# cl-volume-renderer/cl-volume-renderer

Measured on AMD Instinct MI355X. Metric: msamples_per_sec, higher is better.
Workload: dtype f32

## Files before the change

cl_volume_renderer_amd/csrc/bounce_device.hpp:

```cpp
#pragma once
#include "render_device.hpp"

namespace clvr {

__device__ __forceinline__ VolumePacked make_volume(const RenderArgs &a) {
  return VolumePacked{a.grec, a.stepb, a.volume_lin, a.sdf_lin, a.X, a.Y, a.Z, a.NBX, a.NBY};
}

__device__ __forceinline__ uint32_t udivmod24(uint32_t n, uint32_t d, uint32_t &rem) {
  uint32_t q = (uint32_t)((float)n * __builtin_amdgcn_rcpf((float)d));
  uint32_t qd;
  asm("v_mul_u32_u24 %0, %1, %2" : "=v"(qd) : "v"(q), "v"(d));
  int32_t r = (int32_t)(n - qd);
  if (r < 0) { q -= 1u; r += (int32_t)d; }
  if (r >= (int32_t)d) { q += 1u; r -= (int32_t)d; }
  rem = (uint32_t)r;
  return q;
}

__device__ __forceinline__ unsigned prefix_count(unsigned long long mask) {
  return __builtin_amdgcn_mbcnt_hi((unsigned)(mask >> 32), __builtin_amdgcn_mbcnt_lo((unsigned)mask, 0u));
}
__device__ __forceinline__ unsigned lane_id() { return prefix_count(~0ull); }

enum : int { ST_IDLE = 0, ST_MARCH = 1, ST_CERT = 2, ST_EVENT = 8 };
enum : int { EV_START = 3,
             EV_HIT_COLOR_PENDING = 4,
             EV_CHECK = 5 };
constexpr int kCertNever = 255;

template <int MODE>
__device__ __forceinline__ void finish_item(const RenderArgs &a, int64_t entry, uint32_t hit, uint32_t gx, uint32_t gy,
                                            uint32_t bv_r, uint32_t bv_g, uint32_t bv_b) {
  const uint32_t cr = (bv_r / 2u) & 0xFFFFu, cg = (bv_g / 2u) & 0xFFFFu, cb = (bv_b / 2u) & 0xFFFFu;
  if (MODE == CLWH_ACCUM_VOXEL_CACHE && a.grants == nullptr) {
    cache_add(a.cache, entry, cr, cg, cb, 0u);
  } else {
    const unsigned long long packed = (unsigned long long)cr | ((unsigned long long)cg << 16) |
                                      ((unsigned long long)cb << 32) | (1ull << 48);
    atomicAdd(a.delta + hit, packed);
  }
  if (a.contrib_out) {
    uint32_t *q = a.contrib_out + ((size_t)gy * (size_t)a.launch_w + gx) * 4;
    q[0] = cr; q[1] = cg; q[2] = cb; q[3] = 1u;
  }
}

constexpr int kFixupDwords = 32;

__device__ __forceinline__ bool certify_exit(const RenderArgs &a, f3 p, f3 d, int budget, int &away) {
  const unsigned cx = min((unsigned)(int)p.x >> a.macro_shift, (unsigned)a.MNX - 1u), cy = min((unsigned)(int)p.y >> a.macro_shift, (unsigned)a.MNY - 1u),
                 cz = min((unsigned)(int)p.z >> a.macro_shift, (unsigned)a.MNZ - 1u);
  const unsigned octant = (d.x < 0.0f ? 1u : 0u) | (d.y < 0.0f ? 2u : 0u) | (d.z < 0.0f ? 4u : 0u);
  const int entry = a.macro[(((cz * (unsigned)a.MNY + cy) * (unsigned)a.MNX + cx) << 3) | octant];
  const bool refused = (entry & (int)kCertRefused) != 0;
  const int box_min = refused ? 0 : entry;
  away = refused ? ((entry & 0x7F) - 1) << a.macro_shift : 0;
  const float dmin = fminf(fminf(fabsf(d.x), fabsf(d.y)), fabsf(d.z));
  const float dsum = d.x + d.y + d.z;
  const float T = (float)((budget - 5) * box_min);
  const float fx = d.x < 0.0f ? p.x : (float)a.X - p.x, fy = d.y < 0.0f ? p.y : (float)a.Y - p.y, fz = d.z < 0.0f ? p.z : (float)a.Z - p.z;
  const bool leaves = T * fabsf(d.x) >= fx || T * fabsf(d.y) >= fy || T * fabsf(d.z) >= fz;
  return box_min != 0 && budget > 5 && leaves && dmin >= 0.0009765625f && dsum == dsum;
}
__device__ __forceinline__ bool start_certificate(uint32_t mask, f3 d, float dmin_needed) {
  const unsigned octant = (d.x < 0.0f ? 1u : 0u) | (d.y < 0.0f ? 2u : 0u) | (d.z < 0.0f ? 4u : 0u);
  const float dmin = fminf(fminf(fabsf(d.x), fabsf(d.y)), fabsf(d.z));
  const float dsum = d.x + d.y + d.z;
  return ((mask >> octant) & 1u) != 0u && dmin >= dmin_needed && dsum == dsum;
}
__device__ __forceinline__ f3 hull_direction(unsigned k) {
  static_assert(kHullGrid == 64, "cell centres are odd multiples of 1/64");
  const float u = (float)(2 * (int)(k & 63u) - 63) * 0.015625f, v = (float)(2 * (int)((k >> 6) & 63u) - 63) * 0.015625f;
  const float z = (1.0f - fabsf(u)) - fabsf(v);
  const float x = z >= 0.0f ? u : copysignf(1.0f - fabsf(v), u), y = z >= 0.0f ? v : copysignf(1.0f - fabsf(u), v);
  const float r = __builtin_amdgcn_rsqf((x * x + y * y) + z * z);
  return f3{x * r, y * r, z * r};
}
__device__ __forceinline__ bool certify_exit(const RenderArgs &a, f3 p, f3 d, int budget) {
  int away;
  return certify_exit(a, p, d, budget, away);
}

template <int SMALL>
__device__ __forceinline__ void index_tables_to_lds(VolumePacked &vol, const RenderArgs &a, int threads) {
  extern __shared__ uint32_t lds_parts[];
  if (SMALL == 2) {
    vol.parts = lds_parts;
    vol.parts_y0 = a.X;
    vol.parts_z0 = a.X + a.Y;
    for (int k = (int)threadIdx.x; k < a.X + a.Y + a.Z; k += threads)
      lds_parts[k] = k < a.X ? vol.part_x<1>((unsigned)k) : (k < a.X + a.Y ? vol.part_y<1>((unsigned)(k - a.X)) : vol.part_z<1>((unsigned)(k - a.X - a.Y)));
  }
}
__device__ __forceinline__ unsigned home_queue_of(const RenderArgs &a, unsigned waves_per_block) {
  unsigned home_queue = (unsigned)__builtin_amdgcn_s_getreg((3 << 11) | 20) & 7u;
  if (a.unit_affinity == 1) home_queue = (blockIdx.x * waves_per_block + (threadIdx.x >> 6)) & 7u;
  if (a.unit_affinity == 2) home_queue = 0u;
  return home_queue;
}

#ifdef CLVR_BOUNCE_STATS
constexpr bool kBounceStats = true;
constexpr bool kStartCertVerify = (CLVR_BOUNCE_STATS + 0) != 2;
#else
constexpr bool kBounceStats = false;
constexpr bool kStartCertVerify = false;
#endif
template <bool ON> struct BounceStatsT;
template <> struct BounceStatsT<false> {
  __device__ void step(int) {}
  __device__ void cert_begin(int, int) {}
  __device__ void cert_end(int, int) {}
  __device__ void closing_half(int) {}
  __device__ void event_phase(int) {}
  __device__ void refill(uint32_t) {}
  __device__ void fresh_items(int, int) {}
  __device__ void swap_point() {}
  __device__ void start_cert(bool, bool) {}
  __device__ void hull_cert(bool, bool, bool) {}
  __device__ void hull_more(bool, bool, bool, bool) {}
  __device__ void hull_fired(bool, bool) {}
  __device__ void march_end(uint32_t *, int) {}
  template <bool TWO_RAYS> __device__ void flush(uint32_t *) {}
};
template <> struct BounceStatsT<true> {
  uint32_t step_iters = 0, step_lanes = 0, event_phases = 0, event_lanes = 0, refills = 0, refill_lanes = 0;
  uint32_t ev_kind[4] = {0, 0, 0, 0};
  uint32_t cert_phases = 0, cert_lanes = 0, cert_granted = 0;
  uint32_t step_idle = 0;
  uint32_t swaps = 0;
  uint32_t closing = 0, marching_before = 0;
  __device__ __forceinline__ void step(int st) {
    step_iters += 1; step_lanes += (uint32_t)__popcll(__ballot(st == ST_MARCH));
    step_idle += (uint32_t)__popcll(__ballot(st == ST_IDLE));
  }
  __device__ __forceinline__ void cert_begin(int st, int n_cert) {
    cert_phases += 1; cert_lanes += (uint32_t)n_cert;
    marching_before = (uint32_t)__popcll(__ballot(st == ST_MARCH));
  }
  __device__ __forceinline__ void cert_end(int st, int n_cert) { cert_granted += (uint32_t)(n_cert - (__popcll(__ballot(st == ST_MARCH)) - (int)marching_before)); }
  __device__ __forceinline__ void closing_half(int st) {
    closing = (uint32_t)__popcll(__ballot(st >= ST_EVENT));
    event_lanes += closing;
    ev_kind[1] += (uint32_t)__popcll(__ballot(st == ST_EVENT + EV_EXIT || st == ST_EVENT + EV_CHECK));
    ev_kind[2] += (uint32_t)__popcll(__ballot(st == ST_EVENT + EV_HIT || st == ST_EVENT + EV_HIT_COLOR_PENDING));
    ev_kind[3] += (uint32_t)__popcll(__ballot(st == ST_EVENT + EV_NONE));
  }
  __device__ __forceinline__ void event_phase(int st) {
    if (__ballot(st >= ST_EVENT) != 0ull) { event_phases += 1; event_lanes += (uint32_t)__popcll(__ballot(st >= ST_EVENT)); }
  }
  __device__ __forceinline__ void refill(uint32_t count) { refills += 1; refill_lanes += count; }
  __device__ __forceinline__ void fresh_items(int st, int o) {
    const uint32_t n_fresh = (uint32_t)__popcll(__ballot(st == ST_EVENT + EV_START && o == 1));
    ev_kind[0] += n_fresh; event_lanes += n_fresh;
    if (closing + n_fresh != 0u) event_phases += 1;
  }
  __device__ __forceinline__ void swap_point() { swaps += 1; }
  uint32_t start_tried = 0, start_granted = 0;
  bool start_open = false;
  __device__ __forceinline__ void start_cert(bool tried, bool granted) {
    start_tried += (uint32_t)__popcll(__ballot(tried)); start_granted += (uint32_t)__popcll(__ballot(granted));
    start_open = start_open || granted;
  }
  uint32_t hull_tried = 0, hull_granted = 0, hull_both = 0;
  bool hull_open = false;
  __device__ __forceinline__ void hull_cert(bool tried, bool granted, bool both) {
    hull_tried += (uint32_t)__popcll(__ballot(tried)); hull_granted += (uint32_t)__popcll(__ballot(granted));
    hull_both += (uint32_t)__popcll(__ballot(both));
    hull_open = hull_open || granted;
  }
  uint32_t more_tried[3] = {0, 0, 0}, more_granted[3] = {0, 0, 0};
  int more_open = -1;
  __device__ __forceinline__ void hull_more(bool rebound_tried, bool rebound_granted, bool armed, bool first_leg) {
    more_tried[0] += (uint32_t)__popcll(__ballot(armed && first_leg)); more_tried[2] += (uint32_t)__popcll(__ballot(armed && !first_leg));
    more_tried[1] += (uint32_t)__popcll(__ballot(rebound_tried)); more_granted[1] += (uint32_t)__popcll(__ballot(rebound_granted));
    if (rebound_granted) more_open = 1;
  }
  __device__ __forceinline__ void hull_fired(bool fired, bool first_leg) {
    more_granted[0] += (uint32_t)__popcll(__ballot(fired && first_leg)); more_granted[2] += (uint32_t)__popcll(__ballot(fired && !first_leg));
    if (fired) more_open = first_leg ? 0 : 2;
  }
  __device__ __forceinline__ void march_end(uint32_t *counters, int ev) {
    if (start_open && ev != EV_EXIT) atomicAdd(&counters[CTR_START_WRONG], 1u);
    if (hull_open && ev != EV_EXIT) atomicAdd(&counters[CTR_HULL_WRONG], 1u);
    if (more_open >= 0 && ev != EV_EXIT) atomicAdd(&counters[CTR_HULL_DEFER + 3 * more_open + 2], 1u);
    start_open = false;
    hull_open = false;
    more_open = -1;
  }
  template <bool TWO_RAYS> __device__ __forceinline__ void flush(uint32_t *counters) {
    atomicAdd(&counters[CTR_STEP_ITERS], step_iters); atomicAdd(&counters[CTR_STEP_LANES], step_lanes);
    atomicAdd(&counters[CTR_EVENT_PHASES], event_phases); atomicAdd(&counters[CTR_EVENT_LANES], event_lanes);
    atomicAdd(&counters[CTR_REFILLS], refills); atomicAdd(&counters[CTR_REFILL_LANES], refill_lanes);
    if (TWO_RAYS) { atomicAdd(&counters[CTR_SWAPS], swaps); return; }
    for (int k = 0; k < 4; ++k) atomicAdd(&counters[CTR_EV_KIND + k], ev_kind[k]);
    atomicAdd(&counters[CTR_CERT_PHASES], cert_phases); atomicAdd(&counters[CTR_CERT_LANES], cert_lanes);
    atomicAdd(&counters[CTR_CERT_GRANTED], cert_granted); atomicAdd(&counters[CTR_STEP_IDLE], step_idle);
    atomicAdd(&counters[CTR_START_TRIED], start_tried); atomicAdd(&counters[CTR_START_GRANTED], start_granted);
    atomicAdd(&counters[CTR_HULL_TRIED], hull_tried); atomicAdd(&counters[CTR_HULL_GRANTED], hull_granted); atomicAdd(&counters[CTR_HULL_BOTH], hull_both);
    for (int k = 0; k < 3; ++k) { atomicAdd(&counters[CTR_HULL_DEFER + 3 * k], more_tried[k]); atomicAdd(&counters[CTR_HULL_DEFER + 3 * k + 1], more_granted[k]); }
  }
};
using BounceStats = BounceStatsT<kBounceStats>;

}
```

cl_volume_renderer_amd/csrc/clwh_context.hip:

```cpp
#include <algorithm>
#include <cstdio>
#include <cstdlib>
#include <cstring>
#include <mutex>
#include <new>

#include "clwh_host.hpp"

using namespace clvr;

static thread_local int g_last_hip_error = 0;
void clvr::note_hip_error(hipError_t e) { g_last_hip_error = (int)e; }

static std::atomic<uint64_t> g_content_version{0};
static std::mutex g_cells_mutex;
static std::map<const void *, std::weak_ptr<VersionCell>> g_version_cells;
void clwh_touch(clwh_mem *m) { m->cell->v.store(++g_content_version, std::memory_order_relaxed); }

static std::shared_ptr<VersionCell> version_cell_of(const void *dptr) {
  std::lock_guard<std::mutex> lock(g_cells_mutex);
  auto it = g_version_cells.find(dptr);
  if (it != g_version_cells.end())
    if (auto live = it->second.lock()) return live;
  auto cell = std::make_shared<VersionCell>();
  g_version_cells[dptr] = cell;
  if (g_version_cells.size() > 4096) {
    for (auto i = g_version_cells.begin(); i != g_version_cells.end();)
      i = i->second.expired() ? g_version_cells.erase(i) : std::next(i);
  }
  return cell;
}

static size_t elem_size(int kind) {
  switch (kind) {
    case CLWH_ELEM_S8: case CLWH_ELEM_U8: return 1;
    case CLWH_ELEM_S16: case CLWH_ELEM_U16: return 2;
    case CLWH_ELEM_S32: case CLWH_ELEM_U32: case CLWH_ELEM_F32: return 4;
    default: return 0;
  }
}


void clvr::tf_to_dev(const clwh_tf &tf, TfDev &d) {
  std::memset(&d, 0, sizeof d);
  d.n = tf.n;
  for (int k = 0; k < tf.n; ++k) {
    const clwh_tf_rule &r = tf.rules[k];
    TfRuleDev &o = d.rules[k];
    o.v_lo = r.v_lo; o.v_hi = r.v_hi; o.g_lo = r.g_lo; o.g_hi = r.g_hi;
    o.flags = (r.use_gradient ? TF_USE_GRADIENT : 0u) | (r.writes_color ? TF_WRITES_COLOR : 0u) |
              (r.terminal ? TF_TERMINAL : 0u);
    o.color = ((uint32_t)r.color[0] & 255u) | (((uint32_t)r.color[1] & 255u) << 8) |
              (((uint32_t)r.color[2] & 255u) << 16) | (((uint32_t)r.color[3] & 255u) << 24);
    if (r.use_gradient) d.uses_gradient = 1;
  }
  for (int k = 0; k < tf.n && !d.uses_gradient; ++k) {
    const clwh_tf_rule &r = tf.rules[k];
    if (r.v_lo <= 0 && 0 <= r.v_hi) { d.border_class = k + 1; break; }
    if (r.terminal) break;
  }
}

int clvr::jit_for_source(clwh_ctx *ctx, const char *source, std::shared_ptr<JitTf> &out) {
  auto it = ctx->classes.cache.find(source);
  if (it != ctx->classes.cache.end()) {
    out = it->second;
    return CLWH_OK;
  }
  auto j = std::make_shared<JitTf>();
  j->source = source;
  std::string log;
  const int rc = tf_jit_compile(source, j->code, log);
  if (rc != CLWH_OK) {
    if (!log.empty()) std::fprintf(stderr, "clwhip: transfer-function source is neither in the rule grammar nor compilable:\n%s\n", log.c_str());
    return rc;
  }
  ctx->classes.cache[source] = j;
  out = j;
  return CLWH_OK;
}

int clvr::ensure_classes(clwh_ctx *ctx, const std::shared_ptr<JitTf> &jit, const clwh_mem *volume, TfDev &tf_out, const uint8_t **cls_out) {
  TfClasses &c = ctx->classes;
  if (c.cls.ptr && c.vol == volume->dptr && c.vol_ver == volume->version() && c.source == jit->source) {
    tf_out = c.tf;
    *cls_out = c.cls.as<uint8_t>();
    return CLWH_OK;
  }
  if (!jit->module) {
    HIP_TRY(hipModuleLoadData(&jit->module, jit->code.data()));
    HIP_TRY(hipModuleGetFunction(&jit->classify, jit->module, "clvr_tf_classify"));
  }
  const size_t voxels = volume->dims[0] * volume->dims[1] * volume->dims[2];
  CLWH_TRY(c.cls.reserve(ctx->stream, voxels));
  constexpr int kColors = CLWH_TF_MAX_RULES;
  CLWH_TRY(c.palette.reserve(ctx->stream, (kColors + 2) * sizeof(unsigned long long)));
  unsigned long long *palette = c.palette.as<unsigned long long>();
  HIP_TRY(hipMemsetAsync(palette, 0xFF, kColors * sizeof(unsigned long long), ctx->stream));
  HIP_TRY(hipMemsetAsync(palette + kColors, 0, 2 * sizeof(unsigned long long), ctx->stream));
  const void *vol = volume->dptr;
  int X = (int)volume->dims[0], Y = (int)volume->dims[1], Z = (int)volume->dims[2], max_colors = kColors;
  unsigned char *cls = c.cls.as<unsigned char>();
  int *error = reinterpret_cast<int *>(palette + kColors);
  int *border = reinterpret_cast<int *>(palette + kColors + 1);
  void *args[] = {&vol, &X, &Y, &Z, &cls, &palette, &max_colors, &error, &border};
  const size_t blocks = std::min<size_t>((voxels + 255u) / 256u, (size_t)1u << 23);
  HIP_TRY(hipModuleLaunchKernel(jit->classify, (unsigned)blocks, 1, 1, 256, 1, 1, 0, ctx->stream, args, nullptr));
  unsigned long long host[kColors + 2];
  HIP_TRY(hipMemcpyAsync(host, palette, sizeof host, hipMemcpyDeviceToHost, ctx->stream));
  HIP_TRY(hipStreamSynchronize(ctx->stream));
  c.vol = nullptr;
  if ((int)(host[kColors] & 0xFFFFFFFFull) != 0) return CLWH_ERR_TF_UNSUPPORTED;
  TfDev t;
  std::memset(&t, 0, sizeof t);
  t.opaque = 1;
  for (int k = 0; k < kColors && host[k] != ~0ull; ++k) {
    t.rules[k].flags = (host[k] >> 32) & 1ull ? TF_WRITES_COLOR : 0u;
    t.rules[k].color = (uint32_t)(host[k] & 0xFFFFFFFFull);
    t.n = k + 1;
  }
  t.border_class = (int32_t)(host[kColors + 1] & 0xFFull);
  c.tf = t;
  c.vol = volume->dptr;
  c.vol_ver = volume->version();
  c.source = jit->source;
  tf_out = t;
  *cls_out = cls;
  return CLWH_OK;
}


Tuning clvr::tuning_from_environment() {
  Tuning t;
  auto clamped = [](const char *e, int lo, int hi) { return std::max(lo, std::min(hi, std::atoi(e))); };
  if (const char *e = std::getenv("CLWH_TUNE_STEP")) t.step_min_lanes = clamped(e, 0, 64);
  if (const char *e = std::getenv("CLWH_TUNE_REFILL")) t.refill_min_lanes = clamped(e, 0, 64);
  if (const char *e = std::getenv("CLWH_TUNE_LITERAL_GRADIENT")) t.literal_gradient = std::atoi(e) != 0;
  if (const char *e = std::getenv("CLWH_TUNE_AFFINITY")) t.unit_affinity = std::atoi(e);
  if (const char *e = std::getenv("CLWH_TUNE_QUEUES")) t.unit_queues = clamped(e, 1, 8);
  if (const char *e = std::getenv("CLWH_TUNE_GROUP")) t.unit_group = std::max(1, std::atoi(e));
  if (const char *e = std::getenv("CLWH_TUNE_CHUNK_BLOCK_LOG2")) t.unit_block_log2 = clamped(e, 0, 8);
  if (const char *e = std::getenv("CLWH_TUNE_BLOCKS")) t.bounce_max_blocks = (uint32_t)std::max(1, std::atoi(e));
  if (const char *e = std::getenv("CLWH_TUNE_MACRO_SHIFT")) t.macro_shift = std::atoi(e);
  if (const char *e = std::getenv("CLWH_TUNE_LONG_LAUNCH")) t.force_long_launch = std::atoi(e) != 0;
  if (const char *e = std::getenv("CLWH_TUNE_BOUNCE_RAYS")) t.bounce_rays = std::atoi(e) == 2 ? 2 : 1;
  if (const char *e = std::getenv("CLWH_TUNE_SDF")) t.sdf_front = std::strcmp(e, "front") == 0;
  if (const char *e = std::getenv("CLWH_TUNE_DIST_LINES")) t.dist_lines = std::strcmp(e, "scan") == 0 ? 1 : std::strcmp(e, "search") == 0 ? 2 : 0;
  if (const char *e = std::getenv("CLWH_TUNE_LABEL_STATS")) t.label_stats = std::strcmp(e, "item") == 0 ? 1 : std::strcmp(e, "direct") == 0 ? 2 : 0;
  if (const char *e = std::getenv("CLWH_TUNE_SLICE_COARSE")) t.slice_coarse = std::atoi(e) != 0;
  if (const char *e = std::getenv("CLWH_TUNE_SDFBIT_WAVES")) t.sdfbit_waves = std::atoi(e) == 16 ? 16 : 8;
  if (const char *e = std::getenv("CLWH_TUNE_SDFBIT_GRID")) t.sdfbit_grid = std::max(1, std::atoi(e));
  if (const char *e = std::getenv("CLWH_TUNE_SDFBIT_REC")) t.sdfbit_rec_lds = std::strcmp(e, "lds") == 0 ? 1 : 0;
  if (const char *e = std::getenv("CLWH_TUNE_CERT")) t.cert_min_step = clamped(e, 0, 127);
  if (const char *e = std::getenv("CLWH_TUNE_CERT_HINT")) t.cert_hint = std::atoi(e) != 0;
  if (const char *e = std::getenv("CLWH_TUNE_START_CERT")) t.start_cert = std::atoi(e) != 0;
  if (const char *e = std::getenv("CLWH_TUNE_HULL_CERT")) t.hull_cert = std::atoi(e) != 0;
  if (const char *e = std::getenv("CLWH_TUNE_HULL_DEFER")) t.hull_defer = std::atoi(e) != 0;
  return t;
}

int clvr::check_device_flags(clwh_ctx *ctx) {
  PassScratch &p = ctx->pass;
  if (!p.fixup_overflow_pending || !p.sticky_flags.ptr) return CLWH_OK;
  uint32_t flag = 0;
  HIP_TRY(hipMemcpyAsync(&flag, p.sticky_flags.ptr, sizeof flag, hipMemcpyDeviceToHost, ctx->stream));
  HIP_TRY(hipStreamSynchronize(ctx->stream));
  p.fixup_overflow_pending = false;
  if (!flag) return CLWH_OK;
  HIP_TRY(hipMemsetAsync(p.sticky_flags.ptr, 0, sizeof(uint32_t), ctx->stream));
  return CLWH_ERR_INTERNAL_OVERFLOW;
}

int clvr::timed_begin(clwh_ctx *ctx, int which, hipEvent_t *end) {
  LaunchTimers &t = ctx->timers;
  if (!t.enabled) return CLWH_OK;
  if (t.used == t.pairs.size()) {
    LaunchTimers::Pair &fresh = t.pairs.emplace_back();
    int rc = fresh.begin.ensure(hipEventDefault);
    if (rc == CLWH_OK) rc = fresh.end.ensure(hipEventDefault);
    if (rc != CLWH_OK) {
      t.pairs.pop_back();
      return rc;
    }
  }
  LaunchTimers::Pair &p = t.pairs[t.used++];
  p.which = which;
  HIP_TRY(hipEventRecord(p.begin.ev, ctx->stream));
  *end = p.end.ev;
  return CLWH_OK;
}

static int order_streams(clwh_ctx *ctx, hipStream_t first, hipStream_t then) {
  HIP_TRY(hipSetDevice(ctx->device));
  CLWH_TRY(ctx->handoff.ensure(hipEventDisableTiming));
  HIP_TRY(hipEventRecord(ctx->handoff.ev, first));
  HIP_TRY(hipStreamWaitEvent(then, ctx->handoff.ev, 0));
  return CLWH_OK;
}

extern "C" {

int clwh_ctx_create_on_stream(int device, void *hip_stream, clwh_ctx **out) {
  if (!out) return CLWH_ERR_INVALID_VALUE;
  *out = nullptr;
  int count = 0;
  hipError_t e = hipGetDeviceCount(&count);
  if (e != hipSuccess || count <= 0) {
    note_hip_error(e);
    return CLWH_ERR_NO_DEVICE;
  }
  if (device < 0 || device >= count) return CLWH_ERR_NO_DEVICE;
  HIP_TRY(hipSetDevice(device));
  clwh_ctx *c = new (std::nothrow) clwh_ctx();
  if (!c) return CLWH_ERR_OUT_OF_MEMORY;
  c->device = device;
  c->stream = (hipStream_t)hip_stream;
  c->own_stream = false;
  c->tune = tuning_from_environment();
  *out = c;
  return CLWH_OK;
}

int clwh_ctx_create(int device, clwh_ctx **out) {
  CLWH_TRY(clwh_ctx_create_on_stream(device, nullptr, out));
  hipStream_t s;
  hipError_t e = hipStreamCreateWithFlags(&s, hipStreamNonBlocking);
  if (e != hipSuccess) {
    note_hip_error(e);
    delete *out;
    *out = nullptr;
    return CLWH_ERR_HIP;
  }
  (*out)->stream = s;
  (*out)->own_stream = true;
  return CLWH_OK;
}

int clwh_ctx_destroy(clwh_ctx *ctx) {
  if (!ctx) return CLWH_ERR_INVALID_VALUE;
  (void)hipSetDevice(ctx->device);
  (void)hipStreamSynchronize(ctx->stream);
  for (auto &kv : ctx->classes.cache)
    if (kv.second->module) (void)hipModuleUnload(kv.second->module);
  ctx->scene.reset();
  const hipStream_t owned = ctx->own_stream ? ctx->stream : nullptr;
  delete ctx;
  if (owned) (void)hipStreamDestroy(owned);
  return CLWH_OK;
}

int clwh_ctx_finish(clwh_ctx *ctx) {
  if (!ctx) return CLWH_ERR_INVALID_VALUE;
  HIP_TRY(hipStreamSynchronize(ctx->stream));
  return check_device_flags(ctx);
}

int clwh_ctx_acquire_from(clwh_ctx *ctx, void *hip_stream) {
  if (!ctx) return CLWH_ERR_INVALID_VALUE;
  return order_streams(ctx, (hipStream_t)hip_stream, ctx->stream);
}

int clwh_ctx_release_to(clwh_ctx *ctx, void *hip_stream) {
  if (!ctx) return CLWH_ERR_INVALID_VALUE;
  return order_streams(ctx, ctx->stream, (hipStream_t)hip_stream);
}

void *clwh_ctx_stream(clwh_ctx *ctx) { return ctx ? (void *)ctx->stream : nullptr; }
int clwh_ctx_device(clwh_ctx *ctx) { return ctx ? ctx->device : -1; }

int clwh_ctx_set_timing(clwh_ctx *ctx, int enabled) {
  if (!ctx) return CLWH_ERR_INVALID_VALUE;
  ctx->timers.enabled = enabled != 0;
  ctx->timers.used = 0;
  return CLWH_OK;
}

int clwh_ctx_timing_read_all(clwh_ctx *ctx, float *ms, int32_t *launches, int32_t n) {
  if (!ctx || !ms || !launches || n <= 0) return CLWH_ERR_INVALID_VALUE;
  for (int k = 0; k < n; ++k) { ms[k] = 0.0f; launches[k] = 0; }
  HIP_TRY(hipSetDevice(ctx->device));
  LaunchTimers &timers = ctx->timers;
  for (size_t i = 0; i < timers.used; ++i) {
    const LaunchTimers::Pair &p = timers.pairs[i];
    HIP_TRY(hipEventSynchronize(p.end.ev));
    float t = 0.0f;
    HIP_TRY(hipEventElapsedTime(&t, p.begin.ev, p.end.ev));
    if (p.which >= 0 && p.which < n) { ms[p.which] += t; launches[p.which] += 1; }
  }
  timers.used = 0;
  return CLWH_OK;
}

int clwh_ctx_timing_read(clwh_ctx *ctx, float *total_ms, int32_t *launches) {
  if (!ctx || !total_ms || !launches) return CLWH_ERR_INVALID_VALUE;
  float ms[CLWH_TIMER_COUNT];
  int32_t n[CLWH_TIMER_COUNT];
  const int rc = clwh_ctx_timing_read_all(ctx, ms, n, CLWH_TIMER_COUNT);
  *total_ms = ms[CLWH_TIMER_BOUNCE];
  *launches = n[CLWH_TIMER_BOUNCE];
  return rc;
}


static int mem_new(clwh_ctx *ctx, void *dptr, size_t bytes, bool owned, clwh_mem **out) {
  clwh_mem *m = new (std::nothrow) clwh_mem();
  if (!m) return CLWH_ERR_OUT_OF_MEMORY;
  m->ctx = ctx;
  m->dptr = dptr;
  m->bytes = bytes;
  m->owned = owned;
// ... 155 lines not shown
```

cl_volume_renderer_amd/csrc/clwh_host.hpp:

```cpp
#pragma once

#include <atomic>
#include <deque>
#include <map>
#include <memory>
#include <string>
#include <vector>

#include "clwh_internal.hpp"

namespace clvr {

void note_hip_error(hipError_t e);
inline int hip_failed(hipError_t e) {
  note_hip_error(e);
  return e == hipErrorOutOfMemory ? CLWH_ERR_OUT_OF_MEMORY : CLWH_ERR_HIP;
}
#define HIP_TRY(expr)                                   \
  do {                                                  \
    hipError_t _e = (expr);                             \
    if (_e != hipSuccess) return clvr::hip_failed(_e);  \
  } while (0)
#define CLWH_TRY(expr)                \
  do {                                \
    int _rc = (expr);                 \
    if (_rc != CLWH_OK) return _rc;   \
  } while (0)

struct NoCopy {
  NoCopy() = default;
  NoCopy(const NoCopy &) = delete;
  NoCopy &operator=(const NoCopy &) = delete;
};

struct DeviceBuffer : NoCopy {
  void *ptr = nullptr;
  size_t bytes = 0;
  ~DeviceBuffer() { if (ptr) (void)hipFree(ptr); }
  template <class T>
  T *as() const { return static_cast<T *>(ptr); }
  void *release() {
    void *p = ptr;
    ptr = nullptr;
    bytes = 0;
    return p;
  }
  int reserve(hipStream_t stream, size_t need, bool *reallocated = nullptr) {
    if (reallocated) *reallocated = bytes < need;
    if (bytes >= need) return CLWH_OK;
    if (ptr) {
      HIP_TRY(hipStreamSynchronize(stream));
      HIP_TRY(hipFree(ptr));
      (void)release();
    }
    HIP_TRY(hipMalloc(&ptr, need));
    bytes = need;
    return CLWH_OK;
  }
};

struct Event : NoCopy {
  hipEvent_t ev = nullptr;
  ~Event() { if (ev) (void)hipEventDestroy(ev); }
  int ensure(unsigned flags) {
    if (!ev) HIP_TRY(hipEventCreateWithFlags(&ev, flags));
    return CLWH_OK;
  }
};

struct PinnedWord : NoCopy {
  uint32_t *ptr = nullptr;
  ~PinnedWord() { if (ptr) (void)hipHostFree(ptr); }
  int ensure() {
    if (!ptr) HIP_TRY(hipHostMalloc((void **)&ptr, 64, hipHostMallocDefault));
    return CLWH_OK;
  }
};

int tf_jit_compile(const char *user_source, std::vector<char> &code, std::string &log);
struct JitTf {
  std::string source;
  std::vector<char> code;
  hipModule_t module = nullptr;
  hipFunction_t classify = nullptr;
};

struct PackedScene {
  int device = 0;
  DeviceBuffer data;
  const void *vol = nullptr, *sdf = nullptr;
  uint64_t vol_ver = 0, sdf_ver = 0;
  TfDev tf{};
  std::string tf_identity;
  int32_t macro_shift = 0;
  bool start_table = false;
  bool hull_table = false;
  int32_t dims[3] = {0, 0, 0};
  uint64_t generation = 0;
  Event ready;
  bool stale = false;
  ~PackedScene();
};

struct VersionCell {
  std::atomic<uint64_t> v{0};
};


struct Tuning {
  int32_t step_min_lanes = 0;
  int32_t refill_min_lanes = 0;
  int32_t macro_shift = 0;
  int32_t bounce_rays = 1;
  int32_t force_long_launch = 0;
  int32_t literal_gradient = 0;
  int32_t unit_block_log2 = 4;
  int32_t unit_group = 1, unit_affinity = 0, unit_queues = 8;
  int32_t cert_hint = 1;
  int32_t start_cert = 1;
  int32_t hull_cert = 1;
  int32_t hull_defer = 1;
  int32_t cert_min_step = -1;
  uint32_t bounce_max_blocks = 2048;
  int32_t sdfbit_waves = 8;
  int32_t sdfbit_grid = 512;
  int32_t sdfbit_rec_lds = 0;
  int32_t sdf_front = 0;
  int32_t dist_lines = 0;
  int32_t label_stats = 0;
  int32_t slice_coarse = 1;
};
Tuning tuning_from_environment();

struct PrimaryHits {
  struct Key {
    float cam_pos[3], cam_dir[3];
    int32_t frame_w, frame_h, launch_w, launch_h, tile_rank, tile_world;
    int64_t cache_entries;
    int32_t mode, shading;
    uint64_t packed_generation;
    const void *env;
    uint64_t env_version;
    int32_t env_w, env_h;
  } key{};
  bool valid = false;
  DeviceBuffer pix_slot, hits;
  DeviceBuffer hull_codes;
  DeviceBuffer hull_planes;
  uint32_t n_hits = 0;
  bool n_hits_known = false;
  PinnedWord host_n_hits;
  Event n_hits_event;
  bool n_hits_in_flight = false;
  uint32_t last_known_n_hits = 0;
};

struct PassScratch {
  static constexpr size_t kCounters = CTR_QUEUE_STRIDE * 10;
  DeviceBuffer counters;
  DeviceBuffer fixups, delta;
  DeviceBuffer sticky_flags;
  bool fixup_overflow_pending = false;
};

struct VoxelPlan {
  DeviceBuffer plan;
  DeviceBuffer temp;
  bool valid = false;
  uint32_t n = 0;
};

struct TfClasses {
  std::map<std::string, std::shared_ptr<JitTf>> cache;
  DeviceBuffer cls;
  DeviceBuffer palette;
  const void *vol = nullptr;
  uint64_t vol_ver = 0;
  std::string source;
  TfDev tf{};
};

struct SdfScratch {
  DeviceBuffer counters;
  DeviceBuffer flags;
  DeviceBuffer bits;
#ifdef CLVR_SDFBIT_TIMING
  DeviceBuffer timing;
#endif
};

struct TileScratch {
  DeviceBuffer tiles, seeds;
  PinnedWord host;
};

struct GrowScratch {
  DeviceBuffer admissible;
  TileScratch work;
};

struct LabelScratch {
  DeviceBuffer admissible, keys, temp, counters;
  PinnedWord host;
};

struct DistanceScratch {
  DeviceBuffer map_a, map_b, bits;
};

struct GeodesicScratch {
  DeviceBuffer keys, trace;
  TileScratch work;
};

struct RegionStatsScratch {
  DeviceBuffer result;
};

struct OverlayScratch {
  DeviceBuffer pixel_ids, occupancy;
};

struct ProjectionData {
  DeviceBuffer data;
  bool valid = false;
  const void *vol = nullptr;
  uint64_t vol_ver = 0;
  size_t dims[3] = {0, 0, 0};
  DeviceBuffer dilated;
  bool dilated_valid = false;
  DeviceBuffer mesh_counts, mesh_temp, mesh_points;
  DeviceBuffer lut_prefix;
  bool lut_valid = false;
  const void *lut = nullptr;
  uint64_t lut_ver = 0;
  int32_t lut_len = 0;
};

struct LaunchTimers {
  struct Pair {
    Event begin, end;
    int which = 0;
  };
  bool enabled = false;
  std::deque<Pair> pairs;
  size_t used = 0;
};

}

struct clwh_ctx {
  int device = 0;
  hipStream_t stream = nullptr;
  bool own_stream = false;
  clvr::Event handoff;
  clvr::Tuning tune;
  clvr::PrimaryHits primary;
  clvr::PassScratch pass;
  clvr::VoxelPlan vox;
  clvr::TfClasses classes;
  clvr::SdfScratch sdf;
  clvr::GrowScratch grow;
  clvr::LabelScratch label;
  clvr::DistanceScratch distance;
  clvr::GeodesicScratch geodesic;
  clvr::RegionStatsScratch region_stats;
  clvr::OverlayScratch overlay;
  clvr::ProjectionData proj;
  clvr::DeviceBuffer bilateral_weights;
  std::shared_ptr<clvr::PackedScene> scene;
  clvr::LaunchTimers timers;
};

struct clwh_mem {
  clwh_ctx *ctx = nullptr;
  void *dptr = nullptr;
  size_t bytes = 0;
  bool owned = false;
  bool is_image = false;
  size_t dims[3] = {1, 1, 1};
  int channels = 1;
  int elem_kind = CLWH_ELEM_U8;
  int flags = 0;
  std::shared_ptr<clvr::VersionCell> cell;
  uint64_t version() const { return cell ? cell->v.load(std::memory_order_relaxed) : 0; }
};

enum clwh_kernel_id {
  CLWH_K_EMPTY = 0,
  CLWH_K_RENDER,
  CLWH_K_SDF_BASE,
  CLWH_K_SDF_LAYER,
  CLWH_K_BUFFER_RESET,
  CLWH_K_FETCH_STATS,
  CLWH_K_APPLY_CLIP,
  CLWH_K_TF_SORT_VALUES,
  CLWH_K_TF_FLUSH_COLOR_FRAME,
  CLWH_K_BILATERAL_FILTER
};

struct clwh_kernel {
  clwh_ctx *ctx = nullptr;
  int id = CLWH_K_EMPTY;
  clwh_tf tf{};
  bool has_tf = false;
  std::shared_ptr<clvr::JitTf> jit;
};

void clwh_touch(clwh_mem *m);

namespace clvr {

inline void touch(clwh_mem *m) { clwh_touch(m); }
// ... 102 lines not shown
```

cl_volume_renderer_amd/csrc/clwh_internal.hpp:

```cpp
#pragma once

#include <hip/hip_runtime.h>
#include <stdint.h>

#include "../../include/clwh.h"

namespace clvr {

struct TfRuleDev {
  int32_t v_lo, v_hi, g_lo, g_hi;
  uint32_t flags;
  uint32_t color;
};
struct TfDev {
  int32_t n;
  int32_t uses_gradient;
  int32_t literal_gradient_taps;
  int32_t opaque;
  int32_t border_class;
  TfRuleDev rules[CLWH_TF_MAX_RULES];
};

enum : uint32_t { TF_USE_GRADIENT = 1u, TF_WRITES_COLOR = 2u, TF_TERMINAL = 4u };

struct HitRec {
  float origin[3];
  float direction[3];
  float normal[3];
  uint32_t color;
  int32_t entry_lo;
  int32_t entry_hi;
  uint32_t xy;
  uint32_t pslot;
  uint32_t start_free;
  uint32_t pad;
};
static_assert(sizeof(HitRec) == 64, "HitRec must be one 64-byte line");

enum : uint32_t { PIX_HIT = 0x80000000u };

constexpr uint32_t kCertMinStep = 2u;
constexpr uint32_t kCertRefused = 0x80u;

enum : uint32_t {
  CTR_HITS = 0, CTR_FIXUPS = 2,
  CTR_STEP_ITERS = 8, CTR_STEP_LANES, CTR_EVENT_PHASES, CTR_EVENT_LANES, CTR_REFILLS, CTR_REFILL_LANES,
  CTR_EV_KIND,
  CTR_CERT_PHASES = CTR_EV_KIND + 4, CTR_CERT_LANES, CTR_CERT_GRANTED,
  CTR_SWAPS, CTR_STEP_IDLE,
  CTR_START_TRIED, CTR_START_GRANTED, CTR_START_WRONG,
  CTR_HULL_TRIED, CTR_HULL_GRANTED, CTR_HULL_BOTH, CTR_HULL_WRONG,
  CTR_STATS_END,
  CTR_QUEUE_STRIDE = 32,
  CTR_HULL_DEFER = CTR_QUEUE_STRIDE * 9, CTR_HULL_DEFER_END = CTR_HULL_DEFER + 9,
};
struct RenderArgs {
  int32_t X, Y, Z;
  const uint2 *grec;
  const uint8_t *stepb;
  const int16_t *volume_lin;
  const int8_t *sdf_lin;
  const uint8_t *macro;
  int32_t MNX, MNY, MNZ, macro_shift;
  int32_t cert_min_step;
  int32_t cert_min_lanes;
  int32_t cert_hint;
  const uint8_t *start_free;
  float start_cert_dmin;
  const float4 *hull;
  uint32_t *hull_codes;
  float hull_delta0;
  uint32_t *hull_planes;
  float hull_defer_delta0;
  int32_t NBX, NBY;
  const uint32_t *env;
  int32_t env_w, env_h;
  uint32_t *cache;
  int64_t cache_entries;
  uint32_t *frame;
  int32_t frame_w, frame_h;
  int32_t launch_w, launch_h;
  int32_t tiles_x, tiles_y, tiles_per_row;
  int32_t tile_rank, tile_world;
  float cam_pos[3];
  float cam_dir[3];
  int32_t mode;
  float4 *accum;
  unsigned long long *delta;
  const uint32_t *grants;
  uint32_t *pix_slot;
  HitRec *hits;
  uint32_t *counters;
  uint32_t *fixups;
  uint32_t fixup_capacity;
  uint32_t *sticky_flags;
  uint32_t n_hits;
  uint32_t n_hits_estimate;
  int32_t n_hits_on_device;
  int32_t shading;
  int64_t *hit_index_out;
  uint32_t *contrib_out;
  uint32_t num_tile_slots;
  int32_t n_seeds;
  int32_t seeds[CLWH_MAX_SEEDS];
  int32_t step_min_lanes;
  int32_t refill_min_lanes;
  int32_t force_long_launch;
  int32_t bounce_rays;
  uint32_t bounce_max_blocks;
  int32_t unit_group;
  int32_t unit_block_log2;
  int32_t unit_queues;
  int32_t unit_affinity;
  TfDev tf;
};

struct RepackArgs {
  const int16_t *volume;
  const int8_t *sdf;
  int32_t X, Y, Z;
  int32_t NBX, NBY, NBZ;
  uint2 *grec;
  uint8_t *stepb;
  uint32_t *brick_min;
  const uint8_t *cls_in;
  TfDev tf;
};

struct SdfArgs {
  const int16_t *volume;
  int32_t X, Y, Z;
  int8_t *ping;
  int8_t *pong;
  int32_t max_iterations;
  int32_t iteration;
  int32_t *counters;
  int32_t *done;
  int32_t *counter_out;
  const uint8_t *cls_in;
  TfDev tf;
};

hipError_t launch_repack(const RepackArgs &a, hipStream_t s);
inline int macro_cell_shift(int X, int Y, int Z, int forced) {
  if (forced >= 3 && forced <= 8) return forced;
  auto cells = [&](int sh) { return (int64_t)((X >> sh) + 1) * ((Y >> sh) + 1) * ((Z >> sh) + 1); };
  int shift = 4;
  if (cells(4) > 40000) {
    shift = 5;
    while (shift < 8 && cells(shift) > 300000) ++shift;
  }
  return shift;
}
hipError_t launch_macro_table(const uint32_t *brick_min, int NBX, int NBY, int NBZ, uint8_t *macro, int X, int Y, int Z, int shift, hipStream_t s);
hipError_t launch_start_table(const uint8_t *stepb, uint8_t *table, uint32_t *regular, int2 *ends, int X, int Y, int Z, int NBX, int NBY, int NBZ, hipStream_t s);
inline int start_cert_cap(int X, int Y, int Z) {
  const int longest = X > Y ? (X > Z ? X : Z) : (Y > Z ? Y : Z);
  return longest / 2 < 127 ? longest / 2 : 127;
}
inline float start_cert_dmin(int X, int Y, int Z) {
  const double longest = (double)(X > Y ? (X > Z ? X : Z) : (Y > Z ? Y : Z));
  const double reach = 1.7320508075688772 * (longest + 1.0), cap = (double)start_cert_cap(X, Y, Z);
  for (int k = 1; k <= 64; ++k) {
    const double dmin = (double)k / 64.0;
    double t = 0.0;
    for (int step = 0; step < 70 - 5 && t <= reach; ++step) {
      const double m = (double)(long long)(t * dmin) - 2.0;
      const double bound = m > cap ? cap : m;
      t += bound < 1.0 ? 1.0 : bound;
    }
    if (t > reach) return (float)dmin;
  }
  return 2.0f;
}
constexpr int kHullGrid = 64;
constexpr int kHullPlanes = kHullGrid * kHullGrid;
constexpr float kHullSlack = 0.0625f;
constexpr int kHullMaxDim = 2048;
inline float hull_cert_delta0(int X, int Y, int Z) {
  const double longest = (double)(X > Y ? (X > Z ? X : Z) : (Y > Z ? Y : Z));
  const double reach = 1.7320508075688772 * (longest + 1.0), cap = (double)start_cert_cap(X, Y, Z);
  for (int k = 1; k <= 64; ++k) {
    const double delta0 = (double)k / 64.0;
    double t = 0.0;
    for (int step = 0; step < 70 - 5 && t <= reach; ++step) {
      const double m = (double)(long long)(t * delta0 / 1.7320508075688772) - 2.0;
      const double bound = m > cap ? cap : m;
      t += bound < 1.0 ? 1.0 : bound;
    }
    if (t > reach) return (float)delta0;
  }
  return 2.0f;
}
constexpr int kHullDeferSteps = 3;
constexpr float kHullDeferDeficit = 1.5f;
constexpr int kHullMarginScale = 16;
inline float hull_defer_delta0(int X, int Y, int Z) {
  const double longest = (double)(X > Y ? (X > Z ? X : Z) : (Y > Z ? Y : Z));
  const double reach = 1.7320508075688772 * (longest + 1.0), cap = (double)start_cert_cap(X, Y, Z);
  for (int k = 1; k <= 64; ++k) {
    const double delta0 = (double)k / 64.0;
    double t = 0.0;
    for (int step = 0; step < 70 - 5 - kHullDeferSteps && t <= reach; ++step) {
      const double m = (double)(long long)(t * delta0 / 1.7320508075688772) - 2.0;
      const double bound = m > cap ? cap : m;
      t += bound < 1.0 ? 1.0 : bound;
    }
    if (t > reach) return (float)delta0;
  }
  return 2.0f;
}
hipError_t launch_hull_table(const int2 *ends, const uint32_t *regular, float4 *hull, int X, int Y, int Z, hipStream_t s);
constexpr uint64_t kStartTableBudget = 2ull << 30;
hipError_t launch_primary(const RenderArgs &a, hipStream_t s);
hipError_t launch_bounce(const RenderArgs &a, hipStream_t s);
inline bool bounce_queues_fit(uint32_t n_hits, int32_t unit_block_log2, int32_t n_seeds) {
  return (uint64_t)(((n_hits + 63u) >> 6) + 8u * (1u << unit_block_log2)) * (uint64_t)n_seeds < (1ull << 24);
}
hipError_t launch_env_fixup(const RenderArgs &a, hipStream_t s);
hipError_t launch_commit(const RenderArgs &a, hipStream_t s);
constexpr int64_t kVoxKeyInvalid = (int64_t)1 << 38;
constexpr int64_t kVoxKeyNone = ((int64_t)1 << 38) + 1;
hipError_t launch_vox_keys(const RenderArgs &a, int64_t *keys, uint32_t *iota, uint32_t n, hipStream_t s);
hipError_t launch_vox_grant(const RenderArgs &a, const int64_t *sorted_keys, const uint32_t *order, uint32_t n, uint32_t *grants, hipStream_t s);
hipError_t launch_commit_voxel(const RenderArgs &a, hipStream_t s);
hipError_t sort_entry_pairs(void *temp, size_t &temp_bytes, const int64_t *keys_in, int64_t *keys_out, const uint32_t *vals_in,
                            uint32_t *vals_out, size_t n, unsigned end_bit, hipStream_t s);
hipError_t launch_resolve(const RenderArgs &a, hipStream_t s);
hipError_t launch_ao(const RenderArgs &a, hipStream_t s);
hipError_t launch_accum_resolve(const RenderArgs &a, const float4 *accum_all, hipStream_t s);
hipError_t launch_accum_resolve_tiles(const RenderArgs &a, const float4 *accum, uint32_t *tiles_out, hipStream_t s);
hipError_t launch_frame_from_tiles(const RenderArgs &a, const uint32_t *tiles_all, hipStream_t s);
struct ProbeShape {
  uint32_t in_words, out_words;
};
ProbeShape probe_shape(int which);
hipError_t launch_device_probe(int which, const uint32_t *in, uint64_t n, uint32_t *out, const uint32_t *aux, const int32_t params[4], hipStream_t s);
struct SdfFrontArgs {
  int8_t *sdf;
  int32_t X, Y, Z;
  int32_t TX, TY, TZ;
  const uint8_t *flags_cur;
  uint8_t *flags_next;
  uint8_t *flags_clear;
  uint8_t *tile_done;
  int32_t iteration;
  int32_t max_iterations;
  int32_t *counters;
};

struct SdfBitArgs {
  int8_t *sdf;
  const uint32_t *ev;
  const uint32_t *r_in;
  uint32_t *r_out;
  uint8_t *state;
  uint8_t *wake;
  int32_t launch;
  int32_t *presence;
  int32_t X, Y, Z, WP;
  int32_t BX, BY, BZ, core_z;
  int32_t r0, steps;
  uint32_t *planes;
  size_t plane_words;
  uint32_t *list;
  uint32_t *list_count;
  uint32_t *list_head;
#ifdef CLVR_SDFBIT_TIMING
  unsigned long long *timing;
#endif
};
void sdfbit_block_grid(int X, int Y, int Z, int waves, int32_t *BX, int32_t *BY, int32_t *BZ, int32_t *core_z);
hipError_t launch_sdfbit_events(const SdfArgs &a, uint32_t *ev, int32_t WP, hipStream_t s);
hipError_t launch_sdfbit_seed(const SdfBitArgs &a, hipStream_t s);
hipError_t launch_sdfbit_expand(const SdfBitArgs &a, const uint32_t *reached, int32_t max_iterations, hipStream_t s);
hipError_t launch_sdfbit_state(const SdfBitArgs &a, hipStream_t s);
hipError_t launch_sdfbit_layers(const SdfBitArgs &a, int waves, unsigned grid_blocks, bool rec_in_lds, hipStream_t s);

inline unsigned row_block(int X) { return X <= 64 ? 64u : (X <= 128 ? 128u : 256u); }
inline dim3 row_grid(int X, int Y, int Z) { return dim3(((unsigned)X + row_block(X) - 1u) / row_block(X), (unsigned)Y, (unsigned)Z); }
hipError_t launch_sdf_base(const SdfArgs &a, hipStream_t s);
hipError_t launch_sdf_base_front(const SdfArgs &a, uint8_t *flags, int32_t TX, int32_t TY, hipStream_t s);
hipError_t launch_sdf_front(const SdfFrontArgs &a, hipStream_t s);
hipError_t launch_sdf_layer(const SdfArgs &a, hipStream_t s);
hipError_t launch_fetch_stats(const int16_t *vol, int X, int Y, int Z, int32_t *stats, hipStream_t s);
hipError_t launch_tf_sort_values(const int16_t *vol, int X, int Y, int Z, uint32_t *frame, int width, int height,
                                 float min_v, float max_v, float min_g, float max_g, hipStream_t s);
hipError_t launch_tf_flush_color_frame(uint32_t *color_frame, int fw, int fh, const int32_t *frame, const int32_t *lookup,
                                       int lookup_len, hipStream_t s);
hipError_t launch_bilateral_filter(const int16_t *src, int X, int Y, int Z, int16_t *dst, const float *weights, hipStream_t s);
hipError_t launch_apply_clip(const int16_t *src, int SX, int SY, int SZ, int16_t *dst, int DX, int DY, int DZ,
                             const uint32_t *start, const uint32_t *len, hipStream_t s);


struct ViewVolume {
  const int16_t *bricks;
  const uint32_t *table, *dilated, *coarse;
  int32_t X, Y, Z, NBX, NBY, NBZ, CNX, CNY;
};
struct ViewFrame {
  uint32_t *frame;
  int32_t frame_w, frame_h;
  int32_t launch_w, launch_h, tiles_x, num_tiles;
};
struct ViewCamera {
  float cam_pos[3], cam_dir[3];
  float step, t_near, t_far;
  int32_t k_cap;
};

struct ProjRepackArgs {
  const int16_t *volume;
  int32_t X, Y, Z, NBX, NBY, NBZ;
  int16_t *bricks;
  uint32_t *table;
};
struct ProjArgs {
  ViewVolume vol;
  ViewFrame fr;
  ViewCamera cam;
  float window_center, window_width;
  float *values;
  float *t_extreme;
};
hipError_t launch_proj_repack(const ProjRepackArgs &a, hipStream_t s);
hipError_t launch_projection(const ProjArgs &a, int mode, bool dense, hipStream_t s);

struct CompArgs {
  ViewVolume vol;
  ViewFrame fr;
  ViewCamera cam;
  const float4 *lut;
  const uint32_t *prefix;
  int32_t lut_first, lut_len;
  float alpha_stop, ambient;
  float4 *rgba;
  float *t_first;
  float *t_stop;
};
hipError_t launch_comp_prefix(const float4 *lut, int32_t lut_len, uint32_t *prefix, hipStream_t s);
hipError_t launch_composite(const CompArgs &a, bool shade, bool dense, hipStream_t s);

struct IsoArgs {
  ViewVolume vol;
  ViewFrame fr;
  ViewCamera cam;
  int64_t threshold;
  int32_t skip_bound;
  int32_t refine;
  float color[3], ambient;
  float *t_hit;
  float4 *normal;
};
hipError_t launch_iso_dilate(const ViewVolume &v, uint32_t *dilated, hipStream_t s);
hipError_t launch_isosurface(const IsoArgs &a, bool below, bool dense, hipStream_t s);

struct SliceArgs {
  ViewVolume vol;
  ViewFrame fr;
  int32_t use_coarse;
  float origin[3], du[3], dv[3], normal[3];
  float step;
  float window_center, window_width;
  int32_t slab_samples;
  float *values;
  float *t_extreme;
};
hipError_t launch_slice(const SliceArgs &a, int mode, bool dense, hipStream_t s);
// ... 186 lines not shown
```

cl_volume_renderer_amd/csrc/clwh_render.hip:

```cpp
#include <algorithm>
#include <cstdio>
#include <cstring>
#include <mutex>

#include "clwh_host.hpp"

using namespace clvr;


static std::mutex g_scenes_mutex;
static std::vector<std::weak_ptr<PackedScene>> g_packed_scenes;
static std::atomic<uint64_t> g_packed_generation{0};

PackedScene::~PackedScene() {
  (void)hipSetDevice(device);
  (void)hipDeviceSynchronize();
}

struct PackedLayout {
  int X, Y, Z, NBX, NBY, NBZ, mshift, MNX, MNY, MNZ;
  size_t records, n_bricks, off_stepb, off_brick_min, off_macro, off_start, off_hull_ends, off_hull, bytes;
  bool start_table;
  bool hull_table;
};
// ... 81 lines not shown
  r.cls_in = cls_in;
  r.tf = tf;
  CLWH_TRY(timed(ctx, CLWH_TIMER_REPACK, [&] {
    const hipError_t e = launch_repack(r, ctx->stream);
    if (e != hipSuccess) return e;
    return launch_macro_table(r.brick_min, L.NBX, L.NBY, L.NBZ, data + L.off_macro, L.X, L.Y, L.Z, L.mshift, ctx->stream);
  }));
  if (L.start_table)
    CLWH_TRY(timed(ctx, CLWH_TIMER_REPACK, [&] {
      int2 *ends = L.hull_table ? reinterpret_cast<int2 *>(data + L.off_hull_ends) : nullptr;
      const hipError_t e = launch_start_table(r.stepb, data + L.off_start + 16u, reinterpret_cast<uint32_t *>(data + L.off_start), ends, L.X, L.Y, L.Z, L.NBX, L.NBY, L.NBZ, ctx->stream);
      if (e != hipSuccess || !L.hull_table) return e;
      return launch_hull_table(ends, reinterpret_cast<const uint32_t *>(data + L.off_start), reinterpret_cast<float4 *>(data + L.off_hull), L.X, L.Y, L.Z, ctx->stream);
    }));
  HIP_TRY(hipEventRecord(entry->ready.ev, ctx->stream));
  ctx->scene = entry;
  {
    std::lock_guard<std::mutex> lock(g_scenes_mutex);
    entry->vol = volume->dptr;
    entry->sdf = sdf->dptr;
    entry->vol_ver = volume->version();
    entry->sdf_ver = sdf->version();
    entry->tf = tf;
    entry->tf_identity = tf_identity;
    entry->macro_shift = L.mshift;
    entry->start_table = L.start_table;
    entry->hull_table = L.hull_table;
    entry->dims[0] = L.X; entry->dims[1] = L.Y; entry->dims[2] = L.Z;
    entry->generation = ++g_packed_generation;
    entry->stale = false;
    bool listed = false;
    for (auto &w : g_packed_scenes)
      if (w.lock() == entry) listed = true;
    if (!listed) g_packed_scenes.push_back(entry);
  }
  return CLWH_OK;
}


static void describe_frame(RenderArgs &a, int32_t launch_w, int32_t launch_h, int32_t frame_w, int32_t frame_h,
                           int32_t rank, int32_t world, const float cam_pos[3], const float cam_dir[3]) {
  a.launch_w = launch_w;
  a.launch_h = launch_h;
  a.frame_w = frame_w;
  a.frame_h = frame_h;
  a.tiles_x = launch_w / 8;
  a.tiles_y = launch_h / 8;
  a.tile_rank = rank;
  a.tile_world = world;
  a.tiles_per_row = (a.tiles_x + world - 1) / world;
  a.num_tile_slots = (uint32_t)a.tiles_y * (uint32_t)a.tiles_per_row;
  for (int q = 0; q < 3; ++q) {
    a.cam_pos[q] = cam_pos[q];
    a.cam_dir[q] = cam_dir[q];
  }
}

static size_t pixel_slots(const RenderArgs &a) { return (size_t)a.num_tile_slots * 64u; }
static size_t launch_pixels(const RenderArgs &a) { return (size_t)a.launch_w * (size_t)a.launch_h; }
static bool is_planned(const RenderArgs &a) { return a.mode == CLWH_ACCUM_VOXEL_CACHE && a.n_seeds > 1; }

static int validate_desc(const clwh_render_desc *d) {
  if (!is_image(d->volume, 3, 1, CLWH_ELEM_S16) || !is_image(d->sdf, 3, 1, CLWH_ELEM_S8) ||
      !is_image(d->env, 2, 4, CLWH_ELEM_U8))
    return CLWH_ERR_BAD_ARGS;
  if (d->frame && !is_image(d->frame, 2, 4, CLWH_ELEM_U8)) return CLWH_ERR_BAD_ARGS;
  if (!same_dims(d->volume, d->sdf)) return CLWH_ERR_SIZE_MISMATCH;
  if (!launch_size_ok(d->width, d->height)) return CLWH_ERR_BAD_NDRANGE;
  if (d->width > 65535u || d->height > 65535u) return CLWH_ERR_BAD_NDRANGE;
  if (d->env->dims[0] > 32768u || d->env->dims[1] > 32768u) return CLWH_ERR_INVALID_VALUE;
  if (!dims_fit_int32(d->volume)) return CLWH_ERR_INVALID_VALUE;
  const int world = d->tile_world < 1 ? 1 : d->tile_world;
  if (d->tile_rank < 0 || d->tile_rank >= world) return CLWH_ERR_INVALID_VALUE;
  if (d->n_seeds < 0 || d->n_seeds > CLWH_MAX_SEEDS) return CLWH_ERR_INVALID_VALUE;
  if (d->n_seeds > 1 && d->contrib) return CLWH_ERR_BAD_ARGS;
  if (d->shading != CLWH_SHADE_LIGHT && d->shading != CLWH_SHADE_AO) return CLWH_ERR_INVALID_VALUE;
  if (d->shading == CLWH_SHADE_AO && d->accum_mode != CLWH_ACCUM_VOXEL_CACHE) return CLWH_ERR_BAD_ARGS;
  return CLWH_OK;
}

static int describe_launch(const clwh_ctx *ctx, const clwh_render_desc *d, RenderArgs &a) {
  std::memset(&a, 0, sizeof a);
  a.X = (int32_t)d->volume->dims[0];
  a.Y = (int32_t)d->volume->dims[1];
  a.Z = (int32_t)d->volume->dims[2];
  env_into_args(a, d->env);
  const int32_t fw = d->frame ? (int32_t)d->frame->dims[0] : (int32_t)d->width;
  const int32_t fh = d->frame ? (int32_t)d->frame->dims[1] : (int32_t)d->height;
  const int world = d->tile_world < 1 ? 1 : d->tile_world;
  describe_frame(a, (int32_t)d->width, (int32_t)d->height, fw, fh, d->tile_rank, world, d->cam_pos, d->cam_dir);
  a.frame = d->frame ? (uint32_t *)d->frame->dptr : nullptr;
  a.mode = d->accum_mode;
  a.shading = d->shading;
  if (a.mode == CLWH_ACCUM_VOXEL_CACHE) {
    if (!d->buffer_volume || d->buffer_volume->bytes < 8) return CLWH_ERR_BAD_ARGS;
    a.cache = (uint32_t *)d->buffer_volume->dptr;
    a.cache_entries = (int64_t)(d->buffer_volume->bytes / (d->shading == CLWH_SHADE_AO ? 4 : 8));
  } else if (a.mode == CLWH_ACCUM_IMAGE_SPACE) {
    const int64_t need = clwh_accum_len(d->width, d->height, world) * 16;
    if (!d->accum || (int64_t)d->accum->bytes < need) return CLWH_ERR_BAD_ARGS;
    a.accum = (float4 *)d->accum->dptr;
  } else {
    return CLWH_ERR_INVALID_VALUE;
  }
  if (d->hit_index) {
    if (d->hit_index->bytes < launch_pixels(a) * 8) return CLWH_ERR_SIZE_MISMATCH;
    a.hit_index_out = (int64_t *)d->hit_index->dptr;
  }
  if (d->contrib) {
    if (d->contrib->bytes < launch_pixels(a) * 16) return CLWH_ERR_SIZE_MISMATCH;
    a.contrib_out = (uint32_t *)d->contrib->dptr;
  }
  if (d->n_seeds > 0) {
    a.n_seeds = d->n_seeds;
    for (int q = 0; q < d->n_seeds; ++q) a.seeds[q] = d->seeds[q];
  } else {
    a.n_seeds = 1;
    a.seeds[0] = d->seed;
  }
  const Tuning &t = ctx->tune;
  a.step_min_lanes = t.step_min_lanes;
  a.refill_min_lanes = t.refill_min_lanes;
  a.force_long_launch = t.force_long_launch;
  a.bounce_rays = t.bounce_rays;
  a.bounce_max_blocks = t.bounce_max_blocks;
  a.unit_group = t.unit_group;
  a.unit_block_log2 = t.unit_block_log2;
  a.unit_affinity = t.unit_affinity;
  a.unit_queues = t.unit_queues;
  a.cert_hint = t.cert_hint;
  a.start_cert_dmin = start_cert_dmin(a.X, a.Y, a.Z);
  a.hull_delta0 = hull_cert_delta0(a.X, a.Y, a.Z);
  a.hull_defer_delta0 = hull_defer_delta0(a.X, a.Y, a.Z);
  return CLWH_OK;
}

static int bind_scene(clwh_kernel *k, const clwh_render_desc *d, RenderArgs &a) {
  clwh_ctx *ctx = k->ctx;
  const uint8_t *cls_in = nullptr;
  CLWH_TRY(kernel_tf(k, d->volume, a.tf, &cls_in));
  a.tf.literal_gradient_taps = ctx->tune.literal_gradient;
  const PackedLayout L = packed_layout(d->volume, ctx->tune.macro_shift, wants_start_table(ctx->tune, a.tf, d->volume), wants_hull_table(ctx->tune, a.tf, d->volume));
  CLWH_TRY(ensure_packed(ctx, L, d->volume, d->sdf, a.tf, cls_in, k->jit ? k->jit->source : std::string()));
  const uint8_t *packed = ctx->scene->data.as<uint8_t>();
  a.grec = reinterpret_cast<const uint2 *>(packed);
  a.NBX = L.NBX;
  a.NBY = L.NBY;
  a.stepb = packed + L.off_stepb;
  a.volume_lin = (const int16_t *)d->volume->dptr;
  a.sdf_lin = (const int8_t *)d->sdf->dptr;
  a.macro = packed + L.off_macro;
  a.start_free = L.start_table ? packed + L.off_start + 16u : nullptr;
  a.hull = L.hull_table ? reinterpret_cast<const float4 *>(packed + L.off_hull) : nullptr;
  a.macro_shift = L.mshift;
  a.MNX = L.MNX; a.MNY = L.MNY; a.MNZ = L.MNZ;
  bool zero_may_hit = a.tf.border_class != 0;
  for (int q = 0; q < a.tf.n && a.tf.uses_gradient && !a.tf.opaque; ++q)
    if (a.tf.rules[q].v_lo <= 0 && 0 <= a.tf.rules[q].v_hi) zero_may_hit = true;
  const int cert_auto = a.macro_shift < 4 ? 12 >> (4 - a.macro_shift) : std::min(12 << (a.macro_shift - 4), 48);
  a.cert_min_step = zero_may_hit ? 0 : (ctx->tune.cert_min_step >= 0 ? ctx->tune.cert_min_step : cert_auto);
  return CLWH_OK;
}

static int ensure_primary_hits(clwh_ctx *ctx, const clwh_render_desc *d, RenderArgs &a) {
  PrimaryHits &p = ctx->primary;
  PassScratch &s = ctx->pass;
  const size_t slots = pixel_slots(a);
  CLWH_TRY(p.pix_slot.reserve(ctx->stream, slots * sizeof(uint32_t)));
  CLWH_TRY(p.hits.reserve(ctx->stream, slots * sizeof(HitRec)));
  if (a.hull) CLWH_TRY(p.hull_codes.reserve(ctx->stream, slots * sizeof(uint32_t)));
  const bool defer = a.hull && ctx->tune.hull_defer != 0;
  if (defer) CLWH_TRY(p.hull_planes.reserve(ctx->stream, slots * sizeof(uint32_t)));
  CLWH_TRY(s.counters.reserve(ctx->stream, PassScratch::kCounters * sizeof(uint32_t)));
  bool fresh_flags = false;
  CLWH_TRY(s.sticky_flags.reserve(ctx->stream, 64, &fresh_flags));
  if (fresh_flags) HIP_TRY(hipMemsetAsync(s.sticky_flags.ptr, 0, 64, ctx->stream));
  a.sticky_flags = s.sticky_flags.as<uint32_t>();
  a.pix_slot = p.pix_slot.as<uint32_t>();
  a.hits = p.hits.as<HitRec>();
  a.hull_codes = a.hull ? p.hull_codes.as<uint32_t>() : nullptr;
  a.hull_planes = defer ? p.hull_planes.as<uint32_t>() : nullptr;
  a.counters = s.counters.as<uint32_t>();

  PrimaryHits::Key key;
  std::memset(&key, 0, sizeof key);
  for (int q = 0; q < 3; ++q) {
    key.cam_pos[q] = a.cam_pos[q];
    key.cam_dir[q] = a.cam_dir[q];
  }
  key.frame_w = a.frame_w; key.frame_h = a.frame_h;
  key.launch_w = a.launch_w; key.launch_h = a.launch_h;
  key.tile_rank = a.tile_rank; key.tile_world = a.tile_world;
  key.cache_entries = a.cache_entries;
  key.mode = a.mode;
  key.shading = a.shading;
  key.packed_generation = ctx->scene->generation;
  key.env = d->env->dptr;
  key.env_version = d->env->version();
  key.env_w = a.env_w; key.env_h = a.env_h;
  if (p.valid && std::memcmp(&key, &p.key, sizeof key) == 0 && !a.hit_index_out) return CLWH_OK;
  p.valid = false;
  HIP_TRY(hipMemsetAsync(a.counters, 0, PassScratch::kCounters * sizeof(uint32_t), ctx->stream));
  CLWH_TRY(timed(ctx, CLWH_TIMER_PRIMARY, [&] { return launch_primary(a, ctx->stream); }));
  CLWH_TRY(p.host_n_hits.ensure());
  CLWH_TRY(p.n_hits_event.ensure(hipEventDisableTiming));
  HIP_TRY(hipMemcpyAsync(p.host_n_hits.ptr, a.counters + CTR_HITS, sizeof(uint32_t), hipMemcpyDeviceToHost, ctx->stream));
  HIP_TRY(hipEventRecord(p.n_hits_event.ev, ctx->stream));
  p.n_hits_in_flight = true;
  ctx->vox.valid = false;
  p.n_hits_known = false;
  p.key = key;
  p.valid = true;
  return CLWH_OK;
}

static int pick_up_hit_count(clwh_ctx *ctx, RenderArgs &a) {
  PrimaryHits &p = ctx->primary;
  if (p.n_hits_in_flight && !p.n_hits_known) {
    if (hipEventQuery(p.n_hits_event.ev) == hipSuccess) {
      p.n_hits = *p.host_n_hits.ptr;
      p.n_hits_known = true;
      p.n_hits_in_flight = false;
      p.last_known_n_hits = p.n_hits;
    } else {
      (void)hipGetLastError();
    }
  }
  const size_t slots = pixel_slots(a);
  a.n_hits_on_device = !p.n_hits_known;
  a.n_hits = p.n_hits_known ? p.n_hits : (uint32_t)std::min<size_t>(slots, 0xFFFFFFFFu);
  a.n_hits_estimate = a.n_hits;
  if (!p.n_hits_known && p.last_known_n_hits != 0)
    a.n_hits_estimate = (uint32_t)std::min<uint64_t>(a.n_hits, std::max<uint64_t>(2ull * p.last_known_n_hits, slots / 4u));
  if (!bounce_queues_fit(a.n_hits, ctx->tune.unit_block_log2, a.n_seeds)) return CLWH_ERR_INVALID_VALUE;
  return CLWH_OK;
}

static int size_pass_buffers(clwh_ctx *ctx, RenderArgs &a) {
  PassScratch &s = ctx->pass;
  const double rate = std::min(1.0, std::max(1.0 / 64.0, 3.0 * 8.0e-6 * (0.16 * a.env_w + 0.32 * a.env_h)));
  const size_t fix_cap = std::max<size_t>((size_t)((double)a.n_hits_estimate * (double)a.n_seeds * rate), 4096u);
  CLWH_TRY(s.fixups.reserve(ctx->stream, fix_cap * 128u));
  a.fixups = s.fixups.as<uint32_t>();
  a.fixup_capacity = (uint32_t)std::min<size_t>(s.fixups.bytes / 128u, 0x7fffffffu);
  if (a.mode == CLWH_ACCUM_IMAGE_SPACE || is_planned(a)) {
    bool fresh = false;
    CLWH_TRY(s.delta.reserve(ctx->stream, std::max<size_t>(pixel_slots(a), 1) * sizeof(unsigned long long), &fresh));
    a.delta = s.delta.as<unsigned long long>();
    if (fresh) HIP_TRY(hipMemsetAsync(s.delta.ptr, 0, s.delta.bytes, ctx->stream));
  }
  return CLWH_OK;
}

static int plan_voxel_grants(clwh_ctx *ctx, RenderArgs &a) {
  if (!is_planned(a)) return CLWH_OK;
  VoxelPlan &v = ctx->vox;
  constexpr size_t kPerElement = 2 * sizeof(int64_t) + 3 * sizeof(uint32_t);
  bool moved = false;
  CLWH_TRY(v.plan.reserve(ctx->stream, pixel_slots(a) * kPerElement, &moved));
  if (moved) v.valid = false;
  const size_t have = v.plan.bytes / kPerElement;
  int64_t *keys_in = v.plan.as<int64_t>(), *keys = keys_in + have;
  uint32_t *iota = reinterpret_cast<uint32_t *>(keys + have), *order = iota + have, *grants = order + have;
  if (!v.valid) {
    const uint32_t n = a.n_hits;
    HIP_TRY(launch_vox_keys(a, keys_in, iota, n, ctx->stream));
    size_t need = 0;
    HIP_TRY(sort_entry_pairs(nullptr, need, keys_in, keys, iota, order, n, 39u, ctx->stream));
    CLWH_TRY(v.temp.reserve(ctx->stream, std::max<size_t>(need, 16)));
    size_t tb = v.temp.bytes;
    HIP_TRY(sort_entry_pairs(v.temp.ptr, tb, keys_in, keys, iota, order, n, 39u, ctx->stream));
    v.valid = true;
    v.n = n;
  }
  HIP_TRY(launch_vox_grant(a, keys, order, v.n, grants, ctx->stream));
  a.grants = grants;
  return CLWH_OK;
}

#ifdef CLVR_BOUNCE_STATS
static int print_bounce_stats(clwh_ctx *ctx, const RenderArgs &a) {
  uint32_t h[CTR_HULL_DEFER_END];
  HIP_TRY(hipMemcpyAsync(h, a.counters, sizeof h, hipMemcpyDeviceToHost, ctx->stream));
  HIP_TRY(hipStreamSynchronize(ctx->stream));
  auto per = [&](int sum, int n) { return h[n] ? (double)h[sum] / h[n] : 0.0; };
  std::fprintf(stderr, "[bounce stats] items=%llu step_iters=%u avg_march_lanes=%.2f event_phases=%u avg_event_lanes=%.2f "
               "refills=%u avg_refill=%.2f events start/exit/hit/none=%u/%u/%u/%u cert_phases=%u avg_cert_lanes=%.2f cert_granted=%u\n",
               (unsigned long long)h[CTR_HITS] * (unsigned long long)a.n_seeds, h[CTR_STEP_ITERS], per(CTR_STEP_LANES, CTR_STEP_ITERS),
               h[CTR_EVENT_PHASES], per(CTR_EVENT_LANES, CTR_EVENT_PHASES), h[CTR_REFILLS], per(CTR_REFILL_LANES, CTR_REFILLS), h[CTR_EV_KIND],
               h[CTR_EV_KIND + 1], h[CTR_EV_KIND + 2], h[CTR_EV_KIND + 3], h[CTR_CERT_PHASES], per(CTR_CERT_LANES, CTR_CERT_PHASES), h[CTR_CERT_GRANTED]);
  if (h[CTR_SWAPS]) std::fprintf(stderr, "[bounce stats] two rays per lane: %u swap points\n", h[CTR_SWAPS]);
  std::fprintf(stderr, "[bounce stats] per step iteration: avg_idle_lanes=%.2f (lane sum %u)\n", per(CTR_STEP_IDLE, CTR_STEP_ITERS), h[CTR_STEP_IDLE]);
  std::fprintf(stderr, "[bounce stats] lane_steps=%u event_lanes=%u start certificates (%s) tried/granted/wrong=%u/%u/%u dmin=%.6f\n", h[CTR_STEP_LANES],
               h[CTR_EVENT_LANES], (CLVR_BOUNCE_STATS + 0) == 2 ? "taken" : "verified: marched literally", h[CTR_START_TRIED], h[CTR_START_GRANTED],
               h[CTR_START_WRONG], (double)a.start_cert_dmin);
  std::fprintf(stderr, "[bounce stats] hull certificates tried/granted/wrong=%u/%u/%u, of the granted the octant proof grants %u; either proof grants %u first legs; delta0=%.6f\n",
               h[CTR_HULL_TRIED], h[CTR_HULL_GRANTED], h[CTR_HULL_WRONG], h[CTR_HULL_BOTH], h[CTR_START_GRANTED] + h[CTR_HULL_GRANTED] - h[CTR_HULL_BOTH],
               (double)a.hull_delta0);
  const uint32_t *m = h + CTR_HULL_DEFER;
  std::fprintf(stderr, "[bounce stats] hull certificates tried/granted/wrong: first legs deferred=%u/%u/%u rebounds at once=%u/%u/%u rebounds deferred=%u/%u/%u; "
               "J=%d D=%.4g defer_delta0=%.6f; look-ups=%u\n", m[0], m[1], m[2], m[3], m[4], m[5], m[6], m[7], m[8], kHullDeferSteps, (double)kHullDeferDeficit,
               (double)a.hull_defer_delta0, h[CTR_CERT_LANES] - ((CLVR_BOUNCE_STATS + 0) == 2 ? m[1] + m[7] : 0u));
  return CLWH_OK;
}
#endif

static int run_pass(clwh_ctx *ctx, const RenderArgs &a) {
  CLWH_TRY(timed(ctx, CLWH_TIMER_BOUNCE, [&] { return launch_bounce(a, ctx->stream); }));
#ifdef CLVR_BOUNCE_STATS
  CLWH_TRY(print_bounce_stats(ctx, a));
#endif
  CLWH_TRY(timed(ctx, CLWH_TIMER_FIXUP, [&] {
    hipError_t e = launch_env_fixup(a, ctx->stream);
    if (e == hipSuccess) e = launch_commit(a, ctx->stream);
    if (e == hipSuccess && is_planned(a)) e = launch_commit_voxel(a, ctx->stream);
    return e;
  }));
  ctx->pass.fixup_overflow_pending = true;
  return CLWH_OK;
}

extern "C" {

int64_t clwh_cache_len(uint32_t X, uint32_t Y, uint32_t Z) {
  return ((int64_t)X * Z * Y + (int64_t)X * Z + X + 1) * 4;
}

int64_t clwh_accum_len(uint32_t width, uint32_t height, int32_t tile_world) {
  if (tile_world < 1) tile_world = 1;
  const int64_t tiles_x = width / 8, tiles_y = height / 8;
  const int64_t tiles_per_row = (tiles_x + tile_world - 1) / tile_world;
  return tiles_y * tiles_per_row * 64;
}

int clwh_render(clwh_kernel *k, const clwh_render_desc *d) {
  if (!k || !d || k->id != CLWH_K_RENDER || !k->has_tf) return CLWH_ERR_INVALID_VALUE;
  clwh_ctx *ctx = k->ctx;
  RenderArgs a;
  CLWH_TRY(validate_desc(d));
  CLWH_TRY(describe_launch(ctx, d, a));
  HIP_TRY(hipSetDevice(ctx->device));
  CLWH_TRY(bind_scene(k, d, a));
  CLWH_TRY(ensure_primary_hits(ctx, d, a));
  CLWH_TRY(pick_up_hit_count(ctx, a));

  HIP_TRY(hipMemsetAsync(a.counters + CTR_HITS + 1, 0, (PassScratch::kCounters - CTR_HITS - 1) * sizeof(uint32_t), ctx->stream));
  if (a.contrib_out) HIP_TRY(hipMemsetAsync(a.contrib_out, 0, launch_pixels(a) * 16, ctx->stream));

  if (d->resolve_only) {
    if (!a.frame) return CLWH_ERR_BAD_ARGS;
  } else if (d->shading == CLWH_SHADE_AO) {
    CLWH_TRY(timed(ctx, CLWH_TIMER_AO, [&] { return launch_ao(a, ctx->stream); }));
  } else {
    CLWH_TRY(size_pass_buffers(ctx, a));
    CLWH_TRY(plan_voxel_grants(ctx, a));
    CLWH_TRY(run_pass(ctx, a));
  }
  if ((d->write_frame || d->resolve_only) && a.frame)
    CLWH_TRY(timed(ctx, CLWH_TIMER_RESOLVE, [&] { return launch_resolve(a, ctx->stream); }));
  if (d->frame) touch(d->frame);
  return CLWH_OK;
}


int clwh_accum_resolve(clwh_ctx *ctx, clwh_mem *accum_all, int32_t tile_world, uint32_t width, uint32_t height,
                       clwh_mem *frame, clwh_mem *env, const float cam_pos[3], const float cam_dir[3]) {
  if (!ctx || !accum_all || !frame || !env || !cam_pos || !cam_dir || tile_world < 1) return CLWH_ERR_INVALID_VALUE;
  if (!is_image(frame, 2, 4, CLWH_ELEM_U8) || !is_image(env, 2, 4, CLWH_ELEM_U8)) return CLWH_ERR_BAD_ARGS;
  if (!launch_size_ok(width, height)) return CLWH_ERR_BAD_NDRANGE;
  const int64_t need = clwh_accum_len(width, height, tile_world) * 16 * tile_world;
  if ((int64_t)accum_all->bytes < need) return CLWH_ERR_SIZE_MISMATCH;
  RenderArgs a;
  std::memset(&a, 0, sizeof a);
  describe_frame(a, (int32_t)width, (int32_t)height, (int32_t)frame->dims[0], (int32_t)frame->dims[1], 0, tile_world,
                 cam_pos, cam_dir);
  a.frame = (uint32_t *)frame->dptr;
  env_into_args(a, env);
  HIP_TRY(hipSetDevice(ctx->device));
  CLWH_TRY(timed(ctx, CLWH_TIMER_RESOLVE, [&] { return launch_accum_resolve(a, (const float4 *)accum_all->dptr, ctx->stream); }));
  touch(frame);
  return CLWH_OK;
}

int clwh_accum_resolve_tiles(clwh_ctx *ctx, clwh_mem *accum, int32_t tile_rank, int32_t tile_world, uint32_t width, uint32_t height,
                             clwh_mem *tiles_rgba8, clwh_mem *env, const float cam_pos[3], const float cam_dir[3]) {
  if (!ctx || !accum || !tiles_rgba8 || !env || !cam_pos || !cam_dir || tile_world < 1 || tile_rank < 0 || tile_rank >= tile_world)
    return CLWH_ERR_INVALID_VALUE;
  if (!is_image(env, 2, 4, CLWH_ELEM_U8)) return CLWH_ERR_BAD_ARGS;
  if (!launch_size_ok(width, height)) return CLWH_ERR_BAD_NDRANGE;
  const int64_t n = clwh_accum_len(width, height, tile_world);
  if ((int64_t)accum->bytes < n * 16 || (int64_t)tiles_rgba8->bytes < n * 4) return CLWH_ERR_SIZE_MISMATCH;
  RenderArgs a;
  std::memset(&a, 0, sizeof a);
  describe_frame(a, (int32_t)width, (int32_t)height, (int32_t)width, (int32_t)height, tile_rank, tile_world, cam_pos, cam_dir);
  env_into_args(a, env);
  HIP_TRY(hipSetDevice(ctx->device));
  CLWH_TRY(timed(ctx, CLWH_TIMER_RESOLVE, [&] {
    return launch_accum_resolve_tiles(a, (const float4 *)accum->dptr, (uint32_t *)tiles_rgba8->dptr, ctx->stream);
  }));
  touch(tiles_rgba8);
  return CLWH_OK;
}

int clwh_frame_from_tiles(clwh_ctx *ctx, clwh_mem *tiles_all, int32_t tile_world, uint32_t width, uint32_t height, clwh_mem *frame) {
  if (!ctx || !tiles_all || !frame || tile_world < 1) return CLWH_ERR_INVALID_VALUE;
  if (!is_image(frame, 2, 4, CLWH_ELEM_U8)) return CLWH_ERR_BAD_ARGS;
  if (!launch_size_ok(width, height)) return CLWH_ERR_BAD_NDRANGE;
  if ((int64_t)tiles_all->bytes < clwh_accum_len(width, height, tile_world) * 4 * tile_world) return CLWH_ERR_SIZE_MISMATCH;
  const float zero[3] = {0.0f, 0.0f, 0.0f};
  RenderArgs a;
  std::memset(&a, 0, sizeof a);
  describe_frame(a, (int32_t)width, (int32_t)height, (int32_t)frame->dims[0], (int32_t)frame->dims[1], 0, tile_world, zero, zero);
  a.frame = (uint32_t *)frame->dptr;
  HIP_TRY(hipSetDevice(ctx->device));
  HIP_TRY(launch_frame_from_tiles(a, (const uint32_t *)tiles_all->dptr, ctx->stream));
  touch(frame);
  return CLWH_OK;
}


int clwh_ctx_invalidate_derived(clwh_ctx *ctx, int what) {
  if (!ctx) return CLWH_ERR_INVALID_VALUE;
  if ((what & CLWH_DERIVED_SCENE) && ctx->scene) {
    {
      std::lock_guard<std::mutex> lock(g_scenes_mutex);
      ctx->scene->stale = true;
    }
    if (ctx->scene.use_count() > 1) ctx->scene.reset();
  }
  if (what & (CLWH_DERIVED_SCENE | CLWH_DERIVED_CAMERA)) ctx->primary.valid = false;
  if (what & CLWH_DERIVED_PROJECTION) ctx->proj.valid = ctx->proj.lut_valid = ctx->proj.dilated_valid = false;
  return CLWH_OK;
}

int clwh_ctx_scene_info(clwh_ctx *ctx, uint64_t *scene_id, uint64_t *bytes, int32_t *holders) {
  if (!ctx) return CLWH_ERR_INVALID_VALUE;
  std::lock_guard<std::mutex> lock(g_scenes_mutex);
  if (scene_id) *scene_id = ctx->scene ? ctx->scene->generation : 0;
  if (bytes) *bytes = ctx->scene ? ctx->scene->data.bytes : 0;
  if (holders) *holders = ctx->scene ? (int32_t)ctx->scene.use_count() : 0;
  return CLWH_OK;
}

int clwh_debug_device_probe(clwh_ctx *ctx, int32_t which, clwh_mem *in, uint64_t n, clwh_mem *out, clwh_mem *aux, const int32_t params[4]) {
  if (!ctx || !in || !out || !params) return CLWH_ERR_INVALID_VALUE;
  const ProbeShape shape = probe_shape(which);
  if (shape.in_words == 0u) return CLWH_ERR_INVALID_VALUE;
  const bool env = which == CLWH_PROBE_ENV_EXACT || which == CLWH_PROBE_ENV_FAST;
  if (env && (!aux || params[0] < 1 || params[1] < 1)) return CLWH_ERR_INVALID_VALUE;
  if (n >= (1ull << 31) || in->bytes < n * shape.in_words * 4u || out->bytes < n * shape.out_words * 4u) return CLWH_ERR_SIZE_MISMATCH;
  if (env && aux->bytes < (uint64_t)params[0] * (uint64_t)params[1] * 4u) return CLWH_ERR_SIZE_MISMATCH;
  if (n == 0) return CLWH_OK;
  HIP_TRY(hipSetDevice(ctx->device));
  HIP_TRY(launch_device_probe(which, (const uint32_t *)in->dptr, n, (uint32_t *)out->dptr, env ? (const uint32_t *)aux->dptr : nullptr, params, ctx->stream));
  return CLWH_OK;
}

static PackedLayout scene_layout(clwh_ctx *ctx) {
  std::lock_guard<std::mutex> lock(g_scenes_mutex);
  clwh_mem shape{};
  for (int q = 0; q < 3; ++q) shape.dims[q] = (size_t)ctx->scene->dims[q];
  return packed_layout(&shape, ctx->scene->macro_shift, ctx->scene->start_table, ctx->scene->hull_table);
}

int clwh_debug_macro_table(clwh_ctx *ctx, void *host_out, uint64_t capacity, int32_t info_out[4]) {
  if (!ctx || !info_out) return CLWH_ERR_INVALID_VALUE;
  if (!ctx->scene) return CLWH_ERR_BAD_ARGS;
  const PackedLayout L = scene_layout(ctx);
  info_out[0] = L.MNX; info_out[1] = L.MNY; info_out[2] = L.MNZ; info_out[3] = L.mshift;
  const size_t bytes = (size_t)L.MNX * L.MNY * L.MNZ * 8u;
  if (!host_out) return CLWH_OK;
  if (capacity < bytes || ctx->scene->data.bytes != L.bytes) return CLWH_ERR_SIZE_MISMATCH;
  HIP_TRY(hipSetDevice(ctx->device));
  HIP_TRY(hipMemcpyAsync(host_out, ctx->scene->data.as<uint8_t>() + L.off_macro, bytes, hipMemcpyDeviceToHost, ctx->stream));
  HIP_TRY(hipStreamSynchronize(ctx->stream));
  return CLWH_OK;
}

int clwh_debug_packed_scene(clwh_ctx *ctx, int32_t which, void *host_out, uint64_t capacity, int32_t info_out[4]) {
  if (!ctx || !info_out) return CLWH_ERR_INVALID_VALUE;
  if (which != CLWH_SCENE_HIT_RECORDS && which != CLWH_SCENE_STEP_BYTES && which != CLWH_SCENE_BRICK_MIN) return CLWH_ERR_INVALID_VALUE;
  if (!ctx->scene) return CLWH_ERR_BAD_ARGS;
  const PackedLayout L = scene_layout(ctx);
  info_out[0] = L.NBX; info_out[1] = L.NBY; info_out[2] = L.NBZ; info_out[3] = 0;
  if (!host_out) return CLWH_OK;
  const size_t offset = which == CLWH_SCENE_HIT_RECORDS ? 0u : (which == CLWH_SCENE_STEP_BYTES ? L.off_stepb : L.off_brick_min);
  const size_t bytes = which == CLWH_SCENE_HIT_RECORDS ? L.records * sizeof(uint2) : (which == CLWH_SCENE_STEP_BYTES ? L.records : L.n_bricks * sizeof(uint32_t));
  if (capacity < bytes || ctx->scene->data.bytes != L.bytes) return CLWH_ERR_SIZE_MISMATCH;
  HIP_TRY(hipSetDevice(ctx->device));
  HIP_TRY(hipMemcpyAsync(host_out, ctx->scene->data.as<uint8_t>() + offset, bytes, hipMemcpyDeviceToHost, ctx->stream));
  HIP_TRY(hipStreamSynchronize(ctx->stream));
  return CLWH_OK;
}

int clwh_debug_view_data(clwh_ctx *ctx, int32_t which, void *host_out, uint64_t capacity, int32_t info_out[4]) {
  if (!ctx || !info_out) return CLWH_ERR_INVALID_VALUE;
  if (which != CLWH_VIEW_BRICKS && which != CLWH_VIEW_TABLE && which != CLWH_VIEW_DILATED && which != CLWH_VIEW_COARSE) return CLWH_ERR_INVALID_VALUE;
  const ProjectionData &p = ctx->proj;
  if (!p.valid) return CLWH_ERR_BAD_ARGS;
  const size_t NBX = (p.dims[0] + 7) / 8, NBY = (p.dims[1] + 7) / 8, NBZ = (p.dims[2] + 7) / 8;
  const size_t n_bricks = NBX * NBY * NBZ, n_cells = ((NBX + 3) / 4) * ((NBY + 3) / 4) * ((NBZ + 3) / 4);
  info_out[0] = (int32_t)NBX; info_out[1] = (int32_t)NBY; info_out[2] = (int32_t)NBZ; info_out[3] = (int32_t)n_cells;
  const bool second_level = which == CLWH_VIEW_DILATED || which == CLWH_VIEW_COARSE;
  if (second_level && !p.dilated_valid) return CLWH_ERR_BAD_ARGS;
  if (!host_out) return CLWH_OK;
  const size_t off_table = n_bricks * 512u * sizeof(int16_t);
  const DeviceBuffer &from = second_level ? p.dilated : p.data;
  const size_t offset = which == CLWH_VIEW_TABLE ? off_table : (which == CLWH_VIEW_COARSE ? n_bricks * sizeof(uint32_t) : 0u);
  const size_t bytes = which == CLWH_VIEW_BRICKS ? off_table : (which == CLWH_VIEW_COARSE ? n_cells : n_bricks) * sizeof(uint32_t);
  if (capacity < bytes || from.bytes < offset + bytes) return CLWH_ERR_SIZE_MISMATCH;
  HIP_TRY(hipSetDevice(ctx->device));
  HIP_TRY(hipMemcpyAsync(host_out, from.as<uint8_t>() + offset, bytes, hipMemcpyDeviceToHost, ctx->stream));
  HIP_TRY(hipStreamSynchronize(ctx->stream));
  return CLWH_OK;
}

int clwh_debug_start_table(clwh_ctx *ctx, void *host_out, uint64_t capacity, int32_t info_out[4]) {
  if (!ctx || !info_out) return CLWH_ERR_INVALID_VALUE;
  if (!ctx->scene) return CLWH_ERR_BAD_ARGS;
  const PackedLayout L = scene_layout(ctx);
  info_out[0] = L.X; info_out[1] = L.Y; info_out[2] = L.Z; info_out[3] = L.start_table ? 1 : 0;
  if (!host_out || !L.start_table) return CLWH_OK;
  const size_t bytes = (size_t)L.X * L.Y * L.Z;
  if (capacity < bytes || ctx->scene->data.bytes != L.bytes) return CLWH_ERR_SIZE_MISMATCH;
  HIP_TRY(hipSetDevice(ctx->device));
  HIP_TRY(hipMemcpyAsync(host_out, ctx->scene->data.as<uint8_t>() + L.off_start + 16u, bytes, hipMemcpyDeviceToHost, ctx->stream));
  HIP_TRY(hipStreamSynchronize(ctx->stream));
  return CLWH_OK;
}

int clwh_debug_start_cert_dmin(int32_t X, int32_t Y, int32_t Z, float *dmin_out) {
  if (!dmin_out || X < 1 || Y < 1 || Z < 1) return CLWH_ERR_INVALID_VALUE;
  *dmin_out = start_cert_dmin(X, Y, Z);
  return CLWH_OK;
}

int clwh_debug_hull_table(clwh_ctx *ctx, void *host_out, uint64_t capacity, int32_t info_out[4]) {
  if (!ctx || !info_out) return CLWH_ERR_INVALID_VALUE;
  if (!ctx->scene) return CLWH_ERR_BAD_ARGS;
  const PackedLayout L = scene_layout(ctx);
  info_out[0] = kHullGrid; info_out[1] = kHullPlanes; info_out[2] = 0; info_out[3] = L.hull_table ? 1 : 0;
  if (!host_out || !L.hull_table) return CLWH_OK;
  const size_t bytes = (size_t)kHullPlanes * sizeof(float4);
  if (capacity < bytes || ctx->scene->data.bytes != L.bytes) return CLWH_ERR_SIZE_MISMATCH;
  HIP_TRY(hipSetDevice(ctx->device));
  HIP_TRY(hipMemcpyAsync(host_out, ctx->scene->data.as<uint8_t>() + L.off_hull, bytes, hipMemcpyDeviceToHost, ctx->stream));
  HIP_TRY(hipStreamSynchronize(ctx->stream));
  return CLWH_OK;
}

int clwh_debug_hull_cert_bound(int32_t X, int32_t Y, int32_t Z, float out[2]) {
  if (!out || X < 1 || Y < 1 || Z < 1) return CLWH_ERR_INVALID_VALUE;
  out[0] = hull_cert_delta0(X, Y, Z);
  out[1] = kHullSlack;
  return CLWH_OK;
}

int clwh_debug_hull_defer_bound(int32_t X, int32_t Y, int32_t Z, float out[4]) {
  if (!out || X < 1 || Y < 1 || Z < 1) return CLWH_ERR_INVALID_VALUE;
  out[0] = hull_defer_delta0(X, Y, Z);
  out[1] = (float)kHullDeferSteps;
  out[2] = kHullDeferDeficit;
  out[3] = (float)kHullMarginScale;
  return CLWH_OK;
}

int clwh_debug_hull_planes(clwh_ctx *ctx, void *host_out, uint64_t capacity, uint32_t *n_hits_out) {
  if (!ctx || !n_hits_out) return CLWH_ERR_INVALID_VALUE;
  PrimaryHits &p = ctx->primary;
  if (!p.valid || !p.hits.ptr || !ctx->pass.counters.ptr) return CLWH_ERR_BAD_ARGS;
  HIP_TRY(hipSetDevice(ctx->device));
  HIP_TRY(hipMemcpyAsync(n_hits_out, ctx->pass.counters.as<uint32_t>() + CTR_HITS, sizeof(uint32_t), hipMemcpyDeviceToHost, ctx->stream));
  HIP_TRY(hipStreamSynchronize(ctx->stream));
  if (!host_out) return CLWH_OK;
  const bool built = ctx->scene && ctx->scene->hull_table && ctx->tune.hull_defer != 0 && p.hull_planes.ptr;
  const size_t bytes = (size_t)*n_hits_out * sizeof(uint32_t);
  if (capacity < bytes || (built && p.hull_planes.bytes < bytes)) return CLWH_ERR_SIZE_MISMATCH;
  if (!built) { std::memset(host_out, 0, bytes); return CLWH_OK;}
  HIP_TRY(hipMemcpyAsync(host_out, p.hull_planes.ptr, bytes, hipMemcpyDeviceToHost, ctx->stream));
  HIP_TRY(hipStreamSynchronize(ctx->stream));
  return CLWH_OK;
}

int clwh_debug_hull_codes(clwh_ctx *ctx, void *host_out, uint64_t capacity, uint32_t *n_hits_out) {
  if (!ctx || !n_hits_out) return CLWH_ERR_INVALID_VALUE;
  PrimaryHits &p = ctx->primary;
  if (!p.valid || !p.hits.ptr || !ctx->pass.counters.ptr) return CLWH_ERR_BAD_ARGS;
  HIP_TRY(hipSetDevice(ctx->device));
  HIP_TRY(hipMemcpyAsync(n_hits_out, ctx->pass.counters.as<uint32_t>() + CTR_HITS, sizeof(uint32_t), hipMemcpyDeviceToHost, ctx->stream));
  HIP_TRY(hipStreamSynchronize(ctx->stream));
  if (!host_out) return CLWH_OK;
  const bool built = ctx->scene && ctx->scene->hull_table && p.hull_codes.ptr;
  const size_t bytes = (size_t)*n_hits_out * sizeof(uint32_t);
  if (capacity < bytes || (built && p.hull_codes.bytes < bytes)) return CLWH_ERR_SIZE_MISMATCH;
  if (!built) { std::memset(host_out, 0, bytes); return CLWH_OK; }
  HIP_TRY(hipMemcpyAsync(host_out, p.hull_codes.ptr, bytes, hipMemcpyDeviceToHost, ctx->stream));
  HIP_TRY(hipStreamSynchronize(ctx->stream));
  return CLWH_OK;
}

int clwh_debug_hit_records(clwh_ctx *ctx, void *host_out, uint64_t capacity, uint32_t *n_hits_out) {
  if (!ctx || !n_hits_out) return CLWH_ERR_INVALID_VALUE;
  PrimaryHits &p = ctx->primary;
  if (!p.valid || !p.hits.ptr || !ctx->pass.counters.ptr) return CLWH_ERR_BAD_ARGS;
  HIP_TRY(hipSetDevice(ctx->device));
  HIP_TRY(hipMemcpyAsync(n_hits_out, ctx->pass.counters.as<uint32_t>() + CTR_HITS, sizeof(uint32_t), hipMemcpyDeviceToHost, ctx->stream));
  HIP_TRY(hipStreamSynchronize(ctx->stream));
  if (!host_out) return CLWH_OK;
  const size_t bytes = (size_t)*n_hits_out * sizeof(HitRec);
  if (capacity < bytes || p.hits.bytes < bytes) return CLWH_ERR_SIZE_MISMATCH;
  HIP_TRY(hipMemcpyAsync(host_out, p.hits.ptr, bytes, hipMemcpyDeviceToHost, ctx->stream));
  HIP_TRY(hipStreamSynchronize(ctx->stream));
  return CLWH_OK;
}

}
```

cl_volume_renderer_amd/csrc/primary_kernels.hip:

```cpp
#include "bounce_device.hpp"

namespace clvr {

template <bool USE_GRAD>
__global__ __launch_bounds__(64) void k_primary(const RenderArgs a) {
  const uint32_t slot = xcd_contiguous_slot(blockIdx.x, a.num_tile_slots);
  int tx, ty;
  if (!tile_from_slot(a, slot, tx, ty)) return;
  const uint32_t lane = threadIdx.x;
  const uint32_t x = (uint32_t)tx * 8u + (lane & 7u);
  const uint32_t y = (uint32_t)ty * 8u + (lane >> 3);
  const uint32_t pslot = slot * 64u + lane;

  const VolumePacked vol = make_volume(a);
  const f3 cam_o = f3{a.cam_pos[0], a.cam_pos[1], a.cam_pos[2]};
  const f3 cam_d = f3{a.cam_dir[0], a.cam_dir[1], a.cam_dir[2]};
  const Ray vray = generate_ray(cam_o, cam_d, (int)x, (int)y, a.frame_w, a.frame_h);
  const float dx = (float)a.X, dy = (float)a.Y, dz = (float)a.Z;

  bool cut_ok;
  f3 cut_point;
  if (!(within(vray.origin.x, dx) && within(vray.origin.y, dy) && within(vray.origin.z, dz))) {
    cut_ok = cut_box(dx, dy, dz, vray, cut_point);
  } else {
    cut_ok = true;
    cut_point = vray.origin;
  }

  bool hit = false;
  Ray current_ray{cut_point, vray.direction};
  uint32_t current_color = 0u;
  if (cut_ok) {
    int ev;
    current_ray = march_to_next_event<USE_GRAD>(vol, a.tf, current_ray, ev, current_color);
    hit = (ev == EV_HIT);
  }

  const unsigned long long hit_mask = __ballot(hit);
  uint32_t base = 0u;
  if (hit_mask != 0ull) {
    const int leader = __ffsll((long long)hit_mask) - 1;
    if ((int)lane == leader) base = atomicAdd(&a.counters[CTR_HITS], (uint32_t)__popcll(hit_mask));
    base = __shfl(base, leader);
  }

  constexpr int kHullCoarse = kHullGrid / 4;
  __shared__ float4 hull_coarse[kHullCoarse * kHullCoarse];
  if (a.hull != nullptr && hit_mask != 0ull) {
    for (int c = (int)lane; c < kHullCoarse * kHullCoarse; c += 64)
      hull_coarse[c] = a.hull[((c / kHullCoarse) * 4 + 2) * kHullGrid + (c % kHullCoarse) * 4 + 2];
    __syncthreads();
  }

  int64_t raw_entry = -1;
  if (hit) {
    const uint32_t h = base + prefix_count(hit_mask);
    const f3 normal = -normalize3(gradient_nn(vol, current_ray.origin));
    raw_entry = cache_entry_of(a.X, a.Z, current_ray.origin);
    int64_t entry = raw_entry;
    if (a.mode == CLWH_ACCUM_VOXEL_CACHE && !(entry >= 0 && entry < a.cache_entries)) entry = -2;
    uint4 q0, q1, q2, q3;
    q0.x = __float_as_uint(current_ray.origin.x); q0.y = __float_as_uint(current_ray.origin.y);
    q0.z = __float_as_uint(current_ray.origin.z); q0.w = __float_as_uint(current_ray.direction.x);
    q1.x = __float_as_uint(current_ray.direction.y); q1.y = __float_as_uint(current_ray.direction.z);
    q1.z = __float_as_uint(normal.x); q1.w = __float_as_uint(normal.y);
    q2.x = __float_as_uint(normal.z); q2.y = current_color;
    q2.z = (uint32_t)((uint64_t)entry & 0xFFFFFFFFull); q2.w = (uint32_t)((uint64_t)entry >> 32);
    uint32_t start_free = 0u;
    if (a.start_free) {
      const f3 p = (current_ray.origin + current_ray.direction) + normal * 2.0f;
      if (__float_as_uint(p.x) < __float_as_uint(dx) && __float_as_uint(p.y) < __float_as_uint(dy) && __float_as_uint(p.z) < __float_as_uint(dz))
        start_free = a.start_free[((size_t)(int)p.z * (size_t)a.Y + (size_t)(int)p.y) * (size_t)a.X + (size_t)(int)p.x];
    }
    if (a.hull) {
      const f3 p = (current_ray.origin + current_ray.direction) + normal * 2.0f;
      float best = -INFINITY;
      int bc = 0;
#pragma unroll 4
      for (int c = 0; c < kHullCoarse * kHullCoarse; ++c) {
        const float4 e = hull_coarse[c];
        const float m = ((e.x * p.x + e.y * p.y) + e.z * p.z) - e.w;
        if (m > best) { best = m; bc = c; }
      }
      int bi = (bc % kHullCoarse) * 4 + 2, bj = (bc / kHullCoarse) * 4 + 2;
      uint32_t code = 0u;
      float margin = best;
      const int i0 = bi, j0 = bj;
#pragma unroll 1
      for (int dj = -3; dj <= 3; ++dj)
        for (int di = -3; di <= 3; ++di) {
          const int i = min(max(i0 + di, 0), kHullGrid - 1), j = min(max(j0 + dj, 0), kHullGrid - 1);
          const float4 e = a.hull[j * kHullGrid + i];
          const float m = ((e.x * p.x + e.y * p.y) + e.z * p.z) - e.w;
          if (m >= margin) { margin = m; bi = i; bj = j; }
        }
      if (margin >= 0.0f) code = ((uint32_t)(bj * kHullGrid + bi) + 1u) | ((uint32_t)fminf(floorf(margin * 256.0f), 65535.0f) << 16);
      a.hull_codes[h] = code;
      if (a.hull_planes) {
        uint32_t word = 0u;
        if (margin >= -kHullDeferDeficit) {
          const int q = (int)fminf(floorf(margin * (float)kHullMarginScale), 127.0f);
          word = ((uint32_t)(bj * kHullGrid + bi) + 1u) | (((uint32_t)q & 0xFFu) << 16);
        }
        a.hull_planes[h] = word;
      }
    }
    q3.x = x | (y << 16); q3.y = pslot; q3.z = start_free; q3.w = 0u;
    uint4 *dst = reinterpret_cast<uint4 *>(&a.hits[h]);
    dst[0] = q0; dst[1] = q1; dst[2] = q2; dst[3] = q3;
    a.pix_slot[pslot] = PIX_HIT | h;
  } else {
    const uint32_t e = sample_environment_map(a.env, a.env_w, a.env_h, vray.direction);
    a.pix_slot[pslot] = e & 0x00FFFFFFu;
  }
  if (a.hit_index_out) a.hit_index_out[(size_t)y * (size_t)a.launch_w + x] = raw_entry;
}

template <bool USE_GRAD>
__global__ __launch_bounds__(256) void k_ao(const RenderArgs a) {
  const uint32_t n_hits = a.n_hits_on_device ? a.counters[CTR_HITS] : a.n_hits;
  const uint32_t h = blockIdx.x * blockDim.x + threadIdx.x;
  if (h >= n_hits) return;
  const VolumePacked vol = make_volume(a);
  const uint4 *src = reinterpret_cast<const uint4 *>(&a.hits[h]);
  const uint4 q0 = src[0], q1 = src[1], q2 = src[2], q3 = src[3];
  const f3 hit_origin = f3{__uint_as_float(q0.x), __uint_as_float(q0.y), __uint_as_float(q0.z)};
  const f3 hit_direction = f3{__uint_as_float(q0.w), __uint_as_float(q1.x), __uint_as_float(q1.y)};
  const f3 normal = f3{__uint_as_float(q1.z), __uint_as_float(q1.w), __uint_as_float(q2.x)};
  const int64_t entry = (int64_t)(((uint64_t)q2.w << 32) | (uint64_t)q2.z);
  const uint32_t gx = q3.x & 0xFFFFu, gy = q3.x >> 16;
  if (entry < 0) return;
  uint32_t *word = a.cache + entry;
  for (int s = 0; s < a.n_seeds; ++s) {
    const uint32_t old = atomicAdd(word, 1u);
    uint32_t granted = 1u, occluded = 0u;
    if ((old & 0xFFFFu) >= 100u) {
      atomicSub(word, 1u);
      granted = 0u;
    } else {
      Ray r{hit_origin + hit_direction, hemisphere_direction(gx, gy, normal, a.seeds[s])};
      for (int k = 0; k < 7; ++k) {
        const int sd = (int)(vol.step_i(f2i(r.origin.x), f2i(r.origin.y), f2i(r.origin.z)) & 0x7Fu);
        r.origin = r.origin + r.direction * cl_max((float)sd, 0.5f);
      }
      int ev;
      uint32_t color = 0u;
      march_to_next_event<USE_GRAD>(vol, a.tf, r, ev, color);
      if (ev == EV_HIT) {
        atomicAdd(word, 0x10000u);
        occluded = 1u;
      }
    }
    if (a.contrib_out) {
      uint32_t *q = a.contrib_out + ((size_t)gy * (size_t)a.launch_w + gx) * 4;
      q[0] = occluded; q[1] = 0u; q[2] = 0u; q[3] = granted;
    }
  }
}

hipError_t launch_primary(const RenderArgs &a, hipStream_t s) {
  if (a.tf.uses_gradient)
    hipLaunchKernelGGL(k_primary<true>, dim3(a.num_tile_slots), dim3(64), 0, s, a);
  else
    hipLaunchKernelGGL(k_primary<false>, dim3(a.num_tile_slots), dim3(64), 0, s, a);
  return hipGetLastError();
}
hipError_t launch_ao(const RenderArgs &a, hipStream_t s) {
  if (a.n_hits == 0) return hipSuccess;
  const dim3 grid((a.n_hits + 255u) / 256u), block(256);
  if (a.tf.uses_gradient) hipLaunchKernelGGL(k_ao<true>, grid, block, 0, s, a);
  else hipLaunchKernelGGL(k_ao<false>, grid, block, 0, s, a);
  return hipGetLastError();
}

}
```

cl_volume_renderer_amd/csrc/render_kernels.hip:

```cpp
#include <algorithm>

#include "bounce_two_rays.hpp"

namespace clvr {

#ifndef CLVR_CERT_PHASE_MIN_LANES
#define CLVR_CERT_PHASE_MIN_LANES 16
#endif
constexpr int kCertPhaseMinLanes = CLVR_CERT_PHASE_MIN_LANES;
#ifndef CLVR_BOUNCE_WAVES_PER_SIMD
#define CLVR_BOUNCE_WAVES_PER_SIMD 7
#endif
#ifndef CLVR_BOUNCE_THREADS
#define CLVR_BOUNCE_THREADS 256
#endif
constexpr int kBounceThreads = CLVR_BOUNCE_THREADS;

template <bool USE_GRAD, int MODE, bool SMALL_VOLUME>
__global__ __launch_bounds__(kBounceThreads, CLVR_BOUNCE_WAVES_PER_SIMD) void k_bounce(const RenderArgs a) {
  constexpr int SMALL = SMALL_VOLUME ? 2 : 0;
  VolumePacked vol = make_volume(a);
  index_tables_to_lds<SMALL>(vol, a, kBounceThreads);
  __shared__ float div255[256];
  if (threadIdx.x < 256u) div255[threadIdx.x] = (float)threadIdx.x / 255.0f;
  __syncthreads();
  const uint32_t n_hits = a.n_hits_on_device ? a.counters[CTR_HITS] : a.n_hits;
  const uint32_t n_chunks = (n_hits + 63u) >> 6;
  const unsigned lane = lane_id();
  const unsigned home_queue = home_queue_of(a, (unsigned)(kBounceThreads / 64));
  unsigned queue_dry = 0u;
  enum : int { C_START_X, C_START_Y, C_START_Z,
               C_NORMAL_X, C_NORMAL_Y, C_NORMAL_Z,
               C_ENTRY_LO,
               C_ENTRY_HI,
               C_PIXEL, C_HIT, C_SEED,
               C_FIX,
               C_BV_R, C_BV_G, C_BV_B, C_FIELDS };
  __shared__ uint32_t cold[C_FIELDS][kBounceThreads];
#define COLD(f) cold[f][threadIdx.x]
#define COLD_ENTRY_HI() ((uint32_t)((int32_t)(COLD(C_ENTRY_HI) << (32 - entry_hi_bits)) >> (32 - entry_hi_bits)))
  Ray ray{{0, 0, 0}, {0, 0, 0}};
  float atten = 0.0f, r_energy = 0.0f, g_energy = 0.0f, b_energy = 0.0f;
  uint32_t color = 0u;
  int o = 0, i = 0;
  int st = ST_IDLE;
  int sd = 0;
  uint32_t march = 0u;
  constexpr uint32_t kOneStep = 1u << 24, kCertReady = 1u << 23, kArmed = 1u << 31;
  const bool cert_hint = a.cert_hint != 0;
  const int cert_min_lanes = a.cert_min_lanes;
  const int cert_at = a.cert_min_step != 0 ? a.cert_min_step : kCertNever;
  const bool start_cert = !USE_GRAD && a.cert_min_step != 0;
  const bool hull_cert = start_cert && a.hull_codes != nullptr;
  const bool hull_defer = hull_cert && a.hull_planes != nullptr;
  const int entry_hi_bits = hull_defer ? 3 : 8;
  const uint32_t *hull_words = hull_defer ? a.hull_planes : a.hull_codes;
  bool exhausted = false;
  BounceStats stats;

  for (;;) {
    if (__ballot(st == ST_MARCH) != 0ull) {
      do {
        stats.step(st);
        if (st == ST_MARCH) {
          ray.origin = ray.origin + ray.direction * fmaxf((float)sd, 0.5f);
          march += (uint32_t)sd - kOneStep;
          if (!USE_GRAD) {
            const bool has_voxel = __float_as_uint(ray.origin.x) < __float_as_uint((float)a.X) &&
                                   __float_as_uint(ray.origin.y) < __float_as_uint((float)a.Y) &&
                                   __float_as_uint(ray.origin.z) < __float_as_uint((float)a.Z);
            if (has_voxel) {
              const unsigned q = vol.template step_marched<SMALL>(ray.origin.x, ray.origin.y, ray.origin.z);
              sd = (int)(q & 0x7Fu);
              if (q & 0x80u) st = ST_EVENT + EV_HIT_COLOR_PENDING;
              else if ((march & ~kArmed) < kOneStep) st = ST_EVENT + EV_NONE;
              else if (((march & kArmed) | (uint32_t)sd) >= (uint32_t)cert_at && (march & kCertReady)) st = ST_CERT;
            } else {
              st = ST_EVENT + EV_CHECK;
            }
          } else if (exited_volume(vol, ray.origin)) {
            st = ST_EVENT + EV_EXIT;
          } else {
            int next_sd;
            bool pending = false;
            const bool is_hit = classify_step<USE_GRAD, SMALL, true>(vol, a.tf, ray.origin, color, next_sd, &pending);
            if (is_hit) {
              st = ST_EVENT + (pending ? EV_HIT_COLOR_PENDING : EV_HIT);
            } else if (march < kOneStep) {
              st = ST_EVENT + EV_NONE;
            } else {
              sd = next_sd;
              if (sd >= cert_at && (march & kCertReady)) st = ST_CERT;
            }
          }
        }
        const int n_cert = __popcll(__ballot(st == ST_CERT));
        if (n_cert != 0 && (n_cert >= cert_min_lanes || __popcll(__ballot(st == ST_MARCH)) < a.step_min_lanes)) {
          stats.cert_begin(st, n_cert);
          const bool fired = !USE_GRAD && st == ST_CERT && (march & kArmed) != 0u && (march & ~kArmed) >= (uint32_t)(70 - kHullDeferSteps) * kOneStep;
          stats.hull_fired(fired, i == 8);
          if (st == ST_CERT) {
            if (!USE_GRAD) march &= ~kArmed;
            int away;
            if (fired && !kStartCertVerify) {
              st = ST_EVENT + EV_EXIT;
            } else if (certify_exit(a, ray.origin, ray.direction, (int)(march >> 24), away)) {
              st = ST_EVENT + EV_EXIT;
            } else {
              march = (march & ~(kOneStep - 1u)) | (kCertReady - (uint32_t)(cert_hint ? away : 0));
              st = ST_MARCH;
            }
          }
          stats.cert_end(st, n_cert);
        }
      } while (__popcll(__ballot(st == ST_MARCH)) >= a.step_min_lanes);
    }

    stats.closing_half(st);
    if (st >= ST_EVENT) {
      int ev = st - ST_EVENT;
      if (ev == EV_CHECK) {
        for (;;) {
          if (exited_volume(vol, ray.origin)) { ev = EV_EXIT; break; }
          int next_sd;
          bool pending = false;
          if (classify_step<USE_GRAD, SMALL, true>(vol, a.tf, ray.origin, color, next_sd, &pending)) {
            ev = pending ? EV_HIT_COLOR_PENDING : EV_HIT;
            break;
          }
          if ((march & ~kArmed) < kOneStep) { ev = EV_NONE; break; }
          ray.origin = ray.origin + ray.direction * fmaxf((float)next_sd, 0.5f);
          march -= kOneStep;
        }
      }
      stats.march_end(a.counters, ev);
      bool ended = false;

      if (ev == EV_EXIT) {
        const float factor = i == 8 ? 8.0f / 8.0f : (i == 9 ? 8.0f / 9.0f : (i == 10 ? 8.0f / 10.0f : 8.0f / (float)i));
        const float p_r = atten * r_energy, p_g = atten * g_energy, p_b = atten * b_energy;
        uint32_t light = 0u;
        const uint32_t fix_word = COLD(C_FIX);
        int fix = (int)(fix_word >> 2) - 2, npend = (int)(fix_word & 3u);
        bool certain = (fix == -1) && sample_environment_map_fast(a.env, a.env_w, a.env_h, ray.direction, light);
        if (certain) {
          COLD(C_BV_R) = f2u((float)COLD(C_BV_R) + p_r * (float)(light & 255u) * factor / 1.0f);
          COLD(C_BV_G) = f2u((float)COLD(C_BV_G) + p_g * (float)((light >> 8) & 255u) * factor / 1.0f);
          COLD(C_BV_B) = f2u((float)COLD(C_BV_B) + p_b * (float)((light >> 16) & 255u) * factor / 1.0f);
        } else {
          if (fix == -1) {
            const uint32_t slot = atomicAdd(&a.counters[CTR_FIXUPS], 1u);
            if (slot < a.fixup_capacity) {
              fix = (int)slot;
              uint32_t *rec = a.fixups + (size_t)slot * kFixupDwords;
              rec[0] = COLD(C_HIT);
              rec[1] = COLD(C_ENTRY_LO);
              rec[2] = COLD_ENTRY_HI();
              rec[3] = COLD(C_PIXEL);
              rec[4] = COLD(C_BV_R); rec[5] = COLD(C_BV_G); rec[6] = COLD(C_BV_B);
            } else {
              a.sticky_flags[0] = 1u;
              fix = -2;
            }
          }
          if (fix >= 0) {
            uint32_t *e = a.fixups + (size_t)fix * kFixupDwords + 8 + 7 * npend;
            e[0] = __float_as_uint(p_r); e[1] = __float_as_uint(p_g); e[2] = __float_as_uint(p_b);
            e[3] = __float_as_uint(factor);
            e[4] = __float_as_uint(ray.direction.x); e[5] = __float_as_uint(ray.direction.y);
            e[6] = __float_as_uint(ray.direction.z);
            npend += 1;
          }
          COLD(C_FIX) = ((uint32_t)(fix + 2) << 2) | (uint32_t)npend;
        }
        o += 1;
        ev = EV_START;
        ended = true;
      } else if (ev == EV_HIT || ev == EV_HIT_COLOR_PENDING) {
        i += 1;
        if (i > 10) {
          o += 1;
          ended = true;
        }
      } else if (ev == EV_NONE) {
        i += 1;
        if (i > 10) {
          o += 1;
          ev = EV_START;
          ended = true;
        }
      }

      if (ended && o > 2) {
        const int fix = (int)(COLD(C_FIX) >> 2) - 2;
        if (fix == -1)
          finish_item<MODE>(a, (int64_t)(((uint64_t)COLD_ENTRY_HI() << 32) | (uint64_t)COLD(C_ENTRY_LO)), COLD(C_HIT), COLD(C_PIXEL) & 0xFFFFu,
                            COLD(C_PIXEL) >> 16, COLD(C_BV_R), COLD(C_BV_G), COLD(C_BV_B));
        else if (fix >= 0) a.fixups[(size_t)fix * kFixupDwords + 7] = COLD(C_FIX) & 3u;
        st = ST_IDLE;
      } else {
        st = ST_EVENT + ev;
      }
    }

    const unsigned long long idle_mask = __ballot(st == ST_IDLE);
    const uint32_t n_idle = (uint32_t)__popcll(idle_mask);
    if (!exhausted && n_idle >= (uint32_t)a.refill_min_lanes) {
      const uint32_t NQ = (uint32_t)a.unit_queues, S = (uint32_t)a.n_seeds, G = (uint32_t)a.unit_group;
      const uint32_t KB = (uint32_t)a.unit_block_log2, n_blocks = (n_chunks + (1u << KB) - 1u) >> KB;
      uint32_t base = 0u, count = 0u, q_sel = 0u;
      if (lane == 0u) {
        for (uint32_t tries = 0; tries < NQ && count == 0u; ++tries) {
          const uint32_t q = (home_queue + tries) % NQ;
          const uint32_t blocks_q = (n_blocks + NQ - 1u - q) / NQ;
          const uint32_t chunks_q = blocks_q << KB;
          if (chunks_q == 0u || ((queue_dry >> q) & 1u)) continue;
          const uint32_t total = chunks_q * S * 64u;
          const uint32_t p = atomicAdd(&a.counters[CTR_QUEUE_STRIDE * (q + 1u)], n_idle);
          if (p + n_idle >= total) queue_dry |= 1u << q;
          if (p < total) {
            base = p;
            count = min(n_idle, total - p);
            q_sel = q;
          }
        }
      }
      base = __shfl(base, 0);
      count = __shfl(count, 0);
      q_sel = __shfl(q_sel, 0);
      stats.refill(count);
      if (count == 0u) {
        exhausted = true;
      } else if (st == ST_IDLE) {
        const uint32_t rank = (uint32_t)__popcll(idle_mask & ((1ull << lane) - 1ull));
        if (rank < count) {
          const uint32_t item = base + rank, p = item >> 6;
          const uint32_t chunks_q = ((n_blocks + NQ - 1u - q_sel) / NQ) << KB;
          uint32_t r, c_in;
          const uint32_t g = udivmod24(p, G * S, r);
          const uint32_t in_group = min(G, chunks_q - g * G);
          const uint32_t s = udivmod24(r, in_group, c_in), ch = g * G + c_in;
          const uint32_t chunk = ((q_sel + NQ * (ch >> KB)) << KB) + (ch & ((1u << KB) - 1u));
          const uint32_t h = chunk * 64u + (item & 63u);
          if (h < n_hits) {
            const uint4 *src = reinterpret_cast<const uint4 *>(&a.hits[h]);
            const uint4 q0 = src[0], q1 = src[1], q2 = src[2], q3 = src[3];
            const f3 hit_origin = f3{__uint_as_float(q0.x), __uint_as_float(q0.y), __uint_as_float(q0.z)};
            const f3 hit_direction = f3{__uint_as_float(q0.w), __uint_as_float(q1.x), __uint_as_float(q1.y)};
            const f3 start = hit_origin + hit_direction;
            color = q2.y;
            const int64_t entry = (int64_t)(((uint64_t)q2.w << 32) | (uint64_t)q2.z);
            bool granted = true;
            if (MODE == CLWH_ACCUM_VOXEL_CACHE)
              granted = a.grants ? s < a.grants[h] : (entry >= 0 && cache_take_token(a.cache, entry, 256u));
            if (granted) {
              COLD(C_START_X) = __float_as_uint(start.x); COLD(C_START_Y) = __float_as_uint(start.y); COLD(C_START_Z) = __float_as_uint(start.z);
              COLD(C_NORMAL_X) = q1.z; COLD(C_NORMAL_Y) = q1.w; COLD(C_NORMAL_Z) = q2.x;
              COLD(C_ENTRY_LO) = q2.z;
              const uint32_t plane = hull_cert ? hull_words[h] : 0u;
              COLD(C_ENTRY_HI) = (q2.w & ((1u << entry_hi_bits) - 1u)) | ((plane & 0x1FFFu) << entry_hi_bits) | (plane & (hull_defer ? 0x00FF0000u : 0u)) | (q3.z << 24);
              COLD(C_PIXEL) = q3.x;
              COLD(C_HIT) = h;
              COLD(C_SEED) = (uint32_t)a.seeds[s];
              COLD(C_FIX) = (uint32_t)(-1 + 2) << 2;
              COLD(C_BV_R) = 0u; COLD(C_BV_G) = 0u; COLD(C_BV_B) = 0u;
              r_energy = div255[color & 255u];
              g_energy = div255[(color >> 8) & 255u];
              b_energy = div255[(color >> 16) & 255u];
              o = 1;
              st = ST_EVENT + EV_START;
            } else if (a.contrib_out) {
              uint32_t *q = a.contrib_out + ((size_t)(q3.x >> 16) * (size_t)a.launch_w + (q3.x & 0xFFFFu)) * 4;
              q[0] = 0u; q[1] = 0u; q[2] = 0u; q[3] = 0u;
            }
          }
        }
      }
    }
    stats.fresh_items(st, o);
    if (__ballot(st != ST_IDLE) == 0ull) {
      if (exhausted && lane == 0u) stats.flush<false>(a.counters);
      if (exhausted) break;
      continue;
    }

    bool sc_tried = false, sc_granted = false;
    bool hc_tried = false, hc_granted = false;
    bool rb_tried = false, rb_granted = false;
    uint32_t armed_path = 0u;
    if (st >= ST_EVENT) {
      const int ev = st - ST_EVENT;
      bool start_path = (ev == EV_START);
      bool bounce = false, from_hit = false;
      f3 bn{0, 0, 0}, bstart{0, 0, 0};
      int bseed = 0;

      if (ev == EV_HIT || ev == EV_HIT_COLOR_PENDING) {
        bn = -normalize3(hit_gradient_and_color<SMALL>(vol, a.tf, ray.origin, ev == EV_HIT_COLOR_PENDING, color));
        bstart = ray.origin + ray.direction;
        bseed = o + i - 1;
        bounce = true;
        from_hit = true;
        if (i > 10) {
          r_energy *= div255[color & 255u];
          g_energy *= div255[(color >> 8) & 255u];
          b_energy *= div255[(color >> 16) & 255u];
          bounce = false;
          start_path = true;
        }
      }

      if (start_path) {
        bn = f3{__uint_as_float(COLD(C_NORMAL_X)), __uint_as_float(COLD(C_NORMAL_Y)), __uint_as_float(COLD(C_NORMAL_Z))};
        bstart = f3{__uint_as_float(COLD(C_START_X)), __uint_as_float(COLD(C_START_Y)), __uint_as_float(COLD(C_START_Z))};
        bseed = o;
        bounce = true;
        from_hit = false;
      }

      if (bounce) {
        const float roughness = div255[color >> 24];
        const uint32_t pixel = COLD(C_PIXEL);
        Ray nr;
        nr.direction = hemisphere_reflective(pixel & 0xFFFFu, pixel >> 16, bn, (int)COLD(C_SEED) + bseed, roughness);
        nr.origin = bstart + bn * 2.0f;
        const float d = fabsf(dot3(nr.direction, bn));
        if (from_hit) {
          atten *= d;
          r_energy *= div255[color & 255u];
          g_energy *= div255[(color >> 8) & 255u];
          b_energy *= div255[(color >> 16) & 255u];
        } else {
          atten = d;
          i = 8;
          if (start_cert) {
            sc_tried = true;
            const uint32_t word = COLD(C_ENTRY_HI);
            sc_granted = start_certificate(word >> 24, nr.direction, a.start_cert_dmin);
          }
        }
        if (hull_cert && (hull_defer || !from_hit)) {
          const uint32_t word = COLD(C_ENTRY_HI);
          const uint32_t code = (word >> entry_hi_bits) & 0x1FFFu;
          const f3 n = hull_direction(code - 1u);
          const float dn = dot3(nr.direction, n);
          const f3 dir = nr.direction;
          const bool dir_ok = fminf(fminf(fabsf(dir.x), fabsf(dir.y)), fabsf(dir.z)) >= 0.0009765625f && (dir.x + dir.y) + dir.z == (dir.x + dir.y) + dir.z;
          float m = hull_defer ? (float)((int32_t)(word << 8) >> 24) * (1.0f / (float)kHullMarginScale) : 0.0f;
          if (from_hit) {
            const f3 p = f3{__uint_as_float(COLD(C_START_X)), __uint_as_float(COLD(C_START_Y)), __uint_as_float(COLD(C_START_Z))} +
                         f3{__uint_as_float(COLD(C_NORMAL_X)), __uint_as_float(COLD(C_NORMAL_Y)), __uint_as_float(COLD(C_NORMAL_Z))} * 2.0f;
            m = m + dot3(n, f3{nr.origin.x - p.x, nr.origin.y - p.y, nr.origin.z - p.z});
          }
          const bool tried = code != 0u, granted = tried && dir_ok && m >= 0.0f && dn >= a.hull_delta0;
          if (from_hit) { rb_tried = tried; rb_granted = granted; }
          else { hc_tried = tried && m >= 0.0f; hc_granted = granted; }
          if (tried && dir_ok && !sc_granted && m < 0.0f && m >= -kHullDeferDeficit && dn >= a.hull_defer_delta0)
            armed_path = (uint32_t)ceilf(-m * __builtin_amdgcn_rcpf(dn) * (1.0f + 0x1p-19f));
        }
        ray = nr;
      }

      if ((sc_granted || hc_granted || rb_granted) && !kStartCertVerify) {
        st = ST_EVENT + EV_EXIT;
      } else {
        sd = (int)(vol.template step_i<SMALL>(f2i(ray.origin.x), f2i(ray.origin.y), f2i(ray.origin.z)) & 0x7Fu);
        march = 70u * kOneStep + kCertReady;
        if (armed_path != 0u) march = kArmed + 70u * kOneStep + kCertReady - armed_path;
        st = ST_MARCH;
      }
    }
    stats.start_cert(sc_tried, sc_granted);
    stats.hull_cert(hc_tried, hc_granted, hc_granted && sc_granted);
    stats.hull_more(rb_tried, rb_granted, armed_path != 0u && st == ST_MARCH, i == 8);
  }
#undef COLD_ENTRY_HI
#undef COLD
}

hipError_t launch_bounce(const RenderArgs &a_in, hipStream_t s) {
  RenderArgs a = a_in;
  const uint64_t total = (uint64_t)a.n_hits * (uint64_t)a.n_seeds;
  if (total == 0) return hipSuccess;
  const uint64_t waves_needed = (total + 63u) / 64u;
  constexpr unsigned wpb = (unsigned)kBounceThreads / 64u;
  const unsigned blocks = (unsigned)std::min<uint64_t>((waves_needed + wpb - 1u) / wpb, ((uint64_t)a.bounce_max_blocks * 4u + wpb - 1u) / wpb);
  const dim3 grid(blocks), block(kBounceThreads);
  const uint64_t waves_likely = ((uint64_t)a.n_hits_estimate * (uint64_t)a.n_seeds + 63u) / 64u;
  const bool long_launch = a.force_long_launch || waves_likely >= 6u * (uint64_t)blocks * wpb;
  if (a.step_min_lanes <= 0) a.step_min_lanes = long_launch ? 16 : 1;
  if (a.refill_min_lanes <= 0) a.refill_min_lanes = long_launch ? 16 : 64;
  a.cert_min_lanes = kCertPhaseMinLanes;
  if (!long_launch) a.cert_min_step = 0;
  if (!bounce_queues_fit(a.n_hits, a.unit_block_log2, a.n_seeds)) return hipErrorInvalidValue;
  const bool g = a.tf.uses_gradient != 0;
  const bool small = (uint64_t)a.NBX * (uint64_t)a.NBY * (uint64_t)((a.Z + 7) / 8) < (1ull << 23) &&
                     a.X + a.Y + a.Z <= VolumePacked::kPartsMaxEntries;
  const size_t lds_parts_bytes = small ? (size_t)(a.X + a.Y + a.Z) * sizeof(uint32_t) : 0u;
  const bool two_rays = a.bounce_rays == 2 && long_launch && a.n_hits < (1u << 26) && kBounceThreads == 256;
  if (two_rays) a.fixup_capacity = std::min<uint32_t>(a.fixup_capacity, (1u << 27) - 4u);
#define CLVR_LAUNCH_BOUNCE(G, M)                                                                    \
  do {                                                                                              \
    if (two_rays) {                                                                                 \
      if (small) hipLaunchKernelGGL((k_bounce2<G, M, true>), grid, block, lds_parts_bytes, s, a);  \
      else hipLaunchKernelGGL((k_bounce2<G, M, false>), grid, block, 0, s, a);                     \
    } else if (small) hipLaunchKernelGGL((k_bounce<G, M, true>), grid, block, lds_parts_bytes, s, a); \
    else hipLaunchKernelGGL((k_bounce<G, M, false>), grid, block, 0, s, a);                        \
  } while (0)
  if (a.mode == CLWH_ACCUM_VOXEL_CACHE) {
    if (g) CLVR_LAUNCH_BOUNCE(true, CLWH_ACCUM_VOXEL_CACHE);
    else CLVR_LAUNCH_BOUNCE(false, CLWH_ACCUM_VOXEL_CACHE);
  } else {
    if (g) CLVR_LAUNCH_BOUNCE(true, CLWH_ACCUM_IMAGE_SPACE);
    else CLVR_LAUNCH_BOUNCE(false, CLWH_ACCUM_IMAGE_SPACE);
  }
#undef CLVR_LAUNCH_BOUNCE
  return hipGetLastError();
}

}
```

cl_volume_renderer_amd/ffi.py:

```python
from __future__ import annotations

import ctypes as C
import os

import numpy as np

_HERE = os.path.dirname(os.path.abspath(__file__))
LIB_PATH = os.environ.get("CLWH_LIBRARY") or os.path.join(_HERE, "libclwhip.so")

OK = 0
ELEM_S8, ELEM_S16, ELEM_S32, ELEM_U8, ELEM_U16, ELEM_U32, ELEM_F32 = range(7)
ARG_MEM, ARG_I32, ARG_U32, ARG_F32, ARG_I64, ARG_U64, ARG_F64 = range(7)
ACCUM_VOXEL_CACHE, ACCUM_IMAGE_SPACE = 0, 1
DERIVED_SCENE, DERIVED_CAMERA, DERIVED_PROJECTION = 1, 2, 4
PROJ_MAX, PROJ_MIN, PROJ_MEAN = 0, 1, 2
PROJ_DENSE = 1
COMP_DENSE, COMP_SHADE = 1, 2
ISO_DENSE, ISO_BELOW = 1, 2
SLICE_MAX, SLICE_MIN, SLICE_MEAN = 0, 1, 2
SLICE_DENSE = 1
MESH_DENSE, MESH_BELOW = 1, 2
GROW_26, GROW_FROM_MASK, GROW_DENSE = 1, 2, 4
GROW_MAX_SEEDS = 65536
LABEL_26, LABEL_FROM_MASK = 1, 2
# ... 223 lines not shown
        ("result", C.POINTER(GeodesicResult)),
    ]


class GeodesicTraceDesc(C.Structure):
    _fields_ = [
        ("dist", C.c_void_p), ("labels", C.c_void_p), ("points", C.c_void_p), ("capacity", C.c_uint64),
        ("dims", C.c_uint32 * 3), ("weight_face", C.c_uint32 * 3), ("weight_edge", C.c_uint32 * 3), ("weight_corner", C.c_uint32),
        ("flags", C.c_int32), ("target", C.c_uint32 * 3),
        ("n_points", C.POINTER(C.c_uint64)),
    ]


assert C.sizeof(GeodesicDesc) == 104 and C.sizeof(GeodesicTraceDesc) == 96 and C.sizeof(GeodesicResult) == 16


class MaskCombineDesc(C.Structure):
    _fields_ = [("a", C.c_void_p), ("b", C.c_void_p), ("out", C.c_void_p), ("dims", C.c_uint32 * 3), ("op", C.c_int32)]


class RegionStats(C.Structure):
    _fields_ = [
        ("count", C.c_uint64), ("sum", C.c_int64), ("sum_sq", C.c_uint64),
        ("vmin", C.c_int32), ("vmax", C.c_int32),
        ("sum_pos", C.c_uint64 * 3),
        ("bbox_lo", C.c_uint32 * 3), ("bbox_hi", C.c_uint32 * 3),
        ("faces", C.c_uint32 * 3), ("border_faces", C.c_uint32 * 3),
    ]

    def as_dict(self):
        return {"count": int(self.count), "sum": int(self.sum), "sum_sq": int(self.sum_sq), "vmin": int(self.vmin), "vmax": int(self.vmax),
                "sum_pos": tuple(int(v) for v in self.sum_pos), "bbox_lo": tuple(self.bbox_lo), "bbox_hi": tuple(self.bbox_hi),
                "faces": tuple(self.faces), "border_faces": tuple(self.border_faces)}


REGION_STATS_DTYPE = np.dtype([("count", np.uint64), ("sum", np.int64), ("sum_sq", np.uint64), ("vmin", np.int32), ("vmax", np.int32),
                               ("sum_pos", np.uint64, (3,)), ("bbox_lo", np.uint32, (3,)), ("bbox_hi", np.uint32, (3,)),
                               ("faces", np.uint32, (3,)), ("border_faces", np.uint32, (3,))])
assert REGION_STATS_DTYPE.itemsize == C.sizeof(RegionStats) == 104
LABEL_STATS_MAX_CAPACITY = 1 << 24


class MaskStatsResult(C.Structure):
    _fields_ = [("stats", RegionStats), ("hist_below", C.c_uint64), ("hist_above", C.c_uint64)]


class MaskStatsDesc(C.Structure):
    _fields_ = [("volume", C.c_void_p), ("mask", C.c_void_p), ("hist", C.c_void_p), ("hist_lo", C.c_int32), ("bin_width", C.c_int32),
                ("n_bins", C.c_int32), ("flags", C.c_int32), ("result", C.POINTER(MaskStatsResult))]


class LabelStatsDesc(C.Structure):
    _fields_ = [("volume", C.c_void_p), ("labels", C.c_void_p), ("stats", C.c_void_p), ("capacity", C.c_uint64), ("flags", C.c_int32),
                ("reserved", C.c_int32)]


class OverlayRegion(C.Structure):
    _fields_ = [("buffer", C.c_void_p), ("kind", C.c_int32), ("dims", C.c_uint32 * 3), ("id_lo", C.c_uint32), ("id_hi", C.c_uint32)]


class OverlayPaint(C.Structure):
    _fields_ = [("palette", C.c_void_p), ("n_colours", C.c_uint32), ("flags", C.c_int32), ("fill_alpha", C.c_uint32),
                ("outline_alpha", C.c_uint32), ("ids", C.c_void_p), ("t_first", C.c_void_p)]


class OverlaySliceDesc(C.Structure):
    _fields_ = [
        ("frame", C.c_void_p), ("region", OverlayRegion), ("paint", OverlayPaint),
        ("origin", C.c_float * 3), ("du", C.c_float * 3), ("dv", C.c_float * 3), ("normal", C.c_float * 3),
        ("width", C.c_uint32), ("height", C.c_uint32),
        ("slab_samples", C.c_int32), ("step", C.c_float),
    ]


class OverlayCameraDesc(C.Structure):
    _fields_ = [
        ("frame", C.c_void_p), ("region", OverlayRegion), ("paint", OverlayPaint),
        ("cam_pos", C.c_float * 3), ("cam_dir", C.c_float * 3),
        ("width", C.c_uint32), ("height", C.c_uint32),
        ("step", C.c_float), ("t_near", C.c_float), ("t_far", C.c_float), ("reserved", C.c_int32),
    ]


_SIZE3 = C.POINTER(C.c_size_t)
_PROTOTYPES = [
    ("clwh_ctx_create", C.c_int, [C.c_int, C.POINTER(C.c_void_p)]),
    ("clwh_ctx_create_on_stream", C.c_int, [C.c_int, C.c_void_p, C.POINTER(C.c_void_p)]),
    ("clwh_ctx_destroy", C.c_int, [C.c_void_p]),
    ("clwh_ctx_finish", C.c_int, [C.c_void_p]),
    ("clwh_ctx_stream", C.c_void_p, [C.c_void_p]),
    ("clwh_ctx_device", C.c_int, [C.c_void_p]),
    ("clwh_mem_create", C.c_int, [C.c_void_p, C.c_size_t, C.c_int, C.POINTER(C.c_void_p)]),
    ("clwh_mem_wrap", C.c_int, [C.c_void_p, C.c_void_p, C.c_size_t, C.POINTER(C.c_void_p)]),
    ("clwh_image_create", C.c_int, [C.c_void_p, _SIZE3, C.c_int, C.c_int, C.c_int, C.POINTER(C.c_void_p)]),
    ("clwh_image_wrap", C.c_int, [C.c_void_p, C.c_void_p, _SIZE3, C.c_int, C.c_int, C.POINTER(C.c_void_p)]),
    ("clwh_mem_push", C.c_int, [C.c_void_p, C.c_void_p, C.c_void_p, C.c_size_t]),
    ("clwh_mem_pull", C.c_int, [C.c_void_p, C.c_void_p, C.c_void_p, C.c_size_t]),
    ("clwh_mem_release", C.c_int, [C.c_void_p]),
    ("clwh_host_register", C.c_int, [C.c_void_p, C.c_size_t]),
    ("clwh_host_unregister", C.c_int, [C.c_void_p]),
    ("clwh_mem_device_ptr", C.c_void_p, [C.c_void_p]),
    ("clwh_mem_size", C.c_size_t, [C.c_void_p]),
    ("clwh_mem_mark_dirty", C.c_int, [C.c_void_p]),
    ("clwh_kernel_get", C.c_int, [C.c_void_p, C.c_char_p, C.c_char_p, C.c_char_p, C.POINTER(C.c_void_p)]),
    ("clwh_kernel_release", C.c_int, [C.c_void_p]),
    ("clwh_launch", C.c_int, [C.c_void_p, _SIZE3, _SIZE3, C.POINTER(Arg), C.c_int]),
    ("clwh_render", C.c_int, [C.c_void_p, C.POINTER(RenderDesc)]),
    ("clwh_cache_len", C.c_int64, [C.c_uint32, C.c_uint32, C.c_uint32]),
    ("clwh_accum_len", C.c_int64, [C.c_uint32, C.c_uint32, C.c_int32]),
    ("clwh_accum_resolve", C.c_int, [C.c_void_p, C.c_void_p, C.c_int32, C.c_uint32, C.c_uint32, C.c_void_p,
                                     C.c_void_p, C.POINTER(C.c_float), C.POINTER(C.c_float)]),
    ("clwh_accum_resolve_tiles", C.c_int, [C.c_void_p, C.c_void_p, C.c_int32, C.c_int32, C.c_uint32, C.c_uint32, C.c_void_p,
                                           C.c_void_p, C.POINTER(C.c_float), C.POINTER(C.c_float)]),
    ("clwh_frame_from_tiles", C.c_int, [C.c_void_p, C.c_void_p, C.c_int32, C.c_uint32, C.c_uint32, C.c_void_p]),
    ("clwh_ctx_invalidate_derived", C.c_int, [C.c_void_p, C.c_int]),
    ("clwh_ctx_scene_info", C.c_int, [C.c_void_p, C.POINTER(C.c_uint64), C.POINTER(C.c_uint64), C.POINTER(C.c_int32)]),
    ("clwh_render_projection", C.c_int, [C.c_void_p, C.POINTER(ProjectionDesc)]),
    ("clwh_render_composite", C.c_int, [C.c_void_p, C.POINTER(CompositeDesc)]),
    ("clwh_render_isosurface", C.c_int, [C.c_void_p, C.POINTER(IsosurfaceDesc)]),
    ("clwh_render_slice", C.c_int, [C.c_void_p, C.POINTER(SliceDesc)]),
    ("clwh_mesh_isosurface", C.c_int, [C.c_void_p, C.POINTER(MeshDesc)]),
    ("clwh_segment_grow", C.c_int, [C.c_void_p, C.POINTER(GrowDesc)]),
    ("clwh_volume_apply_mask", C.c_int, [C.c_void_p, C.POINTER(ApplyMaskDesc)]),
    ("clwh_segment_label", C.c_int, [C.c_void_p, C.POINTER(LabelDesc)]),
    ("clwh_labels_to_mask", C.c_int, [C.c_void_p, C.POINTER(LabelsToMaskDesc)]),
    ("clwh_mask_distance", C.c_int, [C.c_void_p, C.POINTER(DistanceDesc)]),
    ("clwh_mask_morph", C.c_int, [C.c_void_p, C.POINTER(MorphDesc)]),
    ("clwh_mask_combine", C.c_int, [C.c_void_p, C.POINTER(MaskCombineDesc)]),
    ("clwh_mask_geodesic", C.c_int, [C.c_void_p, C.POINTER(GeodesicDesc)]),
    ("clwh_geodesic_trace", C.c_int, [C.c_void_p, C.POINTER(GeodesicTraceDesc)]),
    ("clwh_mask_statistics", C.c_int, [C.c_void_p, C.POINTER(MaskStatsDesc)]),
    ("clwh_label_statistics", C.c_int, [C.c_void_p, C.POINTER(LabelStatsDesc)]),
    ("clwh_overlay_slice", C.c_int, [C.c_void_p, C.POINTER(OverlaySliceDesc)]),
    ("clwh_overlay_camera", C.c_int, [C.c_void_p, C.POINTER(OverlayCameraDesc)]),
    ("clwh_sdf_build", C.c_int, [C.c_void_p, C.c_void_p, C.c_char_p, C.c_void_p, C.POINTER(C.c_int32)]),
    ("clwh_buffer_reset", C.c_int, [C.c_void_p, C.c_void_p]),
    ("clwh_cache_exchange_plan", C.c_int, [C.c_void_p, C.c_void_p, C.c_uint64, C.POINTER(C.c_void_p)]),
    ("clwh_cache_apply_contributions", C.c_int, [C.c_void_p, C.c_void_p, C.c_void_p, C.c_void_p, C.c_int32]),
    ("clwh_cache_exchange_plan_release", C.c_int, [C.c_void_p]),
    ("clwh_tf_parse", C.c_int, [C.c_char_p, C.POINTER(Tf)]),
    ("clwh_debug_float_conversions", C.c_int, [C.c_void_p, C.c_void_p, C.c_uint64, C.c_void_p, C.c_void_p]),
    ("clwh_debug_wave_min", C.c_int, [C.c_void_p, C.c_void_p, C.c_uint64, C.c_void_p]),
    ("clwh_debug_device_probe", C.c_int, [C.c_void_p, C.c_int32, C.c_void_p, C.c_uint64, C.c_void_p, C.c_void_p, C.POINTER(C.c_int32)]),
    ("clwh_debug_macro_table", C.c_int, [C.c_void_p, C.c_void_p, C.c_uint64, C.POINTER(C.c_int32)]),
    ("clwh_debug_packed_scene", C.c_int, [C.c_void_p, C.c_int32, C.c_void_p, C.c_uint64, C.POINTER(C.c_int32)]),
    ("clwh_debug_view_data", C.c_int, [C.c_void_p, C.c_int32, C.c_void_p, C.c_uint64, C.POINTER(C.c_int32)]),
    ("clwh_debug_start_table", C.c_int, [C.c_void_p, C.c_void_p, C.c_uint64, C.POINTER(C.c_int32)]),
    ("clwh_debug_start_cert_dmin", C.c_int, [C.c_int32, C.c_int32, C.c_int32, C.POINTER(C.c_float)]),
    ("clwh_debug_hit_records", C.c_int, [C.c_void_p, C.c_void_p, C.c_uint64, C.POINTER(C.c_uint32)]),
    ("clwh_debug_hull_table", C.c_int, [C.c_void_p, C.c_void_p, C.c_uint64, C.POINTER(C.c_int32)]),
    ("clwh_debug_hull_cert_bound", C.c_int, [C.c_int32, C.c_int32, C.c_int32, C.POINTER(C.c_float)]),
    ("clwh_debug_hull_codes", C.c_int, [C.c_void_p, C.c_void_p, C.c_uint64, C.POINTER(C.c_uint32)]),
    ("clwh_debug_hull_planes", C.c_int, [C.c_void_p, C.c_void_p, C.c_uint64, C.POINTER(C.c_uint32)]),
    ("clwh_debug_hull_defer_bound", C.c_int, [C.c_int32, C.c_int32, C.c_int32, C.POINTER(C.c_float)]),
    ("clwh_strerror", C.c_char_p, [C.c_int]),
    ("clwh_last_hip_error", C.c_int, []),
    ("clwh_version", C.c_char_p, []),
    ("clwh_ctx_acquire_from", C.c_int, [C.c_void_p, C.c_void_p]),
    ("clwh_ctx_release_to", C.c_int, [C.c_void_p, C.c_void_p]),
    ("clwh_ctx_set_timing", C.c_int, [C.c_void_p, C.c_int]),
    ("clwh_ctx_timing_read", C.c_int, [C.c_void_p, C.POINTER(C.c_float), C.POINTER(C.c_int32)]),
    ("clwh_ctx_timing_read_all", C.c_int, [C.c_void_p, C.POINTER(C.c_float), C.POINTER(C.c_int32), C.c_int32]),
]
EXPORTED_SYMBOLS = [p[0] for p in _PROTOTYPES]

_lib = None


def lib():
    global _lib
    if _lib is None:
        if not os.path.exists(LIB_PATH):
            raise RuntimeError(
                "libclwhip.so is missing (%s): build it with `python -m cl_volume_renderer_amd.build`; "
                "there is no CPU fallback for the product path" % LIB_PATH)
        L = C.CDLL(LIB_PATH)
        for name, res, args in _PROTOTYPES:
            if not hasattr(L, name) and os.environ.get("CLWH_LIBRARY"):
                continue
            f = getattr(L, name)
            f.restype = res
            f.argtypes = args
        _lib = L
    return _lib


def _check(status, where):
    if status != OK:
        raise ClwhError(status, where)


def parse_tf(source: str) -> Tf:
    tf = Tf()
    _check(lib().clwh_tf_parse(source.encode(), C.byref(tf)), "clwh_tf_parse")
    return tf


def hull_cert_bound(X: int, Y: int, Z: int):
    v = (C.c_float * 2)()
    _check(lib().clwh_debug_hull_cert_bound(X, Y, Z, v), "clwh_debug_hull_cert_bound")
    return float(v[0]), float(v[1])


def hull_defer_bound(X: int, Y: int, Z: int):
    v = (C.c_float * 4)()
    _check(lib().clwh_debug_hull_defer_bound(X, Y, Z, v), "clwh_debug_hull_defer_bound")
    return float(v[0]), int(v[1]), float(v[2]), int(v[3])


def start_cert_dmin(X: int, Y: int, Z: int) -> float:
    v = C.c_float(0)
    _check(lib().clwh_debug_start_cert_dmin(X, Y, Z, C.byref(v)), "clwh_debug_start_cert_dmin")
    return float(v.value)


def cache_len(X, Y, Z) -> int:
    return int(lib().clwh_cache_len(X, Y, Z))


def accum_len(w, h, world=1) -> int:
    return int(lib().clwh_accum_len(w, h, world))


def _handle(mem):
    return mem.h if mem is not None else None


def _fill_overlay(d, frame, source, kind, dims, palette, width, height, n_colours, flags, fill_alpha, outline_alpha, id_range, ids, t_first):
    d.frame = _handle(frame)
    d.region.buffer, d.region.kind = _handle(source), int(kind)
    for k in range(3):
        d.region.dims[k] = int(dims[k])
    d.region.id_lo, d.region.id_hi = int(id_range[0]), int(id_range[1])
    d.paint.palette = _handle(palette)
    d.paint.n_colours = int(n_colours if n_colours is not None else (palette.nbytes // 4 if palette is not None else 0))
    d.paint.flags, d.paint.fill_alpha, d.paint.outline_alpha = int(flags), int(fill_alpha), int(outline_alpha)
    d.paint.ids, d.paint.t_first = _handle(ids), _handle(t_first)
    d.width, d.height = int(width), int(height)


def _fill_view(d, frame, volume, cam_pos, cam_dir, width, height):
    d.frame, d.volume = frame.h, volume.h
    for k in range(3):
        d.cam_pos[k] = float(cam_pos[k])
        d.cam_dir[k] = float(cam_dir[k])
    d.width, d.height = int(width), int(height)


class Mem:
    def __init__(self, ctx, handle, nbytes, dtype=None, shape=None):
        self.ctx, self.h, self.nbytes, self.dtype, self.shape = ctx, C.c_void_p(handle), nbytes, dtype, shape

    def push(self, arr: np.ndarray):
        a = np.ascontiguousarray(arr)
        _check(lib().clwh_mem_push(self.ctx.h, self.h, a.ctypes.data, a.nbytes), "clwh_mem_push")

    def pull(self, dtype=None, shape=None) -> np.ndarray:
        dtype = np.dtype(dtype or self.dtype or np.uint8)
        out = np.empty(self.nbytes // dtype.itemsize, dtype=dtype)
        _check(lib().clwh_mem_pull(self.ctx.h, self.h, out.ctypes.data, out.nbytes), "clwh_mem_pull")
        shape = shape or self.shape
        return out.reshape(shape) if shape else out

    @property
    def device_ptr(self) -> int:
        return int(lib().clwh_mem_device_ptr(self.h) or 0)

    def release(self):
        if self.h:
            _check(lib().clwh_mem_release(self.h), "clwh_mem_release")
            self.h = None


class Kernel:
    def __init__(self, ctx, handle):
        self.ctx, self.h = ctx, C.c_void_p(handle)

    def launch(self, global_size, local_size, *args):
        g = (C.c_size_t * 3)(*(list(global_size) + [0, 0, 0])[:3])
        l = (C.c_size_t * 3)(*(list(local_size) + [0, 0, 0])[:3])
        arr = (Arg * max(len(args), 1))()
        for i, a in enumerate(args):
            if isinstance(a, Mem):
                arr[i].kind, arr[i].v.mem = ARG_MEM, a.h.value
            elif isinstance(a, (float, np.floating)):
                arr[i].kind, arr[i].v.f32 = ARG_F32, float(a)
            elif isinstance(a, np.unsignedinteger):
                arr[i].kind, arr[i].v.u32 = ARG_U32, int(a)
            elif isinstance(a, (int, np.integer)):
                arr[i].kind, arr[i].v.i32 = ARG_I32, int(a)
            else:
                raise TypeError("unsupported kernel argument %r" % (a,))
        _check(lib().clwh_launch(self.h, g, l, arr, len(args)), "clwh_launch")

    def render(self, *, frame, volume, sdf, env, cam_pos, cam_dir, seed, width, height, buffer_volume=None,
               accum=None, mode=ACCUM_VOXEL_CACHE, tile_rank=0, tile_world=1, write_frame=True,
               hit_index=None, contrib=None, seeds=None, shading=SHADE_LIGHT, resolve_only=False):
        d = RenderDesc()
        d.frame = frame.h if frame is not None else None
        d.volume, d.sdf, d.env = volume.h, sdf.h, env.h
        d.buffer_volume = buffer_volume.h if buffer_volume is not None else None
        for k in range(3):
            d.cam_pos[k] = float(cam_pos[k])
            d.cam_dir[k] = float(cam_dir[k])
        d.seed, d.width, d.height = int(seed), int(width), int(height)
        d.accum_mode = mode
# ... 466 lines not shown
        d.capacity, d.flags = int(capacity), int(flags)
        for k in range(3):
            d.dims[k], d.target[k] = int(dims[k]), int(target[k])
        self._geodesic_weights(d, weights)
        if result:
            d.n_points = C.pointer(n)
        return lib().clwh_geodesic_trace(self.h, C.byref(d)), int(n.value)

    def geodesic_trace(self, dist: Mem, dims, target, labels: Mem = None, connectivity=6, weights=None, capacity=4096):
        if connectivity not in (6, 26):
            raise ValueError("connectivity is 6 or 26")
        capacity = int(capacity)
        buf = self.buffer(max(capacity, 1) * 12, np.uint32)
        try:
            status, n = self.geodesic_trace_raw(dist, dims, target, labels, GEO_26 if connectivity == 26 else 0, weights, buf, capacity)
            _check(status, "clwh_geodesic_trace")
            k = min(n, capacity)
            return (buf.pull(np.uint32)[:3 * k].reshape(k, 3).copy() if k else np.zeros((0, 3), np.uint32)), n
        finally:
            buf.release()

    def split_mask(self, volume: Mem, mask: Mem, dims, radius_sq, weights=(1, 1, 1), connectivity=6):
        eroded = self.mask_morph(mask, dims, MORPH_ERODE, radius_sq, weights)
        try:
            ranks, res, _ = self.label_components(volume, -32768, 32767, connectivity, mask=eroded, capacity=0)
        finally:
            eroded.release()
        n_parts = int(res.n_components)
        if n_parts == 0:
            return ranks, 0
        status, _ = self.mask_geodesic_raw(mask, dims, None, ranks, GEO_FROM_LABELS | (GEO_26 if connectivity == 26 else 0), labels=ranks)
        if status != OK:
            ranks.release()
        _check(status, "clwh_mask_geodesic")
        return ranks, n_parts

    def mask_statistics_raw(self, volume: Mem, mask: Mem, hist: Mem = None, hist_lo=0, bin_width=0, n_bins=0, flags=0, result=True):
        d, res = MaskStatsDesc(), MaskStatsResult()
        d.volume, d.mask, d.hist = _handle(volume), _handle(mask), _handle(hist)
        d.hist_lo, d.bin_width, d.n_bins, d.flags = int(hist_lo), int(bin_width), int(n_bins), int(flags)
        if result:
            d.result = C.pointer(res)
        return lib().clwh_mask_statistics(self.h, C.byref(d)), res

    def mask_statistics(self, volume: Mem, mask: Mem, hist=None):
        table = None
        try:
            if hist is not None:
                lo, width, n = (int(v) for v in hist)
                table = self.buffer(8 * max(n, 1), np.uint64, (max(n, 1),))
                status, res = self.mask_statistics_raw(volume, mask, table, lo, width, n)
            else:
                status, res = self.mask_statistics_raw(volume, mask)
            _check(status, "clwh_mask_statistics")
            counts = table.pull()[:int(hist[2])].copy() if table is not None else None
            return res.stats, counts, int(res.hist_below), int(res.hist_above)
        finally:
            if table is not None:
                table.release()

    def label_statistics_raw(self, volume: Mem, labels: Mem, stats: Mem, capacity, flags=0):
        d = LabelStatsDesc()
        d.volume, d.labels, d.stats = _handle(volume), _handle(labels), _handle(stats)
        d.capacity, d.flags = int(capacity), int(flags)
        return lib().clwh_label_statistics(self.h, C.byref(d))

    def label_statistics(self, volume: Mem, labels: Mem, capacity, stats: Mem = None) -> Mem:
        own = stats is None
        if own:
            stats = self.buffer(104 * max(int(capacity), 1), REGION_STATS_DTYPE, (max(int(capacity), 1),))
        status = self.label_statistics_raw(volume, labels, stats, capacity)
        if status != OK and own:
            stats.release()
        _check(status, "clwh_label_statistics")
        return stats

    def scene_info(self):
        sid, nb, holders = C.c_uint64(0), C.c_uint64(0), C.c_int32(0)
        _check(lib().clwh_ctx_scene_info(self.h, C.byref(sid), C.byref(nb), C.byref(holders)), "clwh_ctx_scene_info")
        return int(sid.value), int(nb.value), int(holders.value)

    def device_probe(self, which, records: np.ndarray, params=(0, 0, 0, 0), aux: np.ndarray = None) -> np.ndarray:
        w_in, w_out = PROBE_WORDS[which]
        rec = np.ascontiguousarray(records, dtype=np.uint32).reshape(-1, w_in)
        n = rec.shape[0]
        m_in, m_out = self.buffer_from(rec if n else np.zeros(1, np.uint32)), self.buffer(max(n, 1) * w_out * 4, np.uint32)
        m_aux = self.buffer_from(np.ascontiguousarray(aux, dtype=np.uint32)) if aux is not None else None
        try:
            _check(lib().clwh_debug_device_probe(self.h, which, m_in.h, C.c_uint64(n), m_out.h, m_aux.h if m_aux else None,
                                                 (C.c_int32 * 4)(*[int(v) for v in params])), "clwh_debug_device_probe")
            self.finish()
            return m_out.pull().reshape(-1, w_out)[:n]
        finally:
            for m in (m_in, m_out, m_aux):
                if m is not None:
                    m.release()

    def macro_table(self):
        info = (C.c_int32 * 4)()
        _check(lib().clwh_debug_macro_table(self.h, None, C.c_uint64(0), info), "clwh_debug_macro_table")
        out = np.empty((info[2], info[1], info[0], 8), np.uint8)
        _check(lib().clwh_debug_macro_table(self.h, out.ctypes.data_as(C.c_void_p), C.c_uint64(out.nbytes), info), "clwh_debug_macro_table")
        return out, int(info[3])

    def packed_scene(self, which):
        info = (C.c_int32 * 4)()
        _check(lib().clwh_debug_packed_scene(self.h, which, None, C.c_uint64(0), info), "clwh_debug_packed_scene")
        n = info[0] * info[1] * info[2]
        out = (np.empty((n, 512, 2), np.uint32) if which == SCENE_HIT_RECORDS else
               np.empty((n, 512), np.uint8) if which == SCENE_STEP_BYTES else np.empty(n, np.uint32))
        _check(lib().clwh_debug_packed_scene(self.h, which, out.ctypes.data_as(C.c_void_p), C.c_uint64(out.nbytes), info), "clwh_debug_packed_scene")
        return out, (int(info[0]), int(info[1]), int(info[2]))

    def view_data(self, which):
        info = (C.c_int32 * 4)()
        _check(lib().clwh_debug_view_data(self.h, which, None, C.c_uint64(0), info), "clwh_debug_view_data")
        n = info[0] * info[1] * info[2]
        out = np.empty((n, 512), np.int16) if which == VIEW_BRICKS else np.empty(info[3] if which == VIEW_COARSE else n, np.uint32)
        _check(lib().clwh_debug_view_data(self.h, which, out.ctypes.data_as(C.c_void_p), C.c_uint64(out.nbytes), info), "clwh_debug_view_data")
        return out, (int(info[0]), int(info[1]), int(info[2]))

    def start_table(self):
        info = (C.c_int32 * 4)()
        _check(lib().clwh_debug_start_table(self.h, None, C.c_uint64(0), info), "clwh_debug_start_table")
        if not info[3]:
            return None
        out = np.empty((info[2], info[1], info[0]), np.uint8)
        _check(lib().clwh_debug_start_table(self.h, out.ctypes.data_as(C.c_void_p), C.c_uint64(out.nbytes), info), "clwh_debug_start_table")
        return out

    def hull_table(self):
        info = (C.c_int32 * 4)()
        _check(lib().clwh_debug_hull_table(self.h, None, C.c_uint64(0), info), "clwh_debug_hull_table")
        if not info[3]:
            return None
        out = np.empty((info[1], 4), np.float32)
        _check(lib().clwh_debug_hull_table(self.h, out.ctypes.data_as(C.c_void_p), C.c_uint64(out.nbytes), info), "clwh_debug_hull_table")
        return out

    def hull_codes(self):
        n = C.c_uint32(0)
        _check(lib().clwh_debug_hull_codes(self.h, None, C.c_uint64(0), C.byref(n)), "clwh_debug_hull_codes")
        out = np.empty(int(n.value), np.uint32)
        _check(lib().clwh_debug_hull_codes(self.h, out.ctypes.data_as(C.c_void_p), C.c_uint64(out.nbytes), C.byref(n)), "clwh_debug_hull_codes")
        return out[:int(n.value)]

    def hull_planes(self):
        n = C.c_uint32(0)
        _check(lib().clwh_debug_hull_planes(self.h, None, C.c_uint64(0), C.byref(n)), "clwh_debug_hull_planes")
        out = np.empty(int(n.value), np.uint32)
        _check(lib().clwh_debug_hull_planes(self.h, out.ctypes.data_as(C.c_void_p), C.c_uint64(out.nbytes), C.byref(n)), "clwh_debug_hull_planes")
        return out[:int(n.value)]

    def hit_records(self):
        n = C.c_uint32(0)
        _check(lib().clwh_debug_hit_records(self.h, None, C.c_uint64(0), C.byref(n)), "clwh_debug_hit_records")
        out = np.empty((int(n.value), 16), np.uint32)
        _check(lib().clwh_debug_hit_records(self.h, out.ctypes.data_as(C.c_void_p), C.c_uint64(out.nbytes), C.byref(n)), "clwh_debug_hit_records")
        return out[:int(n.value)]

    def image_wrap(self, device_ptr: int, dims, channels, dtype, shape=None) -> Mem:
        dtype = np.dtype(dtype)
        d = (C.c_size_t * 3)(*(list(dims) + [1, 1, 1])[:3])
        h = C.c_void_p()
        _check(lib().clwh_image_wrap(self.h, C.c_void_p(device_ptr), d, channels, _ELEM_OF_DTYPE[dtype], C.byref(h)),
               "clwh_image_wrap")
        n = int(np.prod([max(int(x), 1) for x in list(dims)[:3]])) * channels * dtype.itemsize
        return Mem(self, h.value, n, dtype, shape)

    def acquire_from(self, stream: int):
        _check(lib().clwh_ctx_acquire_from(self.h, C.c_void_p(stream)), "clwh_ctx_acquire_from")

    def release_to(self, stream: int):
        _check(lib().clwh_ctx_release_to(self.h, C.c_void_p(stream)), "clwh_ctx_release_to")

    def finish(self):
        _check(lib().clwh_ctx_finish(self.h), "clwh_ctx_finish")

    def set_timing(self, enabled=True):
        _check(lib().clwh_ctx_set_timing(self.h, 1 if enabled else 0), "clwh_ctx_set_timing")

    def timing_read(self):
        ms, n = C.c_float(0), C.c_int32(0)
        _check(lib().clwh_ctx_timing_read(self.h, C.byref(ms), C.byref(n)), "clwh_ctx_timing_read")
        return float(ms.value), int(n.value)

    def timing_read_all(self):
        n = len(TIMERS)
        ms, cnt = (C.c_float * n)(), (C.c_int32 * n)()
        _check(lib().clwh_ctx_timing_read_all(self.h, ms, cnt, n), "clwh_ctx_timing_read_all")
        return {name: (float(ms[i]), int(cnt[i])) for i, name in enumerate(TIMERS)}

    @property
    def stream(self) -> int:
        return int(lib().clwh_ctx_stream(self.h) or 0)

    def destroy(self):
        if self.h:
            _check(lib().clwh_ctx_destroy(self.h), "clwh_ctx_destroy")
            self.h = None
```

include/clwh.h:

```cpp
#ifndef CLWH_H
#define CLWH_H

#include <stddef.h>
#include <stdint.h>

#ifdef __cplusplus
extern "C" {
#endif

typedef struct clwh_ctx clwh_ctx;
typedef struct clwh_mem clwh_mem;
typedef struct clwh_kernel clwh_kernel;

enum clwh_status {
  CLWH_OK = 0,
  CLWH_ERR_INVALID_VALUE = 1,
  CLWH_ERR_NO_DEVICE = 2,
  CLWH_ERR_OUT_OF_MEMORY = 3,
  CLWH_ERR_HIP = 4,
  CLWH_ERR_UNKNOWN_KERNEL = 5,
  CLWH_ERR_TF_UNSUPPORTED = 6,
  CLWH_ERR_BAD_ARGS = 7,
  CLWH_ERR_BAD_NDRANGE = 8,
  CLWH_ERR_SIZE_MISMATCH = 9,
// ... 328 lines not shown
int clwh_mask_geodesic(clwh_ctx *ctx, const clwh_geodesic_desc *desc);

typedef struct clwh_geodesic_trace_desc {
  clwh_mem *dist;
  clwh_mem *labels;
  clwh_mem *points;
  uint64_t capacity;
  uint32_t dims[3];
  uint32_t weight_face[3];
  uint32_t weight_edge[3];
  uint32_t weight_corner;
  int32_t flags;
  uint32_t target[3];
  uint64_t *n_points;
} clwh_geodesic_trace_desc;
int clwh_geodesic_trace(clwh_ctx *ctx, const clwh_geodesic_trace_desc *desc);

typedef struct clwh_region_stats {
  uint64_t count;
  int64_t sum;
  uint64_t sum_sq;
  int32_t vmin, vmax;
  uint64_t sum_pos[3];
  uint32_t bbox_lo[3], bbox_hi[3];
  uint32_t faces[3];
  uint32_t border_faces[3];
} clwh_region_stats;

typedef struct clwh_mask_stats_result {
  clwh_region_stats stats;
  uint64_t hist_below, hist_above;
} clwh_mask_stats_result;
typedef struct clwh_mask_stats_desc {
  clwh_mem *volume;
  clwh_mem *mask;
  clwh_mem *hist;
  int32_t hist_lo;
  int32_t bin_width;
  int32_t n_bins;
  int32_t flags;
  clwh_mask_stats_result *result;
} clwh_mask_stats_desc;
int clwh_mask_statistics(clwh_ctx *ctx, const clwh_mask_stats_desc *desc);

typedef struct clwh_label_stats_desc {
  clwh_mem *volume;
  clwh_mem *labels;
  clwh_mem *stats;
  uint64_t capacity;
  int32_t flags;
  int32_t reserved;
} clwh_label_stats_desc;
int clwh_label_statistics(clwh_ctx *ctx, const clwh_label_stats_desc *desc);

enum clwh_region_kind { CLWH_REGION_MASK = 0, CLWH_REGION_LABELS = 1 };
enum clwh_overlay_flags {
  CLWH_OVERLAY_FILL = 1,
  CLWH_OVERLAY_OUTLINE = 2,
  CLWH_OVERLAY_DENSE = 4
};
typedef struct clwh_overlay_region {
  clwh_mem *buffer;
  int32_t kind;
  uint32_t dims[3];
  uint32_t id_lo, id_hi;
} clwh_overlay_region;
typedef struct clwh_overlay_paint {
  clwh_mem *palette;
  uint32_t n_colours;
  int32_t flags;
  uint32_t fill_alpha, outline_alpha;
  clwh_mem *ids;
  clwh_mem *t_first;
} clwh_overlay_paint;
typedef struct clwh_overlay_slice_desc {
  clwh_mem *frame;
  clwh_overlay_region region;
  clwh_overlay_paint paint;
  float origin[3], du[3], dv[3], normal[3];
  uint32_t width, height;
  int32_t slab_samples;
  float step;
} clwh_overlay_slice_desc;
typedef struct clwh_overlay_camera_desc {
  clwh_mem *frame;
  clwh_overlay_region region;
  clwh_overlay_paint paint;
  float cam_pos[3], cam_dir[3];
  uint32_t width, height;
  float step;
  float t_near, t_far;
  int32_t reserved;
} clwh_overlay_camera_desc;
int clwh_overlay_slice(clwh_ctx *ctx, const clwh_overlay_slice_desc *desc);
int clwh_overlay_camera(clwh_ctx *ctx, const clwh_overlay_camera_desc *desc);

int clwh_sdf_build(clwh_ctx *ctx, clwh_mem *volume, const char *tf_source, clwh_mem *sdf,
                   int32_t *n_launches);

int clwh_buffer_reset(clwh_ctx *ctx, clwh_mem *buffer_volume);

typedef struct clwh_exchange_plan clwh_exchange_plan;
int clwh_cache_exchange_plan(clwh_ctx *ctx, clwh_mem *entries, uint64_t n, clwh_exchange_plan **out);
int clwh_cache_apply_contributions(clwh_ctx *ctx, clwh_exchange_plan *plan, clwh_mem *buffer_volume, clwh_mem *rgb,
                                   int32_t rgb_stride);
int clwh_cache_exchange_plan_release(clwh_exchange_plan *plan);

int clwh_ctx_acquire_from(clwh_ctx *ctx, void *hip_stream);
int clwh_ctx_release_to(clwh_ctx *ctx, void *hip_stream);

#define CLWH_TF_MAX_RULES 16
typedef struct clwh_tf_rule {
  int32_t v_lo, v_hi;
  int32_t g_lo, g_hi;
  int32_t use_gradient;
  int32_t writes_color;
  int32_t terminal;
  int32_t color[4];
} clwh_tf_rule;
typedef struct clwh_tf {
  int32_t n;
  clwh_tf_rule rules[CLWH_TF_MAX_RULES];
} clwh_tf;
int clwh_tf_parse(const char *source, clwh_tf *out);

int clwh_debug_float_conversions(clwh_ctx *ctx, clwh_mem *floats_in, uint64_t n, clwh_mem *i32_out, clwh_mem *u32_out);
int clwh_debug_wave_min(clwh_ctx *ctx, clwh_mem *u32_in, uint64_t n, clwh_mem *u32_out);
enum clwh_probe {
  CLWH_PROBE_ARITH = 0,
  CLWH_PROBE_HASH = 1,
  CLWH_PROBE_HEMISPHERE = 2,
  CLWH_PROBE_RAY = 3,
  CLWH_PROBE_CUT = 4,
  CLWH_PROBE_ENV_EXACT = 5,
  CLWH_PROBE_ENV_FAST = 6,
  CLWH_PROBE_ENV_APPROX = 7,
  CLWH_PROBE_TONE = 8,
  CLWH_PROBE_TAPS = 9,
  CLWH_PROBE_COUNT = 10
};
int clwh_debug_device_probe(clwh_ctx *ctx, int32_t which, clwh_mem *in, uint64_t n, clwh_mem *out, clwh_mem *aux, const int32_t params[4]);
int clwh_debug_macro_table(clwh_ctx *ctx, void *host_out, uint64_t capacity, int32_t info_out[4]);
enum clwh_scene_array { CLWH_SCENE_HIT_RECORDS = 0, CLWH_SCENE_STEP_BYTES = 1, CLWH_SCENE_BRICK_MIN = 2 };
int clwh_debug_packed_scene(clwh_ctx *ctx, int32_t which, void *host_out, uint64_t capacity, int32_t info_out[4]);
enum clwh_view_array { CLWH_VIEW_BRICKS = 0, CLWH_VIEW_TABLE = 1, CLWH_VIEW_DILATED = 2, CLWH_VIEW_COARSE = 3 };
int clwh_debug_view_data(clwh_ctx *ctx, int32_t which, void *host_out, uint64_t capacity, int32_t info_out[4]);
int clwh_debug_start_table(clwh_ctx *ctx, void *host_out, uint64_t capacity, int32_t info_out[4]);
int clwh_debug_start_cert_dmin(int32_t X, int32_t Y, int32_t Z, float *dmin_out);
int clwh_debug_hit_records(clwh_ctx *ctx, void *host_out, uint64_t capacity, uint32_t *n_hits_out);
int clwh_debug_hull_table(clwh_ctx *ctx, void *host_out, uint64_t capacity, int32_t info_out[4]);
int clwh_debug_hull_cert_bound(int32_t X, int32_t Y, int32_t Z, float out[2]);
int clwh_debug_hull_codes(clwh_ctx *ctx, void *host_out, uint64_t capacity, uint32_t *n_hits_out);
int clwh_debug_hull_planes(clwh_ctx *ctx, void *host_out, uint64_t capacity, uint32_t *n_hits_out);
int clwh_debug_hull_defer_bound(int32_t X, int32_t Y, int32_t Z, float out[4]);
const char *clwh_strerror(int status);
int clwh_last_hip_error(void);
const char *clwh_version(void);
int clwh_ctx_set_timing(clwh_ctx *ctx, int enabled);
int clwh_ctx_timing_read(clwh_ctx *ctx, float *total_ms, int32_t *launches);
enum clwh_timer {
  CLWH_TIMER_BOUNCE = 0,
  CLWH_TIMER_PRIMARY = 1,
  CLWH_TIMER_FIXUP = 2,
  CLWH_TIMER_RESOLVE = 3,
  CLWH_TIMER_REPACK = 4,
  CLWH_TIMER_AO = 5,
  CLWH_TIMER_COUNT = 6
};
int clwh_ctx_timing_read_all(clwh_ctx *ctx, float *ms, int32_t *launches, int32_t n);

#ifdef __cplusplus
}
#endif
#endif
```

Baseline: 46730.

## End bounce paths early when remaining energy cannot change quantized colour; add wide hull words

Adds a zero-contribution rule: at each bounce event, an upper bound on the remaining contribution (attenuation times max channel energy, scaled) is compared against a sub-quantum threshold, and the path is ended instead of marched further. It also adds a 'wide' hull word per primary hit holding a quantized margin, which rebounds read in place of the plane word, plus extra statistics and debug entry points. The intent is to skip marching work that cannot change the integer-accumulated output, at the cost of an extra per-hit buffer write and some extra per-event arithmetic. Correctness relies on the bound really being below one quantization step.

```diff
diff --git a/cl_volume_renderer_amd/csrc/bounce_device.hpp b/cl_volume_renderer_amd/csrc/bounce_device.hpp
--- a/cl_volume_renderer_amd/csrc/bounce_device.hpp
+++ b/cl_volume_renderer_amd/csrc/bounce_device.hpp
@@ -26,7 +26,8 @@
 enum : int { ST_IDLE = 0, ST_MARCH = 1, ST_CERT = 2, ST_EVENT = 8 };
 enum : int { EV_START = 3,
              EV_HIT_COLOR_PENDING = 4,
-             EV_CHECK = 5 };
+             EV_CHECK = 5,
+             EV_ZERO = 6 };
 constexpr int kCertNever = 255;
 
 template <int MODE>
@@ -121,6 +122,10 @@
   __device__ void hull_cert(bool, bool, bool) {}
   __device__ void hull_more(bool, bool, bool, bool) {}
   __device__ void hull_fired(bool, bool) {}
+  __device__ void zero_end(bool, bool, uint32_t, uint32_t, uint32_t) {}
+  __device__ void reach_init(const RenderArgs &) {}
+  __device__ void reach(const RenderArgs &, bool, float, f3, f3) {}
+  __device__ void ray_end(uint32_t *, bool, uint32_t, uint32_t, uint32_t) {}
   __device__ void march_end(uint32_t *, int) {}
   template <bool TWO_RAYS> __device__ void flush(uint32_t *) {}
 };
@@ -132,6 +137,7 @@
   uint32_t swaps = 0;
   uint32_t closing = 0, marching_before = 0;
   __device__ __forceinline__ void step(int st) {
+    reach_steps += (uint32_t)__popcll(__ballot(reach_open && st == ST_MARCH));
     step_iters += 1; step_lanes += (uint32_t)__popcll(__ballot(st == ST_MARCH));
     step_idle += (uint32_t)__popcll(__ballot(st == ST_IDLE));
   }
@@ -181,10 +187,54 @@
     more_granted[0] += (uint32_t)__popcll(__ballot(fired && first_leg)); more_granted[2] += (uint32_t)__popcll(__ballot(fired && !first_leg));
     if (fired) more_open = first_leg ? 0 : 2;
   }
+  uint32_t reach_tried = 0, reach_granted = 0, reach_steps = 0;
+  bool reach_open = false;
+  __device__ __forceinline__ float *reach_table() {
+    __shared__ float table[64];
+    return table;
+  }
+  __device__ __forceinline__ void reach_init(const RenderArgs &a) {
+    if (threadIdx.x < 64u) {
+      const int longest = a.X > a.Y ? (a.X > a.Z ? a.X : a.Z) : (a.Y > a.Z ? a.Y : a.Z);
+      const double cap = (double)(longest / 2 < 127 ? longest / 2 : 127), slope = (double)threadIdx.x / 64.0;
+      double t = 0.0;
+      for (int step = 0; step < 70 - 5; ++step) {
+        const double m = (double)(long long)(t * slope / 1.7320508075688772) - 2.0;
+        const double bound = m > cap ? cap : m;
+        t += bound < 1.0 ? 1.0 : bound;
+      }
+      reach_table()[threadIdx.x] = (float)t * (1.0f - 0x1p-20f);
+    }
+  }
+  __device__ __forceinline__ void reach(const RenderArgs &a, bool candidate, float dn, f3 p, f3 d) {
+    const bool tried = candidate && dn >= 0.0f && dn < a.hull_delta0 && dn < 1.0f;
+    bool granted = false;
+    if (tried) {
+      const float r = reach_table()[(int)(dn * 64.0f)];
+      const float fx = d.x < 0.0f ? p.x : (float)a.X - p.x, fy = d.y < 0.0f ? p.y : (float)a.Y - p.y, fz = d.z < 0.0f ? p.z : (float)a.Z - p.z;
+      granted = r * fabsf(d.x) >= fx + 1.0f || r * fabsf(d.y) >= fy + 1.0f || r * fabsf(d.z) >= fz + 1.0f;
+    }
+    reach_tried += (uint32_t)__popcll(__ballot(tried)); reach_granted += (uint32_t)__popcll(__ballot(granted));
+    reach_open = granted;
+  }
+  uint32_t zero_tried = 0, zero_granted = 0;
+  bool zero_open = false;
+  uint32_t zero_bv[3] = {0, 0, 0};
+  __device__ __forceinline__ void zero_end(bool tried, bool granted, uint32_t bv_r, uint32_t bv_g, uint32_t bv_b) {
+    zero_tried += (uint32_t)__popcll(__ballot(tried)); zero_granted += (uint32_t)__popcll(__ballot(granted && !zero_open));
+    if (granted && !zero_open) { zero_open = true; zero_bv[0] = bv_r; zero_bv[1] = bv_g; zero_bv[2] = bv_b; }
+  }
+  __device__ __forceinline__ void ray_end(uint32_t *counters, bool ended, uint32_t bv_r, uint32_t bv_g, uint32_t bv_b) {
+    if (ended && zero_open && (bv_r != zero_bv[0] || bv_g != zero_bv[1] || bv_b != zero_bv[2])) atomicAdd(&counters[CTR_ZERO_END + 2], 1u);
+    if (ended) zero_open = false;
+  }
   __device__ __forceinline__ void march_end(uint32_t *counters, int ev) {
-    if (start_open && ev != EV_EXIT) atomicAdd(&counters[CTR_START_WRONG], 1u);
-    if (hull_open && ev != EV_EXIT) atomicAdd(&counters[CTR_HULL_WRONG], 1u);
-    if (more_open >= 0 && ev != EV_EXIT) atomicAdd(&counters[CTR_HULL_DEFER + 3 * more_open + 2], 1u);
+    if (reach_open && ev != EV_EXIT) atomicAdd(&counters[CTR_REACH + 2], 1u);
+    reach_open = false;
+    const bool exit = ev == EV_EXIT || ev == EV_ZERO;
+    if (start_open && !exit) atomicAdd(&counters[CTR_START_WRONG], 1u);
+    if (hull_open && !exit) atomicAdd(&counters[CTR_HULL_WRONG], 1u);
+    if (more_open >= 0 && !exit) atomicAdd(&counters[CTR_HULL_DEFER + 3 * more_open + 2], 1u);
     start_open = false;
     hull_open = false;
     more_open = -1;
@@ -199,6 +249,8 @@
     atomicAdd(&counters[CTR_CERT_GRANTED], cert_granted); atomicAdd(&counters[CTR_STEP_IDLE], step_idle);
     atomicAdd(&counters[CTR_START_TRIED], start_tried); atomicAdd(&counters[CTR_START_GRANTED], start_granted);
     atomicAdd(&counters[CTR_HULL_TRIED], hull_tried); atomicAdd(&counters[CTR_HULL_GRANTED], hull_granted); atomicAdd(&counters[CTR_HULL_BOTH], hull_both);
+    atomicAdd(&counters[CTR_REACH], reach_tried); atomicAdd(&counters[CTR_REACH + 1], reach_granted); atomicAdd(&counters[CTR_REACH + 3], reach_steps);
+    atomicAdd(&counters[CTR_ZERO_END], zero_tried); atomicAdd(&counters[CTR_ZERO_END + 1], zero_granted);
     for (int k = 0; k < 3; ++k) { atomicAdd(&counters[CTR_HULL_DEFER + 3 * k], more_tried[k]); atomicAdd(&counters[CTR_HULL_DEFER + 3 * k + 1], more_granted[k]); }
   }
 };
diff --git a/cl_volume_renderer_amd/csrc/clwh_context.hip b/cl_volume_renderer_amd/csrc/clwh_context.hip
--- a/cl_volume_renderer_amd/csrc/clwh_context.hip
+++ b/cl_volume_renderer_amd/csrc/clwh_context.hip
@@ -156,6 +156,8 @@
   if (const char *e = std::getenv("CLWH_TUNE_START_CERT")) t.start_cert = std::atoi(e) != 0;
   if (const char *e = std::getenv("CLWH_TUNE_HULL_CERT")) t.hull_cert = std::atoi(e) != 0;
   if (const char *e = std::getenv("CLWH_TUNE_HULL_DEFER")) t.hull_defer = std::atoi(e) != 0;
+  if (const char *e = std::getenv("CLWH_TUNE_HULL_WIDE")) t.hull_wide = std::atoi(e) != 0;
+  if (const char *e = std::getenv("CLWH_TUNE_ZERO_END")) t.zero_end = std::atoi(e) != 0;
   return t;
 }
 
diff --git a/cl_volume_renderer_amd/csrc/clwh_host.hpp b/cl_volume_renderer_amd/csrc/clwh_host.hpp
--- a/cl_volume_renderer_amd/csrc/clwh_host.hpp
+++ b/cl_volume_renderer_amd/csrc/clwh_host.hpp
@@ -120,6 +120,8 @@
   int32_t start_cert = 1;
   int32_t hull_cert = 1;
   int32_t hull_defer = 1;
+  int32_t hull_wide = 1;
+  int32_t zero_end = 1;
   int32_t cert_min_step = -1;
   uint32_t bounce_max_blocks = 2048;
   int32_t sdfbit_waves = 8;
@@ -147,6 +149,7 @@
   DeviceBuffer pix_slot, hits;
   DeviceBuffer hull_codes;
   DeviceBuffer hull_planes;
+  DeviceBuffer hull_wide;
   uint32_t n_hits = 0;
   bool n_hits_known = false;
   PinnedWord host_n_hits;
@@ -157,8 +160,10 @@
 
 struct PassScratch {
   static constexpr size_t kCounters = CTR_QUEUE_STRIDE * 10;
+  static_assert(CTR_REACH_END <= kCounters, "the statistics fit their line");
   DeviceBuffer counters;
   DeviceBuffer fixups, delta;
+  int32_t zero_end_applied = -1;
   DeviceBuffer sticky_flags;
   bool fixup_overflow_pending = false;
 };
diff --git a/cl_volume_renderer_amd/csrc/clwh_internal.hpp b/cl_volume_renderer_amd/csrc/clwh_internal.hpp
--- a/cl_volume_renderer_amd/csrc/clwh_internal.hpp
+++ b/cl_volume_renderer_amd/csrc/clwh_internal.hpp
@@ -53,6 +53,8 @@
   CTR_STATS_END,
   CTR_QUEUE_STRIDE = 32,
   CTR_HULL_DEFER = CTR_QUEUE_STRIDE * 9, CTR_HULL_DEFER_END = CTR_HULL_DEFER + 9,
+  CTR_ZERO_END = CTR_HULL_DEFER_END, CTR_ZERO_END_END = CTR_ZERO_END + 3,
+  CTR_REACH = CTR_ZERO_END_END, CTR_REACH_END = CTR_REACH + 4,
 };
 struct RenderArgs {
   int32_t X, Y, Z;
@@ -72,6 +74,9 @@
   float hull_delta0;
   uint32_t *hull_planes;
   float hull_defer_delta0;
+  uint32_t *hull_wide;
+  const uint32_t *hull_bounce_words;
+  int32_t zero_end;
   int32_t NBX, NBY;
   const uint32_t *env;
   int32_t env_w, env_h;
@@ -210,10 +215,19 @@
   }
   return 2.0f;
 }
+constexpr float kZeroContribution = 1.0f - 0x1p-12f;
+inline bool tf_unit_colour(const TfDev &tf) {
+  if (tf.n <= 0 || tf.opaque) return false;
+  for (int q = 0; q < tf.n; ++q) {
+    const TfRuleDev &r = tf.rules[q];
+    if (!(r.flags & TF_WRITES_COLOR) || (r.color & 0x00FFFFFFu) != 0x00FFFFFFu || r.color != tf.rules[0].color) return false;
+  }
+  return true;
+}
 hipError_t launch_hull_table(const int2 *ends, const uint32_t *regular, float4 *hull, int X, int Y, int Z, hipStream_t s);
 constexpr uint64_t kStartTableBudget = 2ull << 30;
 hipError_t launch_primary(const RenderArgs &a, hipStream_t s);
-hipError_t launch_bounce(const RenderArgs &a, hipStream_t s);
+hipError_t launch_bounce(const RenderArgs &a, hipStream_t s, int32_t *zero_end_applied = nullptr);
 inline bool bounce_queues_fit(uint32_t n_hits, int32_t unit_block_log2, int32_t n_seeds) {
   return (uint64_t)(((n_hits + 63u) >> 6) + 8u * (1u << unit_block_log2)) * (uint64_t)n_seeds < (1ull << 24);
 }
diff --git a/cl_volume_renderer_amd/csrc/clwh_render.hip b/cl_volume_renderer_amd/csrc/clwh_render.hip
--- a/cl_volume_renderer_amd/csrc/clwh_render.hip
+++ b/cl_volume_renderer_amd/csrc/clwh_render.hip
@@ -257,6 +257,7 @@
   a.macro = packed + L.off_macro;
   a.start_free = L.start_table ? packed + L.off_start + 16u : nullptr;
   a.hull = L.hull_table ? reinterpret_cast<const float4 *>(packed + L.off_hull) : nullptr;
+  a.zero_end = ctx->tune.zero_end == 0 ? 0 : (tf_unit_colour(a.tf) ? 2 : 1);
   a.macro_shift = L.mshift;
   a.MNX = L.MNX; a.MNY = L.MNY; a.MNZ = L.MNZ;
   bool zero_may_hit = a.tf.border_class != 0;
@@ -276,6 +277,8 @@
   if (a.hull) CLWH_TRY(p.hull_codes.reserve(ctx->stream, slots * sizeof(uint32_t)));
   const bool defer = a.hull && ctx->tune.hull_defer != 0;
   if (defer) CLWH_TRY(p.hull_planes.reserve(ctx->stream, slots * sizeof(uint32_t)));
+  const bool wide = defer && ctx->tune.hull_wide != 0;
+  if (wide) CLWH_TRY(p.hull_wide.reserve(ctx->stream, slots * sizeof(uint32_t)));
   CLWH_TRY(s.counters.reserve(ctx->stream, PassScratch::kCounters * sizeof(uint32_t)));
   bool fresh_flags = false;
   CLWH_TRY(s.sticky_flags.reserve(ctx->stream, 64, &fresh_flags));
@@ -285,6 +288,8 @@
   a.hits = p.hits.as<HitRec>();
   a.hull_codes = a.hull ? p.hull_codes.as<uint32_t>() : nullptr;
   a.hull_planes = defer ? p.hull_planes.as<uint32_t>() : nullptr;
+  a.hull_wide = wide ? p.hull_wide.as<uint32_t>() : nullptr;
+  a.hull_bounce_words = wide ? a.hull_wide : a.hull_planes;
   a.counters = s.counters.as<uint32_t>();
 
   PrimaryHits::Key key;
@@ -385,7 +390,7 @@
 
 #ifdef CLVR_BOUNCE_STATS
 static int print_bounce_stats(clwh_ctx *ctx, const RenderArgs &a) {
-  uint32_t h[CTR_HULL_DEFER_END];
+  uint32_t h[CTR_REACH_END];
   HIP_TRY(hipMemcpyAsync(h, a.counters, sizeof h, hipMemcpyDeviceToHost, ctx->stream));
   HIP_TRY(hipStreamSynchronize(ctx->stream));
   auto per = [&](int sum, int n) { return h[n] ? (double)h[sum] / h[n] : 0.0; };
@@ -406,12 +411,17 @@
   std::fprintf(stderr, "[bounce stats] hull certificates tried/granted/wrong: first legs deferred=%u/%u/%u rebounds at once=%u/%u/%u rebounds deferred=%u/%u/%u; "
                "J=%d D=%.4g defer_delta0=%.6f; look-ups=%u\n", m[0], m[1], m[2], m[3], m[4], m[5], m[6], m[7], m[8], kHullDeferSteps, (double)kHullDeferDeficit,
                (double)a.hull_defer_delta0, h[CTR_CERT_LANES] - ((CLVR_BOUNCE_STATS + 0) == 2 ? m[1] + m[7] : 0u));
+  std::fprintf(stderr, "[bounce stats] zero-contribution rule (mode %d, %s) bounces asked/rays ended/wrong=%u/%u/%u; rebounds read the %s word\n", a.zero_end,
+               (CLVR_BOUNCE_STATS + 0) == 2 ? "taken" : "verified: marched literally", h[CTR_ZERO_END], h[CTR_ZERO_END + 1], h[CTR_ZERO_END + 2],
+               a.hull_wide ? "wide" : "second");
+  std::fprintf(stderr, "[bounce stats] the ray's own reach (measured only, not in the product path): marches asked/it would grant/wrong=%u/%u/%u, lane-steps they take=%u\n",
+               h[CTR_REACH], h[CTR_REACH + 1], h[CTR_REACH + 2], h[CTR_REACH + 3]);
   return CLWH_OK;
 }
 #endif
 
 static int run_pass(clwh_ctx *ctx, const RenderArgs &a) {
-  CLWH_TRY(timed(ctx, CLWH_TIMER_BOUNCE, [&] { return launch_bounce(a, ctx->stream); }));
+  CLWH_TRY(timed(ctx, CLWH_TIMER_BOUNCE, [&] { return launch_bounce(a, ctx->stream, &ctx->pass.zero_end_applied); }));
 #ifdef CLVR_BOUNCE_STATS
   CLWH_TRY(print_bounce_stats(ctx, a));
 #endif
@@ -687,6 +697,30 @@
   return CLWH_OK;
 }
 
+int clwh_debug_hull_wide(clwh_ctx *ctx, void *host_out, uint64_t capacity, uint32_t *n_hits_out) {
+  if (!ctx || !n_hits_out) return CLWH_ERR_INVALID_VALUE;
+  PrimaryHits &p = ctx->primary;
+  if (!p.valid || !p.hits.ptr || !ctx->pass.counters.ptr) return CLWH_ERR_BAD_ARGS;
+  HIP_TRY(hipSetDevice(ctx->device));
+  HIP_TRY(hipMemcpyAsync(n_hits_out, ctx->pass.counters.as<uint32_t>() + CTR_HITS, sizeof(uint32_t), hipMemcpyDeviceToHost, ctx->stream));
+  HIP_TRY(hipStreamSynchronize(ctx->stream));
+  if (!host_out) return CLWH_OK;
+  const bool built = ctx->scene && ctx->scene->hull_table && ctx->tune.hull_defer != 0 && ctx->tune.hull_wide != 0 && p.hull_wide.ptr;
+  const size_t bytes = (size_t)*n_hits_out * sizeof(uint32_t);
+  if (capacity < bytes || (built && p.hull_wide.bytes < bytes)) return CLWH_ERR_SIZE_MISMATCH;
+  if (!built) { std::memset(host_out, 0, bytes); return CLWH_OK; }
+  HIP_TRY(hipMemcpyAsync(host_out, p.hull_wide.ptr, bytes, hipMemcpyDeviceToHost, ctx->stream));
+  HIP_TRY(hipStreamSynchronize(ctx->stream));
+  return CLWH_OK;
+}
+
+int clwh_debug_zero_end(clwh_ctx *ctx, float out[2]) {
+  if (!ctx || !out) return CLWH_ERR_INVALID_VALUE;
+  out[0] = kZeroContribution;
+  out[1] = (float)ctx->pass.zero_end_applied;
+  return CLWH_OK;
+}
+
 int clwh_debug_hull_codes(clwh_ctx *ctx, void *host_out, uint64_t capacity, uint32_t *n_hits_out) {
   if (!ctx || !n_hits_out) return CLWH_ERR_INVALID_VALUE;
   PrimaryHits &p = ctx->primary;
diff --git a/cl_volume_renderer_amd/csrc/primary_kernels.hip b/cl_volume_renderer_amd/csrc/primary_kernels.hip
--- a/cl_volume_renderer_amd/csrc/primary_kernels.hip
+++ b/cl_volume_renderer_amd/csrc/primary_kernels.hip
@@ -104,6 +104,14 @@
         }
         a.hull_planes[h] = word;
       }
+      if (a.hull_wide) {
+        uint32_t word = 0u;
+        if (margin >= -128.0f / (float)kHullMarginScale) {
+          const int q = (int)fminf(floorf(margin * (float)kHullMarginScale), 127.0f);
+          word = ((uint32_t)(bj * kHullGrid + bi) + 1u) | (((uint32_t)q & 0xFFu) << 16);
+        }
+        a.hull_wide[h] = word;
+      }
     }
     q3.x = x | (y << 16); q3.y = pslot; q3.z = start_free; q3.w = 0u;
     uint4 *dst = reinterpret_cast<uint4 *>(&a.hits[h]);
diff --git a/cl_volume_renderer_amd/csrc/render_kernels.hip b/cl_volume_renderer_amd/csrc/render_kernels.hip
--- a/cl_volume_renderer_amd/csrc/render_kernels.hip
+++ b/cl_volume_renderer_amd/csrc/render_kernels.hip
@@ -23,6 +23,8 @@
   index_tables_to_lds<SMALL>(vol, a, kBounceThreads);
   __shared__ float div255[256];
   if (threadIdx.x < 256u) div255[threadIdx.x] = (float)threadIdx.x / 255.0f;
+  BounceStats stats;
+  stats.reach_init(a);
   __syncthreads();
   const uint32_t n_hits = a.n_hits_on_device ? a.counters[CTR_HITS] : a.n_hits;
   const uint32_t n_chunks = (n_hits + 63u) >> 6;
@@ -54,9 +56,8 @@
   const bool hull_cert = start_cert && a.hull_codes != nullptr;
   const bool hull_defer = hull_cert && a.hull_planes != nullptr;
   const int entry_hi_bits = hull_defer ? 3 : 8;
-  const uint32_t *hull_words = hull_defer ? a.hull_planes : a.hull_codes;
+  const uint32_t *hull_words = hull_defer ? a.hull_bounce_words : a.hull_codes;
   bool exhausted = false;
-  BounceStats stats;
 
   for (;;) {
     if (__ballot(st == ST_MARCH) != 0ull) {
@@ -176,6 +177,10 @@
         o += 1;
         ev = EV_START;
         ended = true;
+      } else if (ev == EV_ZERO) {
+        o += 1;
+        ev = EV_START;
+        ended = true;
       } else if (ev == EV_HIT || ev == EV_HIT_COLOR_PENDING) {
         i += 1;
         if (i > 10) {
@@ -191,6 +196,7 @@
         }
       }
 
+      stats.ray_end(a.counters, ended, COLD(C_BV_R), COLD(C_BV_G), COLD(C_BV_B));
       if (ended && o > 2) {
         const int fix = (int)(COLD(C_FIX) >> 2) - 2;
         if (fix == -1)
@@ -288,6 +294,10 @@
     bool hc_tried = false, hc_granted = false;
     bool rb_tried = false, rb_granted = false;
     uint32_t armed_path = 0u;
+    bool rc_candidate = false;
+    float rc_dn = 0.0f;
+    f3 rc_p{0, 0, 0}, rc_d{0, 0, 0};
+    bool ze_tried = false, ze_granted = false;
     if (st >= ST_EVENT) {
       const int ev = st - ST_EVENT;
       bool start_path = (ev == EV_START);
@@ -339,7 +349,13 @@
             sc_granted = start_certificate(word >> 24, nr.direction, a.start_cert_dmin);
           }
         }
-        if (hull_cert && (hull_defer || !from_hit)) {
+        if (a.zero_end != 0) {
+          const float bound = atten * fmaxf(fmaxf(r_energy, g_energy), b_energy) * 255.0f * (8.0f / (float)i);
+          ze_tried = true;
+          ze_granted = bound <= kZeroContribution && (o >= 2 || a.zero_end == 2);
+          if (ze_granted && !kStartCertVerify) st = ST_EVENT + EV_ZERO;
+        }
+        if (hull_cert && (hull_defer || !from_hit) && st != ST_EVENT + EV_ZERO) {
           const uint32_t word = COLD(C_ENTRY_HI);
           const uint32_t code = (word >> entry_hi_bits) & 0x1FFFu;
           const f3 n = hull_direction(code - 1u);
@@ -353,6 +369,8 @@
             m = m + dot3(n, f3{nr.origin.x - p.x, nr.origin.y - p.y, nr.origin.z - p.z});
           }
           const bool tried = code != 0u, granted = tried && dir_ok && m >= 0.0f && dn >= a.hull_delta0;
+          rc_candidate = tried && dir_ok && m >= 0.0f && !granted && !sc_granted && !ze_granted;
+          rc_dn = dn; rc_p = nr.origin; rc_d = dir;
           if (from_hit) { rb_tried = tried; rb_granted = granted; }
           else { hc_tried = tried && m >= 0.0f; hc_granted = granted; }
           if (tried && dir_ok && !sc_granted && m < 0.0f && m >= -kHullDeferDeficit && dn >= a.hull_defer_delta0)
@@ -361,7 +379,8 @@
         ray = nr;
       }
 
-      if ((sc_granted || hc_granted || rb_granted) && !kStartCertVerify) {
+      if (st == ST_EVENT + EV_ZERO) {
+      } else if ((sc_granted || hc_granted || rb_granted) && !kStartCertVerify) {
         st = ST_EVENT + EV_EXIT;
       } else {
         sd = (int)(vol.template step_i<SMALL>(f2i(ray.origin.x), f2i(ray.origin.y), f2i(ray.origin.z)) & 0x7Fu);
@@ -370,6 +389,8 @@
         st = ST_MARCH;
       }
     }
+    stats.reach(a, rc_candidate && st == ST_MARCH, rc_dn, rc_p, rc_d);
+    stats.zero_end(ze_tried, ze_granted, COLD(C_BV_R), COLD(C_BV_G), COLD(C_BV_B));
     stats.start_cert(sc_tried, sc_granted);
     stats.hull_cert(hc_tried, hc_granted, hc_granted && sc_granted);
     stats.hull_more(rb_tried, rb_granted, armed_path != 0u && st == ST_MARCH, i == 8);
@@ -378,7 +399,7 @@
 #undef COLD
 }
 
-hipError_t launch_bounce(const RenderArgs &a_in, hipStream_t s) {
+hipError_t launch_bounce(const RenderArgs &a_in, hipStream_t s, int32_t *zero_end_applied) {
   RenderArgs a = a_in;
   const uint64_t total = (uint64_t)a.n_hits * (uint64_t)a.n_seeds;
   if (total == 0) return hipSuccess;
@@ -398,6 +419,8 @@
                      a.X + a.Y + a.Z <= VolumePacked::kPartsMaxEntries;
   const size_t lds_parts_bytes = small ? (size_t)(a.X + a.Y + a.Z) * sizeof(uint32_t) : 0u;
   const bool two_rays = a.bounce_rays == 2 && long_launch && a.n_hits < (1u << 26) && kBounceThreads == 256;
+  if (!long_launch || two_rays) a.zero_end = 0;
+  if (zero_end_applied) *zero_end_applied = a.zero_end;
   if (two_rays) a.fixup_capacity = std::min<uint32_t>(a.fixup_capacity, (1u << 27) - 4u);
 #define CLVR_LAUNCH_BOUNCE(G, M)                                                                    \
   do {                                                                                              \
diff --git a/cl_volume_renderer_amd/ffi.py b/cl_volume_renderer_amd/ffi.py
--- a/cl_volume_renderer_amd/ffi.py
+++ b/cl_volume_renderer_amd/ffi.py
@@ -399,6 +399,8 @@
     ("clwh_debug_hull_cert_bound", C.c_int, [C.c_int32, C.c_int32, C.c_int32, C.POINTER(C.c_float)]),
     ("clwh_debug_hull_codes", C.c_int, [C.c_void_p, C.c_void_p, C.c_uint64, C.POINTER(C.c_uint32)]),
     ("clwh_debug_hull_planes", C.c_int, [C.c_void_p, C.c_void_p, C.c_uint64, C.POINTER(C.c_uint32)]),
+    ("clwh_debug_hull_wide", C.c_int, [C.c_void_p, C.c_void_p, C.c_uint64, C.POINTER(C.c_uint32)]),
+    ("clwh_debug_zero_end", C.c_int, [C.c_void_p, C.POINTER(C.c_float)]),
     ("clwh_debug_hull_defer_bound", C.c_int, [C.c_int32, C.c_int32, C.c_int32, C.POINTER(C.c_float)]),
     ("clwh_strerror", C.c_char_p, [C.c_int]),
     ("clwh_last_hip_error", C.c_int, []),
@@ -1171,6 +1173,18 @@
         _check(lib().clwh_debug_hull_planes(self.h, out.ctypes.data_as(C.c_void_p), C.c_uint64(out.nbytes), C.byref(n)), "clwh_debug_hull_planes")
         return out[:int(n.value)]
 
+    def hull_wide(self):
+        n = C.c_uint32(0)
+        _check(lib().clwh_debug_hull_wide(self.h, None, C.c_uint64(0), C.byref(n)), "clwh_debug_hull_wide")
+        out = np.empty(int(n.value), np.uint32)
+        _check(lib().clwh_debug_hull_wide(self.h, out.ctypes.data_as(C.c_void_p), C.c_uint64(out.nbytes), C.byref(n)), "clwh_debug_hull_wide")
+        return out[:int(n.value)]
+
+    def zero_end(self):
+        v = (C.c_float * 2)()
+        _check(lib().clwh_debug_zero_end(self.h, v), "clwh_debug_zero_end")
+        return float(v[0]), int(v[1])
+
     def hit_records(self):
         n = C.c_uint32(0)
         _check(lib().clwh_debug_hit_records(self.h, None, C.c_uint64(0), C.byref(n)), "clwh_debug_hit_records")
diff --git a/include/clwh.h b/include/clwh.h
--- a/include/clwh.h
+++ b/include/clwh.h
@@ -504,6 +504,8 @@
 int clwh_debug_hull_cert_bound(int32_t X, int32_t Y, int32_t Z, float out[2]);
 int clwh_debug_hull_codes(clwh_ctx *ctx, void *host_out, uint64_t capacity, uint32_t *n_hits_out);
 int clwh_debug_hull_planes(clwh_ctx *ctx, void *host_out, uint64_t capacity, uint32_t *n_hits_out);
+int clwh_debug_hull_wide(clwh_ctx *ctx, void *host_out, uint64_t capacity, uint32_t *n_hits_out);
+int clwh_debug_zero_end(clwh_ctx *ctx, float out[2]);
 int clwh_debug_hull_defer_bound(int32_t X, int32_t Y, int32_t Z, float out[4]);
 const char *clwh_strerror(int status);
 int clwh_last_hip_error(void);
```

Result: no change. 47030, median of 6 (+0.6%).
